# AvishaiBarnoy/membrane_solver

Measured on AMD Instinct MI355X. Metric: minimizer steps/sec (energy+grad+CG) on 2M-facet icosphere, higher is better.
Workload: dtype f64

## Files before the change

### include/membrane_hip.h

```cpp
#ifndef MEMBRANE_HIP_H
#define MEMBRANE_HIP_H

#include <stddef.h>
#include <stdint.h>

#ifdef __cplusplus
extern "C" {
#endif

#define MS_OK 0
#define MS_ERR_INVALID (-1)
#define MS_ERR_HIP (-2)
#define MS_ERR_TILE_CAPACITY (-3)
#define MS_ERR_STATE (-4)
#define MS_ERR_NOMEM (-5)

#define MS_MOD_SURFACE 1u
#define MS_MOD_BENDING 2u
#define MS_MOD_VOLUME_PENALTY 4u
#define MS_CON_VOLUME 8u
#define MS_TRACK_VOLUME 16u
#define MS_MOD_TILT 32u
#define MS_MOD_BENDING_TILT 64u
#define MS_MOD_TILT_SMOOTH 128u
// ... 162 lines not shown
  double lambda;
  double center[3];
  double normal[3];
  double radius;
} ms_disk_target_params;
int ms_set_leaflet_disk_target(ms_ctx *ctx, int leaflet, const uint8_t *disk_rows ,
                               const ms_disk_target_params *params);
int ms_set_leaflet_bending(ms_ctx *ctx, int leaflet, const double *kappa , const double *c0 );
int ms_leaflet_tilt_energy_and_gradient(ms_ctx *ctx, double *energy, double *grad_in ,
                                        double *grad_out );
int ms_leaflet_tilt_energy_and_gradient_ex(ms_ctx *ctx, int module_form, double *energy,
                                           double *grad_in , double *grad_out );
int ms_relax_leaflet_tilts(ms_ctx *ctx, const ms_tilt_relax_params *params,
                           int *iters_out, int *evals_out);

int ms_project_tilts_to_tangent(ms_ctx *ctx);

int ms_angle_defects(ms_ctx *ctx, double *defects );
int ms_curvature_fields(ms_ctx *ctx, double *mean_curvature_normal, double *h_area_anglesum,
                        double *defect_kg, double *principal);

int ms_set_positions(ms_ctx *ctx, const double *positions );
int ms_get_positions(ms_ctx *ctx, double *positions );
int ms_get_gradient(ms_ctx *ctx, double *grad );
int ms_get_vertex_buffer(ms_ctx *ctx, int buffer, double *out );

int ms_energy_and_gradient(ms_ctx *ctx, double energies[4], double *grad);
int ms_energy_and_raw_gradient(ms_ctx *ctx, double energies[4], double *grad);
int ms_energy(ms_ctx *ctx, double energies[4]);

int ms_step(ms_ctx *ctx, const ms_stepper_params *sp, double step_size,
            double tol, ms_step_result *out);
int ms_reset_stepper(ms_ctx *ctx);

typedef struct ms_minimize_params {
  ms_stepper_params stepper;
  double step_size;
  double tol;
  int fixed_step_mode;
  double fixed_step;
  int max_zero_steps;
  double step_size_floor;
  int drift_check;
  double target_volume;
  double volume_tolerance;
  int project_on_drift;
  int relax_tilts;
  ms_tilt_relax_params relax;
} ms_minimize_params;

typedef struct ms_minimize_result {
  int iterations;
  int converged;
  int zero_step_exit;
  int step_success;
  int accepted, trials, guard_rejects, moved;
  double step_size;
  double energy_eval;
  double grad_norm;
  int volume_cache_current;
  int energy_current_valid;
  double energy_current;
} ms_minimize_result;

int ms_minimize(ms_ctx *ctx, const ms_minimize_params *params, int n_steps,
                ms_minimize_result *out, double *step_log);
int ms_project_volume(ms_ctx *ctx, double target, double tol, int max_iter,
                      int *iters_out, double *volume_out);
int ms_project_volume_cached(ms_ctx *ctx, double target, double tol, int max_iter,
                             int first_step_cached, int *iters_out, double *volume_out);

int ms_phase_energy(ms_ctx *ctx, int use_direction, double alpha, int write_trial,
                    int guard, int write_bending_factors);
int ms_phase_gradient(ms_ctx *ctx);
int ms_phase_direction(ms_ctx *ctx, int stepper, int use_history);
int ms_phase_accept(ms_ctx *ctx, int keep_history);
int ms_fetch_scalars(ms_ctx *ctx, double *out );
int ms_store_scalars(ms_ctx *ctx, const double *in );

int ms_phase_commit_trial(ms_ctx *ctx, double alpha, int keep_history);

int ms_phase_gradient_direction(ms_ctx *ctx, int stepper, int use_history);
int ms_phase_set_factors_valid(ms_ctx *ctx, int valid);

int ms_boundary_info(ms_ctx *ctx, int64_t info[4]);
size_t ms_exchange_bytes(ms_ctx *ctx, int n_buffers, const int *buffer_ids);
int ms_pack_boundary(ms_ctx *ctx, int n_buffers, const int *buffer_ids,
                     void *send_dev, size_t send_bytes);
int ms_unpack_boundary(ms_ctx *ctx, int n_buffers, const int *buffer_ids,
                       const void *recv_dev, size_t stride_bytes,
                       double *scal_all_host);

typedef int (*ms_allgather_fn)(void *user, const void *send_dev, void *recv_dev,
                               size_t bytes_per_rank);
int ms_shard_unique_id(void *id128);
int ms_shard_comm_init(ms_ctx *ctx, const void *id128);
int ms_shard_set_allgather(ms_ctx *ctx, ms_allgather_fn fn, void *user);
int ms_shard_peer_export(ms_ctx *ctx, void *handles128);
int ms_shard_peer_open(ms_ctx *ctx, const void *handles_all);
int ms_shard_peer_local(ms_ctx *ctx, void **recv_slab, void **flag_words);
int ms_shard_peer_set_pointers(ms_ctx *ctx, void *const *recv_slabs, void *const *flag_words);
typedef int (*ms_barrier_fn)(void *user);
int ms_shard_peer_set_barrier(ms_ctx *ctx, ms_barrier_fn fn, void *user);
int ms_shard_step(ms_ctx *ctx, const ms_stepper_params *params, double step_size,
                  double tol, ms_step_result *out);
int64_t ms_shard_exchange_count(const ms_ctx *ctx);
int ms_shard_chain_stats(const ms_ctx *ctx, int64_t stats[8]);
int ms_shard_comm_ranks(ms_ctx *ctx);
int ms_shard_peer_memory_kind(const ms_ctx *ctx);

size_t ms_state_bytes(const ms_ctx *ctx);
int ms_rebind_state(ms_ctx *ctx, void *device_base, size_t bytes);

int ms_device_buffer(ms_ctx *ctx, int buffer, void **dev_ptr, size_t *bytes);
int ms_shard_info(ms_ctx *ctx, int64_t *nvp, int64_t *row0, int64_t *row1,
                  int64_t *rows_per_shard);
int ms_tile_stats(ms_ctx *ctx, int64_t *n_tiles, int64_t *facet_instances,
                  int64_t *max_halo, int64_t *lds_bytes_energy,
                  int64_t *lds_bytes_gradient);

#define MS_PROF_KINDS 13
int ms_profile_enable(ms_ctx *ctx, int on);
int ms_profile_read(ms_ctx *ctx, double total_ms[MS_PROF_KINDS],
                    int64_t launches[MS_PROF_KINDS]);

int ms_queue_stats(ms_ctx *ctx, int64_t stats[8]);
int ms_direction_stats(ms_ctx *ctx, int64_t *skipped, int64_t *materialized);
int ms_exec_stats(ms_ctx *ctx, int64_t stats[4]);
int ms_resident_stats(ms_ctx *ctx, int64_t stats[4]);

#define MS_PIN_STAGE_FIXED 0
#define MS_PIN_STAGE_PLANE_GROUP 1
#define MS_PIN_STAGE_CIRCLE_GROUP 2
#define MS_PIN_OP_PLANE 0
#define MS_PIN_OP_CIRCLE 1
#define MS_PIN_GRAD_PLANE 0
#define MS_PIN_GRAD_CIRCLE 1
#define MS_PIN_GRAD_RADIAL 2
#define MS_PIN_LANE_SKIP 0
#define MS_PIN_LANE_PROJECT 1
int ms_set_pins(ms_ctx *ctx, int n_params, const double *params, int n_stages, const int32_t *stage_kind,
                const int32_t *stage_param, const int32_t *stage_off, const int32_t *item_row,
                const int32_t *item_arg, int lane, int n_grad, const int32_t *grad_row, const int32_t *grad_kind,
                const int32_t *grad_param, int n_avg, const int32_t *avg_param, const int32_t *avg_off,
                const int32_t *avg_row);
int ms_enforce_pins(ms_ctx *ctx);
int ms_pin_stats(ms_ctx *ctx, int64_t stats[4]);
int ms_tsearch_stats(ms_ctx *ctx, int64_t stats[2]);
int ms_exec_trace(ms_ctx *ctx, int on, double *rows, int max_rows, int *n_rows);

int ms_plan_tiling(int nv, int nf, const double *positions, const int32_t *tri,
                   int tile_vertices, int shard_count, int64_t stats[8],
                   int32_t *perm_out);
int ms_plan_tiling_conflicts(int nv, int nf, const double *positions,
                             const int32_t *tri, int tile_vertices, double model[4]);

int ms_surface_energy_and_gradient_host(int nv, int nf, const double *pos,
                                        const int32_t *tri, const double *gamma,
                                        double *grad, double *energy);
int ms_grad_cotan_batch_host(int n, const double *u, const double *v,
                             double *grad_u, double *grad_v);
int ms_apply_beltrami_laplacian_host(int dim, int nv, int nf,
                                     const double *weights, const int32_t *tri,
                                     const double *field, double *out);
int ms_p1_triangle_divergence_host(int nv, int nf, const double *pos,
                                   const double *tilts, const int32_t *tri,
                                   double *div_tri, double *area, double *g0,
                                   double *g1, double *g2);
int ms_compute_curvature_data_host(int nv, int nf, const double *pos,
                                   const int32_t *tri, double *k_vecs,
                                   double *vertex_areas, double *weights,
                                   double *va0, double *va1, double *va2);

#ifdef __cplusplus
}
#endif
#endif
```

### membrane_solver_amd/_lib.py

```python

from __future__ import annotations

import ctypes
import os
import subprocess

_PKG = os.path.dirname(os.path.abspath(__file__))
LIB_PATH = os.environ.get("MEMBRANE_HIP_LIB") or os.path.join(_PKG, "libmembrane_hip.so")
_CSRC = os.path.join(_PKG, "csrc")

MS_OK = 0
MS_ERR = {-1: "MS_ERR_INVALID", -2: "MS_ERR_HIP", -3: "MS_ERR_TILE_CAPACITY",
          -4: "MS_ERR_STATE", -5: "MS_ERR_NOMEM"}

MS_MOD_SURFACE = 1
MS_MOD_BENDING = 2
MS_MOD_VOLUME_PENALTY = 4
MS_CON_VOLUME = 8
MS_TRACK_VOLUME = 16
MS_MOD_TILT = 32
MS_MOD_BENDING_TILT = 64
MS_MOD_TILT_SMOOTH = 128
MS_MOD_TILT_IN, MS_MOD_TILT_OUT, MS_MOD_TILT_SMOOTH_IN, MS_MOD_TILT_SMOOTH_OUT = 256, 512, 1024, 2048
MS_MOD_BENDING_TILT_IN, MS_MOD_BENDING_TILT_OUT = 4096, 8192
# ... 42 lines not shown
                ("tol", ctypes.c_double), ("jacobi", ctypes.c_int)]


class ms_leaflet_params(ctypes.Structure):
    _fields_ = [("tilt_modulus", ctypes.c_double), ("tilt_mass_consistent", ctypes.c_int),
                ("smoothness", ctypes.c_double), ("precond_smoothness", ctypes.c_double)]


class ms_disk_target_params(ctypes.Structure):
    _fields_ = [("strength", ctypes.c_double), ("theta_b", ctypes.c_double), ("lam", ctypes.c_double),
                ("center", ctypes.c_double * 3), ("normal", ctypes.c_double * 3), ("radius", ctypes.c_double)]


class ms_minimize_params(ctypes.Structure):
    _fields_ = [("stepper", ms_stepper_params), ("step_size", ctypes.c_double), ("tol", ctypes.c_double),
                ("fixed_step_mode", ctypes.c_int), ("fixed_step", ctypes.c_double),
                ("max_zero_steps", ctypes.c_int), ("step_size_floor", ctypes.c_double),
                ("drift_check", ctypes.c_int), ("target_volume", ctypes.c_double),
                ("volume_tolerance", ctypes.c_double), ("project_on_drift", ctypes.c_int),
                ("relax_tilts", ctypes.c_int), ("relax", ms_tilt_relax_params)]


class ms_minimize_result(ctypes.Structure):
    _fields_ = [("iterations", ctypes.c_int), ("converged", ctypes.c_int), ("zero_step_exit", ctypes.c_int),
                ("step_success", ctypes.c_int), ("accepted", ctypes.c_int), ("trials", ctypes.c_int),
                ("guard_rejects", ctypes.c_int), ("moved", ctypes.c_int), ("step_size", ctypes.c_double),
                ("energy_eval", ctypes.c_double), ("grad_norm", ctypes.c_double),
                ("volume_cache_current", ctypes.c_int), ("energy_current_valid", ctypes.c_int),
                ("energy_current", ctypes.c_double)]


class ms_step_result(ctypes.Structure):
    _fields_ = [("success", ctypes.c_int), ("converged", ctypes.c_int), ("trials", ctypes.c_int),
                ("guard_rejects", ctypes.c_int), ("next_step", ctypes.c_double),
                ("energy", ctypes.c_double), ("alpha", ctypes.c_double),
                ("energy_eval", ctypes.c_double), ("grad_norm", ctypes.c_double),
                ("g_dot_d", ctypes.c_double), ("volume", ctypes.c_double)]


_P = ctypes.c_void_p
_D = ctypes.POINTER(ctypes.c_double)
_I32 = ctypes.POINTER(ctypes.c_int32)
_U8 = ctypes.POINTER(ctypes.c_uint8)
_I64 = ctypes.POINTER(ctypes.c_int64)

ALLGATHER_FN = ctypes.CFUNCTYPE(ctypes.c_int, ctypes.c_void_p, ctypes.c_void_p, ctypes.c_void_p, ctypes.c_size_t)

SIGNATURES = {
    "ms_version": (ctypes.c_char_p, []),
    "ms_device_count": (ctypes.c_int, []),
    "ms_last_error": (ctypes.c_char_p, [_P]),
    "ms_create": (ctypes.c_int, [ctypes.POINTER(_P), ctypes.c_int, ctypes.c_int, ctypes.c_int, _D,
                                 _I32, _U8, _U8, _U8, ctypes.c_int, ctypes.c_int, ctypes.c_int]),
    "ms_destroy": (None, [_P]),
    "ms_set_stream": (ctypes.c_int, [_P, _P]),
    "ms_set_surface_tension": (ctypes.c_int, [_P, _D]),
    "ms_set_bending_params": (ctypes.c_int, [_P, _D, _D]),
    "ms_set_params": (ctypes.c_int, [_P, ctypes.POINTER(ms_params)]),
    "ms_set_area_penalty": (ctypes.c_int, [_P, ctypes.c_double, ctypes.c_double]),
    "ms_get_body_area": (ctypes.c_int, [_P, _D]),
    "ms_set_line_tension": (ctypes.c_int, [_P, ctypes.c_int, _I32, _I32, _D]),
    "ms_get_line_energy": (ctypes.c_int, [_P, _D]),
    "ms_line_stats": (ctypes.c_int, [_P, _D]),
    "ms_line_tables_host": (ctypes.c_int, [ctypes.c_int, _I32, ctypes.c_int, _I32, _I32, _D, _I32, _I32, _I32, _D, _I32,
                                          _I32, _I32, _D]),
    "ms_set_tilts": (ctypes.c_int, [_P, _D, ctypes.c_double]),
    "ms_get_tilts": (ctypes.c_int, [_P, _D]),
    "ms_get_tilt_gradient": (ctypes.c_int, [_P, _D]),
    "ms_project_tilts_to_tangent": (ctypes.c_int, [_P]),
    "ms_angle_defects": (ctypes.c_int, [_P, _D]),
    "ms_curvature_fields": (ctypes.c_int, [_P, _D, _D, _D, _D]),
    "ms_set_tilt_fixed": (ctypes.c_int, [_P, ctypes.POINTER(ctypes.c_uint8)]),
    "ms_set_tilt_smoothness": (ctypes.c_int, [_P, ctypes.c_double]),
    "ms_set_deterministic": (ctypes.c_int, [_P, ctypes.c_int]),
    "ms_tilt_energy_and_gradient": (ctypes.c_int, [_P, _D, _D]),
    "ms_relax_tilts": (ctypes.c_int, [_P, ctypes.POINTER(ms_tilt_relax_params),
                                      ctypes.POINTER(ctypes.c_int), ctypes.POINTER(ctypes.c_int)]),
    "ms_set_leaflet_tilts": (ctypes.c_int, [_P, ctypes.c_int, _D, ctypes.POINTER(ctypes.c_uint8),
                                            ctypes.POINTER(ms_leaflet_params)]),
    "ms_get_leaflet_tilts": (ctypes.c_int, [_P, ctypes.c_int, _D]),
    "ms_set_leaflet_bending": (ctypes.c_int, [_P, ctypes.c_int, _D, _D]),
    "ms_set_leaflet_disk_target": (ctypes.c_int, [_P, ctypes.c_int, ctypes.POINTER(ctypes.c_uint8),
                                                  ctypes.POINTER(ms_disk_target_params)]),
    "ms_leaflet_tilt_energy_and_gradient": (ctypes.c_int, [_P, _D, _D, _D]),
    "ms_leaflet_tilt_energy_and_gradient_ex": (ctypes.c_int, [_P, ctypes.c_int, _D, _D, _D]),
    "ms_relax_leaflet_tilts": (ctypes.c_int, [_P, ctypes.POINTER(ms_tilt_relax_params),
                                              ctypes.POINTER(ctypes.c_int), ctypes.POINTER(ctypes.c_int)]),
    "ms_set_positions": (ctypes.c_int, [_P, _D]),
    "ms_get_positions": (ctypes.c_int, [_P, _D]),
    "ms_get_gradient": (ctypes.c_int, [_P, _D]),
    "ms_get_vertex_buffer": (ctypes.c_int, [_P, ctypes.c_int, _D]),
    "ms_energy_and_gradient": (ctypes.c_int, [_P, _D, _D]),
    "ms_energy_and_raw_gradient": (ctypes.c_int, [_P, _D, _D]),
    "ms_energy": (ctypes.c_int, [_P, _D]),
    "ms_step": (ctypes.c_int, [_P, ctypes.POINTER(ms_stepper_params), ctypes.c_double,
                               ctypes.c_double, ctypes.POINTER(ms_step_result)]),
    "ms_reset_stepper": (ctypes.c_int, [_P]),
    "ms_minimize": (ctypes.c_int, [_P, ctypes.POINTER(ms_minimize_params), ctypes.c_int,
                                   ctypes.POINTER(ms_minimize_result), _D]),
    "ms_project_volume": (ctypes.c_int, [_P, ctypes.c_double, ctypes.c_double, ctypes.c_int,
                                         ctypes.POINTER(ctypes.c_int), _D]),
    "ms_project_volume_cached": (ctypes.c_int, [_P, ctypes.c_double, ctypes.c_double, ctypes.c_int, ctypes.c_int,
                                                ctypes.POINTER(ctypes.c_int), _D]),
    "ms_phase_energy": (ctypes.c_int, [_P, ctypes.c_int, ctypes.c_double, ctypes.c_int,
                                       ctypes.c_int, ctypes.c_int]),
    "ms_phase_gradient": (ctypes.c_int, [_P]),
    "ms_phase_direction": (ctypes.c_int, [_P, ctypes.c_int, ctypes.c_int]),
    "ms_phase_accept": (ctypes.c_int, [_P, ctypes.c_int]),
    "ms_phase_commit_trial": (ctypes.c_int, [_P, ctypes.c_double, ctypes.c_int]),
    "ms_phase_gradient_direction": (ctypes.c_int, [_P, ctypes.c_int, ctypes.c_int]),
    "ms_phase_set_factors_valid": (ctypes.c_int, [_P, ctypes.c_int]),
    "ms_boundary_info": (ctypes.c_int, [_P, _I64]),
    "ms_exchange_bytes": (ctypes.c_size_t, [_P, ctypes.c_int, ctypes.POINTER(ctypes.c_int)]),
    "ms_pack_boundary": (ctypes.c_int, [_P, ctypes.c_int, ctypes.POINTER(ctypes.c_int), _P,
                                        ctypes.c_size_t]),
    "ms_unpack_boundary": (ctypes.c_int, [_P, ctypes.c_int, ctypes.POINTER(ctypes.c_int), _P,
                                          ctypes.c_size_t, _D]),
    "ms_shard_unique_id": (ctypes.c_int, [_P]),
    "ms_shard_comm_init": (ctypes.c_int, [_P, _P]),
    "ms_shard_set_allgather": (ctypes.c_int, [_P, ALLGATHER_FN, _P]),
    "ms_shard_step": (ctypes.c_int, [_P, ctypes.POINTER(ms_stepper_params), ctypes.c_double, ctypes.c_double,
                                     ctypes.POINTER(ms_step_result)]),
    "ms_shard_exchange_count": (ctypes.c_int64, [_P]),
    "ms_shard_chain_stats": (ctypes.c_int, [_P, _I64]),
    "ms_shard_comm_ranks": (ctypes.c_int, [_P]),
    "ms_shard_peer_memory_kind": (ctypes.c_int, [_P]),
    "ms_state_bytes": (ctypes.c_size_t, [_P]),
    "ms_rebind_state": (ctypes.c_int, [_P, _P, ctypes.c_size_t]),
    "ms_fetch_scalars": (ctypes.c_int, [_P, _D]),
    "ms_store_scalars": (ctypes.c_int, [_P, _D]),
    "ms_device_buffer": (ctypes.c_int, [_P, ctypes.c_int, ctypes.POINTER(_P),
                                        ctypes.POINTER(ctypes.c_size_t)]),
    "ms_shard_info": (ctypes.c_int, [_P, _I64, _I64, _I64, _I64]),
    "ms_tile_stats": (ctypes.c_int, [_P, _I64, _I64, _I64, _I64, _I64]),
    "ms_profile_enable": (ctypes.c_int, [_P, ctypes.c_int]),
    "ms_profile_read": (ctypes.c_int, [_P, _D, _I64]),
    "ms_queue_stats": (ctypes.c_int, [_P, _I64]),
    "ms_direction_stats": (ctypes.c_int, [_P, _I64, _I64]),
    "ms_exec_stats": (ctypes.c_int, [_P, _I64]),
    "ms_resident_stats": (ctypes.c_int, [_P, _I64]),
    "ms_set_pins": (ctypes.c_int, [_P, ctypes.c_int, _D, ctypes.c_int, _I32, _I32, _I32, _I32, _I32, ctypes.c_int,
                                   ctypes.c_int, _I32, _I32, _I32, ctypes.c_int, _I32, _I32, _I32]),
    "ms_enforce_pins": (ctypes.c_int, [_P]),
    "ms_pin_stats": (ctypes.c_int, [_P, _I64]),
    "ms_tsearch_stats": (ctypes.c_int, [_P, _I64]),
    "ms_exec_trace": (ctypes.c_int, [_P, ctypes.c_int, _D, ctypes.c_int, ctypes.POINTER(ctypes.c_int)]),
    "ms_shard_peer_export": (ctypes.c_int, [_P, _P]),
    "ms_shard_peer_open": (ctypes.c_int, [_P, _P]),
    "ms_shard_peer_local": (ctypes.c_int, [_P, ctypes.POINTER(_P), ctypes.POINTER(_P)]),
    "ms_shard_peer_set_pointers": (ctypes.c_int, [_P, ctypes.POINTER(_P), ctypes.POINTER(_P)]),
    "ms_shard_peer_set_barrier": (ctypes.c_int, [_P, _P, _P]),
    "ms_plan_tiling": (ctypes.c_int, [ctypes.c_int, ctypes.c_int, _D, _I32, ctypes.c_int, ctypes.c_int,
                                      _I64, _I32]),
    "ms_plan_tiling_conflicts": (ctypes.c_int, [ctypes.c_int, ctypes.c_int, _D, _I32, ctypes.c_int, _D]),
    "ms_surface_energy_and_gradient_host": (ctypes.c_int, [ctypes.c_int, ctypes.c_int, _D, _I32, _D,
                                                           _D, _D]),
    "ms_grad_cotan_batch_host": (ctypes.c_int, [ctypes.c_int, _D, _D, _D, _D]),
    "ms_apply_beltrami_laplacian_host": (ctypes.c_int, [ctypes.c_int, ctypes.c_int, ctypes.c_int, _D,
                                                        _I32, _D, _D]),
    "ms_p1_triangle_divergence_host": (ctypes.c_int, [ctypes.c_int, ctypes.c_int, _D, _D, _I32, _D,
                                                      _D, _D, _D, _D]),
    "ms_compute_curvature_data_host": (ctypes.c_int, [ctypes.c_int, ctypes.c_int, _D, _I32, _D, _D,
                                                      _D, _D, _D, _D]),
}

_lib = None


def build(force: bool = False, fp_contract: str | None = None) -> str:
    srcs = [os.path.join(_CSRC, f) for f in ("ms_kernels.hip", "ms_pins.hip", "ms_line.hip", "ms_api.cpp",
                                             "ms_tiles.cpp", "ms_internal.h", "Makefile")]
    srcs.append(os.path.join(_PKG, "..", "include", "membrane_hip.h"))
    stale = (not os.path.exists(LIB_PATH)) or any(
        os.path.exists(s) and os.path.getmtime(s) > os.path.getmtime(LIB_PATH) for s in srcs)
    if force or stale:
        cmd = ["make", "-s", "-C", _CSRC]
        if force:
            cmd.append("-B")
        if fp_contract:
            cmd.append(f"MS_FP_CONTRACT={fp_contract}")
        subprocess.check_call(cmd)
    return LIB_PATH


HIP_RUNTIME_PATH = None


def _preload_hip_runtime() -> str:
    global HIP_RUNTIME_PATH
    if HIP_RUNTIME_PATH is not None:
        return HIP_RUNTIME_PATH
    candidates = []
    if os.environ.get("MEMBRANE_HIP_RUNTIME"):
        candidates.append(os.environ["MEMBRANE_HIP_RUNTIME"])
    try:
        import importlib.util

        spec = importlib.util.find_spec("torch")
        if spec is not None and spec.submodule_search_locations:
            candidates.append(os.path.join(list(spec.submodule_search_locations)[0], "lib", "libamdhip64.so"))
    except Exception:
        pass
    rocm = os.environ.get("ROCM_PATH", "/opt/rocm")
    candidates += [os.path.join(rocm, "lib", "libamdhip64.so"), "libamdhip64.so.7", "libamdhip64.so"]
    errors = []
    for c in candidates:
        if os.path.isabs(c) and not os.path.exists(c):
            continue
        try:
            ctypes.CDLL(c, mode=ctypes.RTLD_GLOBAL)
            HIP_RUNTIME_PATH = c
            return c
        except OSError as e:
            errors.append(f"{c}: {e}")
    raise MembraneHipError("no HIP runtime (libamdhip64) could be loaded: " + "; ".join(errors))


def lib() -> ctypes.CDLL:
    global _lib
    if _lib is None:
        if not os.path.exists(LIB_PATH):
            raise MembraneHipError(
                f"{LIB_PATH} is missing: run `python -c 'import __graft_entry__ as g; g.build()'` "
                "(hipcc --offload-arch=gfx950).  There is no CPU fallback for this path.")
        _preload_hip_runtime()
        cd = ctypes.CDLL(LIB_PATH)
        for name, (res, args) in SIGNATURES.items():
            fn = getattr(cd, name)
            fn.restype = res
            fn.argtypes = args
        _lib = cd
    return _lib


def check(rc: int, ctx=None, what: str = "") -> None:
    if rc == MS_OK:
        return
    msg = lib().ms_last_error(ctx)
    text = msg.decode("utf-8", "replace") if msg else ""
    raise MembraneHipError(f"{what or 'libmembrane_hip'} failed: {MS_ERR.get(rc, rc)}: {text}")
```

### membrane_solver_amd/csrc/ms_api_context.inc

```
extern "C" {

const char* ms_version(void) { return "membrane_hip 0.1 (gfx950)"; }

int ms_device_count(void) {
  int n = 0;
  hipError_t e = hipGetDeviceCount(&n);
  if (e != hipSuccess) {
    g_last_error = std::string("hipGetDeviceCount: ") + hipGetErrorString(e);
    return MS_ERR_HIP;
  }
  return n;
}

const char* ms_last_error(const ms_ctx* ctx) {
  return ctx ? ctx->err.c_str() : g_last_error.c_str();
}

int ms_create(ms_ctx** out, int device, int nv, int nf, const double* positions,
              const int32_t* tri, const uint8_t* fixed, const uint8_t* boundary,
              const uint8_t* body_facets, int tile_vertices, int shard_rank, int shard_count) {
  if (!out) return fail(nullptr, MS_ERR_INVALID, "ms_create: out is NULL");
  *out = nullptr;
  if (shard_count < 1 || shard_rank < 0 || shard_rank >= shard_count)
    return fail(nullptr, MS_ERR_INVALID, "ms_create: bad shard_rank/shard_count");
  ms_ctx* c = new (std::nothrow) ms_ctx();
  if (!c) return fail(nullptr, MS_ERR_NOMEM, "ms_create: out of host memory");
  std::string err;
  int rc = build_tiling(nv, nf, positions, tri, body_facets, tile_vertices, shard_count, c->til, err);
  if (rc != MS_OK) {
    delete c;
    return fail(nullptr, rc, err);
  }
  c->device = device;
  c->shard_rank = shard_rank;
  c->shard_count = shard_count;
  const Tiling& t = c->til;
  c->tile0 = std::min(t.n_tiles, shard_rank * t.tiles_per_shard);
  c->tile1 = std::min(t.n_tiles, (shard_rank + 1) * t.tiles_per_shard);
  c->cap = t.own + t.max_halo;
  {
    const size_t le = energy_lds_bytes(t.T, c->cap, t.max_ent, true, true, true);
    const size_t lg = gradient_lds_bytes(t.T, c->cap, t.max_ent, true, true);
    if (le > 160 * 1024 || lg > 160 * 1024) {
      delete c;
      return fail(nullptr, MS_ERR_TILE_CAPACITY,
                  "ms_create: a vertex patch (tile + halo) exceeds the 160 KiB LDS of a CU; "
                  "use a smaller tile_vertices");
    }
  }
#define CREATE_CHK(call)                                       \
  do {                                                         \
    int rc_ = (call);                                          \
    if (rc_ != MS_OK) {                                        \
      std::string m_ = c->err;                                 \
      ms_destroy(c);                                           \
      return fail(nullptr, rc_, m_);                           \
    }                                                          \
  } while (0)
#define CREATE_HIP(call)                                                         \
  do {                                                                           \
    hipError_t e_ = (call);                                                      \
    if (e_ != hipSuccess) {                                                      \
      std::string m_ = std::string(#call) + ": " + hipGetErrorString(e_);        \
      ms_destroy(c);                                                             \
      return fail(nullptr, MS_ERR_HIP, m_);                                      \
    }                                                                            \
  } while (0)
  CREATE_HIP(hipSetDevice(device));
  CREATE_HIP(hipStreamCreateWithFlags(&c->stream, hipStreamNonBlocking));
  c->own_stream = true;
  CREATE_CHK(upload(c, &c->d_perm, t.perm));
  CREATE_CHK(upload(c, &c->d_tile_facet_off, t.tile_facet_off));
  CREATE_CHK(upload(c, &c->d_tile_facets, t.tile_facets));
  if (t.own + t.max_halo <= 1024) {
    std::vector<uint32_t> packed(t.tile_facets.size());
    for (size_t i = 0; i < packed.size(); ++i) {
      const TileFacet& f = t.tile_facets[i];
      packed[i] = (uint32_t)f.l0 | ((uint32_t)f.l1 << 10) | ((uint32_t)f.l2 << 20) | ((uint32_t)(f.flags & 3u) << 30);
    }
    CREATE_CHK(upload(c, &c->d_tile_facets32, packed));
  }
  CREATE_CHK(upload(c, &c->d_tile_halo_off, t.tile_halo_off));
  CREATE_CHK(upload(c, &c->d_halo_ids, t.halo_ids));
  CREATE_CHK(upload(c, &c->d_tile_ent_off, t.tile_ent_off));
  CREATE_CHK(upload(c, &c->d_tile_voff, t.tile_voff));
  CREATE_CHK(upload(c, &c->d_vent, t.vent));
  {
    std::vector<double> ones(t.tile_facets.size(), 1.0);
    CREATE_CHK(upload(c, &c->d_tf_gamma, ones));
  }
  {
    std::vector<uint8_t> fl((size_t)t.nvp, VF_FIXED);
    for (int i = 0; i < nv; ++i) {
      const int e = t.perm[i];
      uint8_t f = 0;
      if (fixed && fixed[e]) f |= VF_FIXED;
      if (boundary && boundary[e]) {
        f |= VF_BOUNDARY;
        c->has_boundary = true;
      }
      fl[i] = f;
    }
    CREATE_CHK(upload(c, &c->d_vflags, fl));
    c->h_vflags = fl;
    std::vector<double> zeros((size_t)t.nvp, 0.0);
    CREATE_CHK(upload(c, &c->d_kappa, zeros));
    CREATE_CHK(upload(c, &c->d_c0, zeros));
  }
  {
    const size_t n3 = 3 * (size_t)t.nvp;
    const size_t total = 8 * n3 + 2 * (size_t)t.nvp;
    CREATE_HIP(hipMalloc(reinterpret_cast<void**>(&c->state), total * sizeof(double)));
    CREATE_HIP(hipMemset(c->state, 0, total * sizeof(double)));
    for (int b = 0; b <= MS_BUF_FK; ++b) c->buf[b] = c->state + (size_t)b * n3;
    c->buf[MS_BUF_FA] = c->state + 8 * n3;
  }
  CREATE_HIP(hipMalloc(reinterpret_cast<void**>(&c->d_partials),
                       sizeof(double) * MS_NPART * (size_t)std::max(1, t.n_tiles)));
  CREATE_HIP(hipMemset(c->d_partials, 0, sizeof(double) * MS_NPART * (size_t)std::max(1, t.n_tiles)));
  CREATE_HIP(hipMalloc(reinterpret_cast<void**>(&c->d_scal), sizeof(double) * MS_NSCAL));
  CREATE_HIP(hipMemset(c->d_scal, 0, sizeof(double) * MS_NSCAL));
  c->buf[MS_BUF_SCAL] = c->d_scal;
  c->h_scal = static_cast<double*>(calloc(MS_NSCAL, sizeof(double)));
  CREATE_HIP(hipHostMalloc(reinterpret_cast<void**>(&c->h_seq), sizeof(unsigned long long) * 2 * MS_MB_WORDS,
                           hipHostMallocMapped));
  memset(c->h_seq, 0, sizeof(unsigned long long) * 2 * MS_MB_WORDS);
  CREATE_HIP(hipHostGetDevicePointer(reinterpret_cast<void**>(&c->d_h_seq), c->h_seq, 0));
  CREATE_HIP(hipHostMalloc(reinterpret_cast<void**>(&c->h_err), sizeof(unsigned long long) * 8, hipHostMallocMapped));
  memset(c->h_err, 0, sizeof(unsigned long long) * 8);
  CREATE_HIP(hipHostGetDevicePointer(reinterpret_cast<void**>(&c->d_h_err), c->h_err, 0));
  CREATE_HIP(hipMalloc(reinterpret_cast<void**>(&c->d_stage), sizeof(double) * 3 * (size_t)nv));
  {
    const int W = shard_count;
    const int rows_per = t.tiles_per_shard * t.own;
    std::vector<std::vector<int32_t>> lists((size_t)W);
    std::vector<int32_t> my_halo;
    for (int tile = 0; tile < t.n_tiles; ++tile) {
      const int tr = tile / t.tiles_per_shard;
      for (int h = t.tile_halo_off[tile]; h < t.tile_halo_off[tile + 1]; ++h) {
        const int32_t v = t.halo_ids[h];
        const int owner = v / rows_per;
        if (owner == tr) continue;
        lists[(size_t)owner].push_back(v);
        if (tr == shard_rank) my_halo.push_back(v);
      }
    }
    std::vector<int32_t> flat;
    c->bnd_off.assign((size_t)W + 1, 0);
    for (int r = 0; r < W; ++r) {
      auto& l = lists[(size_t)r];
      std::sort(l.begin(), l.end());
      l.erase(std::unique(l.begin(), l.end()), l.end());
      c->bnd_off[(size_t)r + 1] = c->bnd_off[(size_t)r] + (int32_t)l.size();
      c->bnd_max = std::max(c->bnd_max, (int)l.size());
      flat.insert(flat.end(), l.begin(), l.end());
    }
    std::sort(my_halo.begin(), my_halo.end());
    my_halo.erase(std::unique(my_halo.begin(), my_halo.end()), my_halo.end());
    c->n_halo_rows = (int)my_halo.size();
    CREATE_CHK(upload(c, &c->d_bnd_rows, flat));
    CREATE_CHK(upload(c, &c->d_bnd_off, c->bnd_off));
    CREATE_CHK(upload(c, &c->d_halo_rows, my_halo));
    CREATE_HIP(hipMalloc(reinterpret_cast<void**>(&c->d_scal_all), sizeof(double) * MS_NSCAL * (size_t)W));
    CREATE_HIP(hipMemset(c->d_scal_all, 0, sizeof(double) * MS_NSCAL * (size_t)W));
  }
  {
    TiltField& f0 = c->tf[0];
    f0.fixed_bit = VF_TILT_FIXED; f0.mod_tilt = MS_MOD_TILT; f0.mod_smooth = MS_MOD_TILT_SMOOTH;
    f0.s_etilt = MS_S_ETILT; f0.s_ets = MS_S_ETS; f0.s_gn2 = MS_S_TGNORM2; f0.s_rz = MS_S_TRZ;
    TiltField& f1 = c->tf[1];
    f1.fixed_bit = VF_TILT_FIXED_IN; f1.mod_tilt = MS_MOD_TILT_IN; f1.mod_smooth = MS_MOD_TILT_SMOOTH_IN;
    f1.s_etilt = MS_S_ETILT_IN; f1.s_ets = MS_S_ETS_IN; f1.s_gn2 = MS_S_TGNORM2_IN; f1.s_rz = MS_S_TRZ_IN;
    f1.mod_bt = MS_MOD_BENDING_TILT_IN; f1.s_ebt = MS_S_EBT_IN; f1.div_sign = -1.0;
    f0.mod_bt = MS_MOD_BENDING_TILT; f0.s_ebt = MS_S_EBT;
    f1.mod_dt = MS_MOD_TILT_DISK_TARGET_IN; f1.s_edt = MS_S_EDT_IN; f1.s_dtr = MS_S_DTR_IN;
    TiltField& f2 = c->tf[2];
    f2.fixed_bit = VF_TILT_FIXED_OUT; f2.mod_tilt = MS_MOD_TILT_OUT; f2.mod_smooth = MS_MOD_TILT_SMOOTH_OUT;
    f2.s_etilt = MS_S_ETILT_OUT; f2.s_ets = MS_S_ETS_OUT; f2.s_gn2 = MS_S_TGNORM2_OUT; f2.s_rz = MS_S_TRZ_OUT;
    f2.mod_bt = MS_MOD_BENDING_TILT_OUT; f2.s_ebt = MS_S_EBT_OUT; f2.div_sign = 1.0;
    f2.mod_dt = MS_MOD_TILT_DISK_TARGET_OUT; f2.s_edt = MS_S_EDT_OUT; f2.s_dtr = MS_S_DTR_OUT;
  }
  if (const char* pe = getenv("MS_PAIR")) {
    c->pair_enable = atoi(pe) != 0;
    c->pair_force = atoi(pe) >= 2 ? std::min(atoi(pe), 4) : 0;
  }
  c->speculate = !(getenv("MS_SPECULATE") != nullptr && atoi(getenv("MS_SPECULATE")) == 0);
  c->ahead_enable = !(getenv("MS_AHEAD") != nullptr && atoi(getenv("MS_AHEAD")) == 0);
  c->escalate = !(getenv("MS_ESCALATE") != nullptr && atoi(getenv("MS_ESCALATE")) == 0);
  if (getenv("MS_ESCALATE") != nullptr && atoi(getenv("MS_ESCALATE")) > 0) c->escalate_after = atoi(getenv("MS_ESCALATE"));
  c->ls_reset = !(getenv("MS_LS_RESET") != nullptr && atoi(getenv("MS_LS_RESET")) == 0);
  c->no_fast = variant_env("MS_NO_FAST") != nullptr && atoi(variant_env("MS_NO_FAST")) != 0;
  c->pair_lean_enable = !(getenv("MS_PAIR_LEAN") != nullptr && atoi(getenv("MS_PAIR_LEAN")) == 0);
  c->deterministic = getenv("MS_DETERMINISTIC") != nullptr && atoi(getenv("MS_DETERMINISTIC")) != 0;
  c->resident_enable = !(getenv("MS_RESIDENT") != nullptr && atoi(getenv("MS_RESIDENT")) == 0);
  c->params.modules = MS_MOD_SURFACE;
  c->params.bending_model = MS_BEND_HELFRICH;
  c->params.bending_grad_mode = MS_GRAD_ANALYTIC;
  c->params.volume_stiffness = 1000.0;
  c->params.target_volume = 0.0;
  c->carry.last_g = c->buf[MS_BUF_G];
  c->exec_wanted = t.n_tiles == 1 && t.T == 256 && t.own == 256 && shard_count == 1 &&
                   !(getenv("MS_EXEC") != nullptr && atoi(getenv("MS_EXEC")) == 0);
  if (c->exec_wanted) {
    c->exec.stream = c->stream;
    c->exec.T = t.T;
    exec_attach(&c->exec);
    c->exec_on = true;
    c->pair_enable = false;
    c->exec_relax = !(getenv("MS_EXEC_RELAX") != nullptr && atoi(getenv("MS_EXEC_RELAX")) == 0);
    c->exec_fused = !(getenv("MS_EXEC_FUSED") != nullptr && atoi(getenv("MS_EXEC_FUSED")) == 0);
  }
  c->shard_chain_enable = !(getenv("MS_SHARD_CHAIN") != nullptr && atoi(getenv("MS_SHARD_CHAIN")) == 0);
  c->tenergy_enable = shard_count == 1 && !(getenv("MS_TSEARCH") != nullptr && atoi(getenv("MS_TSEARCH")) == 0);
  c->tsearch_enable = !c->exec_on && c->tenergy_enable;
  CREATE_CHK(ext_to_patch(c, positions, c->buf[MS_BUF_X], 3));
#undef CREATE_CHK
#undef CREATE_HIP
  *out = c;
  return MS_OK;
}

void ms_destroy(ms_ctx* c) {
  if (g_host_timing.on && g_host_timing.n > 0) {
    fprintf(stderr, "[ms host timing] %ld waits followed by an energy launch: mailbox seen -> launch call returned %.2f us "
                    "on average (max %.1f), of which the launch call itself %.2f us\n",
            g_host_timing.n, g_host_timing.sum_gap / g_host_timing.n, g_host_timing.max_gap,
            g_host_timing.sum_launch / g_host_timing.n);
    g_host_timing.n = 0;
    g_host_timing.sum_gap = g_host_timing.sum_launch = g_host_timing.max_gap = 0.0;
  }
  if (!c) return;
  (void)hipSetDevice(c->device);
  if (c->exec_on) {
    (void)c->exec.flush();
    exec_detach(&c->exec);
    c->exec_on = false;
  }
  if (c->stream) (void)hipStreamSynchronize(c->stream);
  if (!c->own_state) c->state = nullptr;
  void* ptrs[] = {c->d_perm, c->d_tile_facet_off, c->d_tile_facets, c->d_tile_facets32, c->d_tf_gamma, c->d_volgrad_cache,
                  c->d_tile_halo_off, c->d_halo_ids, c->d_tile_ent_off, c->d_tile_voff, c->d_vent,
                  c->d_vflags, c->d_kappa, c->d_c0, c->tf[0].tilts, c->tf[0].grad, c->tf[0].trial, c->d_bt_vert, c->d_tn, c->tf[0].dir, c->tf[0].minv,
                  c->tf[1].tilts, c->tf[1].grad, c->tf[1].trial, c->tf[1].dir, c->tf[1].minv,
                  c->tf[2].tilts, c->tf[2].grad, c->tf[2].trial, c->tf[2].dir, c->tf[2].minv,
                  c->tf[1].kappa, c->tf[1].c0, c->tf[1].bt_vert, c->tf[2].kappa, c->tf[2].c0, c->tf[2].bt_vert,
                  c->tf[1].disk, c->tf[1].diff, c->tf[2].disk, c->tf[2].diff, c->tf[0].va, c->tf[1].va, c->tf[2].va,
                  c->state, c->d_partials, c->d_scal, c->d_stage, c->d_bnd_rows, c->d_bnd_off,
                  c->d_halo_rows, c->d_scal_all, c->d_pins, c->d_line};
  for (void* p : ptrs)
    if (p) (void)hipFree(p);
  for (auto& evs : c->line_prof)
    for (auto& ev : evs) {
      (void)hipEventDestroy(ev.first);
      (void)hipEventDestroy(ev.second);
    }
  for (void* q : c->peer_opened) (void)hipIpcCloseMemHandle(q);
  if (c->d_peer_slab) (void)hipFree(c->d_peer_slab);
  if (c->d_peer_flag) (void)hipFree(c->d_peer_flag);
  if (c->d_peer_flagtab) (void)hipFree(c->d_peer_flagtab);
  if (c->d_peer_arrived) (void)hipFree(c->d_peer_arrived);
  if (c->comm) shard_comm_destroy(c->comm);
  if (c->d_xsend) (void)hipFree(c->d_xsend);
  if (c->d_xrecv) (void)hipFree(c->d_xrecv);
  if (c->h_scal_all) (void)hipHostFree(c->h_scal_all);
  if (c->h_xseq) (void)hipHostFree(c->h_xseq);
  for (int p = 0; p < 2; ++p) {
    for (auto& m : c->spec[p]) {
      free(m.h_scal);
      if (m.h_seq) (void)hipHostFree(m.h_seq);
    }
    for (ms_ctx::Mailbox* m : {&c->grad_mb[p], &c->first_mb[p]}) {
      free(m->h_scal);
      if (m->h_seq) (void)hipHostFree(m->h_seq);
    }
  }
  if (c->d_sh_dec) (void)hipFree(c->d_sh_dec);
  if (c->h_sh_post) (void)hipHostFree(c->h_sh_post);
  free(c->tsearch_mb.h_scal);
  if (c->tsearch_mb.h_seq) (void)hipHostFree(c->tsearch_mb.h_seq);
  if (c->d_dec) (void)hipFree(c->d_dec);
  if (c->h_err) (void)hipHostFree(c->h_err);
  if (c->d_prof_ran) (void)hipFree(c->d_prof_ran);
  if (c->exec.d_stamps) (void)hipFree(c->exec.d_stamps);
  if (c->d_res_partials) (void)hipFree(c->d_res_partials);
  if (c->d_res_bar) (void)hipFree(c->d_res_bar);
  if (c->d_res_log) (void)hipFree(c->d_res_log);
  if (c->d_res_result) (void)hipFree(c->d_res_result);
  for (int l = 0; l < 3; ++l)
    if (c->tf[l].dt_target) (void)hipFree(c->tf[l].dt_target);
  if (c->d_relax_cells) (void)hipFree(c->d_relax_cells);
  if (c->h_relax_box) (void)hipHostFree(c->h_relax_box);
  for (auto& sd : c->side) {
    if (sd.partials) (void)hipFree(sd.partials);
    if (sd.scal) (void)hipFree(sd.scal);
    for (auto& m : sd.mb) {
      free(m.h_scal);
      if (m.h_seq) (void)hipHostFree(m.h_seq);
    }
  }
  for (double* q : {c->xt2, c->fK2, c->fA2, c->xt3, c->fK3, c->fA3})
    if (q) (void)hipFree(q);
  free(c->h_scal);
  if (c->h_seq) (void)hipHostFree(c->h_seq);
  for (auto& r : c->prof_pending) {
    (void)hipEventDestroy(r.a);
    (void)hipEventDestroy(r.b);
  }
  for (auto e : c->prof_pool) (void)hipEventDestroy(e);
  if (c->own_stream && c->stream) (void)hipStreamDestroy(c->stream);
  delete c;
}

int ms_set_stream(ms_ctx* c, void* hip_stream) {
  if (!c) return MS_ERR_INVALID;
  HIPCHK(c, hipStreamSynchronize(S(c)));
  if (c->own_stream && c->stream) {
    HIPCHK(c, hipStreamDestroy(c->stream));
    c->own_stream = false;
  }
  if (hip_stream) {
    c->stream = static_cast<hipStream_t>(hip_stream);
  } else {
    HIPCHK(c, hipStreamCreateWithFlags(&c->stream, hipStreamNonBlocking));
    c->own_stream = true;
  }
  if (c->exec_on) {
    exec_detach(&c->exec);
    c->exec.stream = c->stream;
    if (exec_find(c->stream) != nullptr) {
      c->exec_on = false;
      c->exec_wanted = false;
    } else {
      exec_attach(&c->exec);
    }
  } else {
    c->exec.stream = c->stream;
  }
  return MS_OK;
}

int ms_set_surface_tension(ms_ctx* c, const double* gamma) {
  if (!c || !gamma) return fail(c, MS_ERR_INVALID, "ms_set_surface_tension: NULL argument");
  const Tiling& t = c->til;
  HIPCHK(c, hipStreamSynchronize(S(c)));
  std::vector<double> g(t.tile_facets.size());
  for (size_t p = 0; p < g.size(); ++p) g[p] = gamma[t.tile_facet_ext[p]];
  c->gamma_uniform = true;
  c->gamma_const = t.nf > 0 ? gamma[0] : 1.0;
  for (int f = 1; f < t.nf && c->gamma_uniform; ++f) c->gamma_uniform = gamma[f] == c->gamma_const;
  if (!g.empty())
    HIPCHK(c, hipMemcpy(c->d_tf_gamma, g.data(), g.size() * sizeof(double), hipMemcpyHostToDevice));
  c->carry.carry_valid = c->carry.grad_valid = c->carry.bt_valid = c->carry.maxg2_valid = false;
  c->sh_carry_valid = c->sh_grad_valid = false;
  return MS_OK;
}

int ms_set_bending_params(ms_ctx* c, const double* kappa, const double* c0) {
  if (!c || !kappa || !c0) return fail(c, MS_ERR_INVALID, "ms_set_bending_params: NULL argument");
  const Tiling& t = c->til;
  HIPCHK(c, hipStreamSynchronize(S(c)));
  std::vector<double> k((size_t)t.nvp, 0.0), z((size_t)t.nvp, 0.0);
  c->kc_uniform = true;
  c->kappa_const = kappa[0];
  c->c0_const = c0[0];
  for (int i = 0; i < t.nv; ++i) {
    k[i] = kappa[t.perm[i]];
    z[i] = c0[t.perm[i]];
    c->kc_uniform = c->kc_uniform && kappa[i] == c->kappa_const && c0[i] == c->c0_const;
  }
  HIPCHK(c, hipMemcpy(c->d_kappa, k.data(), k.size() * sizeof(double), hipMemcpyHostToDevice));
  HIPCHK(c, hipMemcpy(c->d_c0, z.data(), z.size() * sizeof(double), hipMemcpyHostToDevice));
  c->carry.factors_valid = false;
  c->carry.carry_valid = c->carry.grad_valid = c->carry.bt_valid = c->carry.maxg2_valid = false;
  c->sh_carry_valid = c->sh_grad_valid = false;
  return MS_OK;
}

int ms_set_params(ms_ctx* c, const ms_params* p) {
  if (!c || !p) return fail(c, MS_ERR_INVALID, "ms_set_params: NULL argument");
  if (p->bending_model != MS_BEND_HELFRICH && p->bending_model != MS_BEND_WILLMORE)
    return fail(c, MS_ERR_INVALID, "ms_set_params: bad bending_model");
  if (p->bending_grad_mode != MS_GRAD_ANALYTIC && p->bending_grad_mode != MS_GRAD_APPROX)
    return fail(c, MS_ERR_INVALID, "ms_set_params: bad bending_grad_mode");
  if ((p->modules & MS_MOD_BENDING) && (p->modules & MS_MOD_BENDING_TILT))
    return fail(c, MS_ERR_INVALID, "ms_set_params: bending and bending_tilt are mutually exclusive");
  if ((p->modules & MS_LEAFLET_BT) && (p->modules & (MS_MOD_BENDING | MS_MOD_BENDING_TILT)))
    return fail(c, MS_ERR_INVALID, "ms_set_params: bending / bending_tilt together with bending_tilt_in/out is outside the device path");
  if ((p->modules & MS_MOD_BENDING_TILT) && c->shard_count != 1)
    return fail(c, MS_ERR_STATE, "the bending_tilt module is not sharded yet (single GPU only)");
  if ((p->modules & MS_MOD_AREA_PENALTY) && c->shard_count != 1)
    return fail(c, MS_ERR_STATE, "the body_area_penalty module is not sharded (single GPU only)");
  if ((p->modules & MS_MOD_AREA_PENALTY) && (p->modules & MS_ANY_TILT_MODS))
    return fail(c, MS_ERR_STATE, "body_area_penalty together with a tilt-family module is outside the device path");
  if ((p->modules & MS_MOD_LINE_TENSION) && c->shard_count != 1)
    return fail(c, MS_ERR_STATE, "the line_tension module is not sharded (single GPU only)");
  if ((p->modules & MS_MOD_LINE_TENSION) && (p->modules & MS_ANY_TILT_MODS))
    return fail(c, MS_ERR_STATE, "line_tension together with a tilt-family module is outside the device path");
  if ((p->modules & MS_MOD_BENDING_TILT) && !c->d_bt_vert) {
    const size_t bytes = sizeof(double) * 4 * (size_t)c->til.nvp;
    HIPCHK(c, hipMalloc(reinterpret_cast<void**>(&c->d_bt_vert), bytes));
    HIPCHK(c, hipMemset(c->d_bt_vert, 0, bytes));
  }
  c->params = *p;
  c->carry.factors_valid = false;
  c->carry.carry_valid = c->carry.grad_valid = c->carry.bt_valid = c->carry.maxg2_valid = false;
  c->sh_carry_valid = c->sh_grad_valid = false;
  return MS_OK;
}

int ms_set_area_penalty(ms_ctx* c, double stiffness, double target_area) {
  if (!c) return MS_ERR_INVALID;
  if (!std::isfinite(stiffness) || !std::isfinite(target_area))
    return fail(c, MS_ERR_INVALID, "ms_set_area_penalty: stiffness and target area must be finite");
  c->area_stiffness = stiffness;
  c->target_area = target_area;
  c->carry.carry_valid = c->carry.grad_valid = c->carry.maxg2_valid = false;
  c->sh_carry_valid = c->sh_grad_valid = false;
  return MS_OK;
}

int ms_get_body_area(ms_ctx* c, double* area) {
  if (!c || !area) return fail(c, MS_ERR_INVALID, "ms_get_body_area: NULL argument");
  if (!(c->params.modules & MS_MOD_AREA_PENALTY))
    return fail(c, MS_ERR_STATE, "ms_get_body_area: MS_MOD_AREA_PENALTY is not in the module mask");
  int rc = fetch(c);
  if (rc) return rc;
  *area = c->h_scal[MS_S_AREA];
  return MS_OK;
}

int ms_set_tilts(ms_ctx* c, const double* tilts, double tilt_rigidity) {
  if (!c || !tilts) return fail(c, MS_ERR_INVALID, "ms_set_tilts: NULL argument");
  const size_t bytes = sizeof(double) * 3 * (size_t)c->til.nvp;
  if (!c->tf[0].tilts) {
    HIPCHK(c, hipMalloc(reinterpret_cast<void**>(&c->tf[0].tilts), bytes));
    HIPCHK(c, hipMalloc(reinterpret_cast<void**>(&c->tf[0].grad), bytes));
    HIPCHK(c, hipMalloc(reinterpret_cast<void**>(&c->tf[0].trial), bytes));
    HIPCHK(c, hipMemset(c->tf[0].trial, 0, bytes));
    HIPCHK(c, hipMemset(c->tf[0].tilts, 0, bytes));
    HIPCHK(c, hipMemset(c->tf[0].grad, 0, bytes));
  }
  c->tf[0].k_tilt = tilt_rigidity;
  c->carry.carry_valid = c->carry.grad_valid = c->carry.bt_valid = c->carry.maxg2_valid = false;
  c->sh_carry_valid = c->sh_grad_valid = false;
  return ext_to_patch(c, tilts, c->tf[0].tilts, 3);
}

int ms_get_tilts(ms_ctx* c, double* tilts) {
  if (!c || !tilts || !c->tf[0].tilts) return fail(c, MS_ERR_INVALID, "ms_get_tilts: no tilts set");
  return patch_to_ext(c, c->tf[0].tilts, tilts, 3);
}

int ms_get_tilt_gradient(ms_ctx* c, double* tilt_grad) {
  if (!c || !tilt_grad || !c->tf[0].grad) return fail(c, MS_ERR_INVALID, "ms_get_tilt_gradient: no tilts set");
  return patch_to_ext(c, c->tf[0].grad, tilt_grad, 3);
}

int ms_angle_defects(ms_ctx* c, double* defects) {
  if (!c || !defects) return fail(c, MS_ERR_INVALID, "ms_angle_defects: NULL argument");
  if (c->shard_count != 1) return fail(c, MS_ERR_STATE, "ms_angle_defects: single shard only");
  const Tiling& t = c->til;
  double* d_out = nullptr;
  HIPCHK(c, hipMalloc(reinterpret_cast<void**>(&d_out), sizeof(double) * (size_t)std::max<int64_t>(1, t.nvp)));
  HIPCHK(c, hipMemsetAsync(d_out, 0, sizeof(double) * (size_t)std::max<int64_t>(1, t.nvp), S(c)));
  TiltArgs a;
  a.fields = nullptr;
  a.fields_rows = 0;
  a.m = device_mesh(c);
  a.tile0 = c->tile0;
  a.tile1 = c->tile1;
  a.x = c->buf[MS_BUF_X];
  a.d = nullptr;
  a.alpha = 0.0;
  a.tilts = c->buf[MS_BUF_X];
  a.tilts_out = nullptr;
  a.k_tilt = 0.0;
  a.g = nullptr;
  a.tilt_grad = nullptr;
  a.minv = d_out;
  a.partials = c->d_partials;
  a.e_slot = MS_S_ETILT;
  a.consistent = 0;
  a.tg_accumulate = 0;
  a.cons_tilt_grad = 0;
  a.va_out = nullptr;
  hipError_t e = launch_tilt(a, 4, c->cap, t.max_ent, c->stream);
  int rc = MS_OK;
  if (e != hipSuccess) rc = fail(c, MS_ERR_HIP, std::string("ms_angle_defects: ") + hipGetErrorString(e));
  if (rc == MS_OK) rc = patch_to_ext(c, d_out, defects, 1);
  (void)hipStreamSynchronize(S(c));
  (void)hipFree(d_out);
  return rc;
}

int ms_curvature_fields(ms_ctx* c, double* mean_curvature_normal, double* h_area_anglesum, double* defect_kg,
                        double* principal) {
  if (!c) return MS_ERR_INVALID;
  if (c->shard_count != 1) return fail(c, MS_ERR_STATE, "ms_curvature_fields: single shard only");
  const Tiling& t = c->til;
  const size_t plane = 3 * (size_t)std::max<int64_t>(1, t.nvp);
  double* d_out = nullptr;
  HIPCHK(c, hipMalloc(reinterpret_cast<void**>(&d_out), sizeof(double) * 4 * plane));
  HIPCHK(c, hipMemsetAsync(d_out, 0, sizeof(double) * 4 * plane, S(c)));
  TiltArgs a;
// ... 78 lines not shown
```

### membrane_solver_amd/csrc/ms_api_ctx.inc

```
struct StageCtl {
  const uint32_t* cur_gate = nullptr;
  uint32_t cur_gate_want = 0;
  bool cur_gate_fold_only = false;
  bool cur_check_ran = false;
  uint32_t* cur_dec = nullptr;
  double cur_rhs[MS_MAX_TRIALS] = {0};
  const double* cur_rhs_dev = nullptr;
  uint32_t cur_extra_mask = 0;
  int cur_go_kind = 0;
  uint32_t* cur_go = nullptr;
  double cur_go_val[6] = {0};
  int cur_parity = 0;
  int pair_on = 0;
  bool pair_lean = false;
  double pair_alpha[MS_MAX_TRIALS] = {0};
  double* pair_scal2 = nullptr;
  bool multi_any_slot = false;
  bool defer_dir = false;
  bool energy_tilt_only = false;
  bool proj_at_x_in_normals = false;
};
struct CarryState {
  bool dir_implicit = false;
  bool dir_unwritten = false;
  bool pd_neg_pg = false;
  bool kc_pending = false;
  int kc_parity = 0;
  bool bt_valid = false;
  double* last_g = nullptr;
  bool cg_have_history = false;
  int cg_iter_count = 0;
  bool factors_valid = false;
  bool carry_valid = false;
  bool grad_valid = false;
  bool maxg2_valid = false;
};
struct ms_ctx {
  int device = 0;
  hipStream_t stream = nullptr;
  bool own_stream = false;
  Tiling til;
  int shard_rank = 0, shard_count = 1;
  int tile0 = 0, tile1 = 0;
  int cap = 0;
  int32_t* d_perm = nullptr;
  int32_t* d_tile_facet_off = nullptr;
  TileFacet* d_tile_facets = nullptr;
  uint32_t* d_tile_facets32 = nullptr;
  double* d_tf_gamma = nullptr;
  double* d_volgrad_cache = nullptr;
  double volgrad_cache_norm2 = 0.0;
  bool volgrad_cache_valid = false;
  bool gamma_uniform = true, kc_uniform = true;
  double gamma_const = 1.0, kappa_const = 0.0, c0_const = 0.0;
  int32_t* d_tile_halo_off = nullptr;
  int32_t* d_halo_ids = nullptr;
  int32_t* d_tile_ent_off = nullptr;
  uint16_t* d_tile_voff = nullptr;
  uint16_t* d_vent = nullptr;
  uint8_t* d_vflags = nullptr;
  double* d_kappa = nullptr;
  double* d_c0 = nullptr;
  struct TiltField {
    double* tilts = nullptr;
    double* trial = nullptr;
    double* grad = nullptr;
    double* dir = nullptr;
    double* minv = nullptr;
    double k_tilt = 0.0;
    int consistent = 0;
    double k_smooth = 0.0;
    double k_smooth_precond = 0.0;
    uint8_t fixed_bit = 0;
    uint32_t mod_tilt = 0, mod_smooth = 0, mod_bt = 0;
    int s_etilt = 0, s_ets = 0, s_gn2 = 0, s_rz = 0, s_ebt = 0;
    double* kappa = nullptr;
    double* c0 = nullptr;
    double* bt_vert = nullptr;
    double div_sign = 1.0;
    uint8_t* disk = nullptr;
    double* diff = nullptr;
    double* dt_target = nullptr;
    bool dt_target_valid = false;
    ms_disk_target_params dt = {};
    uint32_t mod_dt = 0;
    int s_edt = 0, s_dtr = 0;
    bool any_free = true;
    double* va = nullptr;
  } tf[3];
  CarryState carry;
  bool precond = false;
  static constexpr int SPEC_STAGES = 3;
  struct Mailbox {
    double* h_scal = nullptr;
    unsigned long long* h_seq = nullptr;
    unsigned long long* d_h_seq = nullptr;
    unsigned long long expected[MS_MB_WORDS] = {0};
  } spec[2][SPEC_STAGES];
  Mailbox first_mb[2];
  Mailbox grad_mb[2];
  int next_parity = 0;
  struct RoundPlanT {
    int n0 = 1, n_st = 0;
    double alphas[MS_MAX_TRIALS + SPEC_STAGES] = {0};
  };
  struct Ahead {
    bool valid = false;
    bool go_known = false, go = false;
    int kind = 0, go_kind = 0, parity = 0, src = 0, stepper = 0, max_iter = 0;
    bool implicit = false;
    double alpha0 = 0, energy0 = 0, beta = 0, c1 = 0, tol2p = 0, lim = 0;
    RoundPlanT plan;
  } ahead;
  bool ahead_enable = true;
  int steps_left = 0;
  bool ahead_allowed = false;
  uint32_t dir_deferred_mask = 0;
  bool dir_pending[2] = {false, false};
  uint32_t dir_mask[2] = {0, 0};
  uint32_t* kc_gate[2] = {nullptr, nullptr};
  bool last_hist_descent = false;
  long q_ahead = 0, q_adopted = 0, q_dropped = 0;
  int kc_stepper = 0;
  bool kc_use_history = false;
  bool kc_dir_unwritten[2] = {false, false};
  long dir_skipped = 0, dir_materialized = 0;
  uint32_t* d_dec = nullptr;
  static constexpr int N_DEC = 16;
  unsigned long long* h_err = nullptr;
  unsigned long long* d_h_err = nullptr;
  long queue_mismatches = 0;
  long q_rounds = 0, q_multi = 0, q_wasted = 0, q_side_accepts = 0;
  int escalate_after = 3;
  bool pair_enable = true;
  bool escalate = true;
  int pair_force = 0;
  bool lbt_normals_current = false;
  bool tenergy_enable = true;
  bool tsearch_enable = true;
  bool tsearch_first_single = true;
  int64_t tsearch_launches = 0, tsearch_trials = 0;
  bool tsearch_all_failed = false;
  Mailbox tsearch_mb;
  bool no_fast = false;
  bool pair_lean_enable = true;
  static constexpr int N_SIDE = MS_MAX_TRIALS - 1;
  struct SideSet {
    double* partials = nullptr;
    double* scal = nullptr;
    Mailbox mb[2];
  } side[N_SIDE];
  double* xt3 = nullptr;
  double* fK3 = nullptr;
  double* fA3 = nullptr;
  double* xt2 = nullptr;
  double* fK2 = nullptr;
  double* fA2 = nullptr;
  static constexpr int LS_HIST = 8;
  struct LsHist {
    int pred_trials = 1;
    double acc[LS_HIST] = {0};
    double rej[LS_HIST] = {0};
    int n = 0;
  } ls[2];
  bool ls_reset = true;
  bool speculate = true;
  bool relax_va_valid = false;
  bool tilt_module_form = false;
  int factors_leaflet = 0;
  double* d_bt_vert = nullptr;
  double* d_tn = nullptr;
  std::vector<uint8_t> h_vflags;
  double* state = nullptr;
  bool own_state = true;
  double* buf[MS_BUF_COUNT] = {nullptr};
  double* d_partials = nullptr;
  double* d_scal = nullptr;
  double* h_scal = nullptr;
  unsigned long long* h_seq = nullptr;
  unsigned long long* d_h_seq = nullptr;
  unsigned long long ticket = 0;
  unsigned long long expected[MS_MB_WORDS] = {0};
  bool has_boundary = false;
  double* d_stage = nullptr;
  ms_params params{};
  double area_stiffness = 0.0, target_area = 0.0;
  std::vector<int32_t> bnd_off;
  int32_t* d_bnd_rows = nullptr;
  int32_t* d_bnd_off = nullptr;
  int bnd_max = 0;
  int32_t* d_halo_rows = nullptr;
  int n_halo_rows = 0;
  double* d_scal_all = nullptr;
  void* comm = nullptr;
  ms_allgather_fn allgather_cb = nullptr;
  void* allgather_user = nullptr;
  double* d_xsend = nullptr;
  double* d_xrecv = nullptr;
  bool shard_chain_enable = true;
  uint32_t* d_sh_dec = nullptr;
  unsigned long long* h_sh_post = nullptr;
// ... 93 lines not shown
```

### membrane_solver_amd/csrc/ms_api_misc.inc

```
size_t ms_state_bytes(const ms_ctx* c) {
  if (!c) return 0;
  return sizeof(double) * (8 * 3 * (size_t)c->til.nvp + 2 * (size_t)c->til.nvp);
}

int ms_rebind_state(ms_ctx* c, void* device_base, size_t bytes) {
  if (!c || !device_base) return fail(c, MS_ERR_INVALID, "ms_rebind_state: NULL argument");
  const size_t need = ms_state_bytes(c);
  if (bytes < need) return fail(c, MS_ERR_INVALID, "ms_rebind_state: buffer smaller than ms_state_bytes");
  HIPCHK(c, hipStreamSynchronize(S(c)));
  HIPCHK(c, hipMemcpy(device_base, c->state, need, hipMemcpyDeviceToDevice));
  double* nb = static_cast<double*>(device_base);
  for (int b = 0; b <= MS_BUF_FA; ++b) c->buf[b] = nb + (c->buf[b] - c->state);
  c->carry.last_g = nb + (c->carry.last_g - c->state);
  if (c->own_state) HIPCHK(c, hipFree(c->state));
  c->state = nb;
  c->own_state = false;
  return MS_OK;
}

int ms_fetch_scalars(ms_ctx* c, double* out) {
  if (!c || !out) return MS_ERR_INVALID;
  int rc = fetch(c);
  if (rc) return rc;
  memcpy(out, c->h_scal, sizeof(double) * MS_NSCAL);
// ... 54 lines not shown
  for (int k = 0; k < 8; ++k) stats[k] = 0;
  stats[0] = c->q_rounds;
  stats[1] = c->q_multi;
  stats[2] = c->q_wasted;
  stats[3] = c->q_side_accepts;
  stats[4] = c->queue_mismatches;
  stats[5] = c->q_ahead;
  stats[6] = c->q_adopted;
  stats[7] = c->q_dropped;
  return MS_OK;
}

int ms_direction_stats(ms_ctx* c, int64_t* skipped, int64_t* materialized) {
  if (!c || !skipped || !materialized) return MS_ERR_INVALID;
  *skipped = c->dir_skipped;
  *materialized = c->dir_materialized;
  return MS_OK;
}

int ms_resident_stats(ms_ctx* c, int64_t stats[4]) {
  if (!c || !stats) return MS_ERR_INVALID;
  stats[0] = c->resident_ok;
  stats[1] = c->resident_launches;
  stats[2] = c->resident_steps;
  stats[3] = c->resident_bails;
  return MS_OK;
}

int ms_tsearch_stats(ms_ctx* c, int64_t stats[2]) {
  if (!c || !stats) return MS_ERR_INVALID;
  stats[0] = c->tsearch_launches;
  stats[1] = c->tsearch_trials;
  return MS_OK;
}

int ms_exec_stats(ms_ctx* c, int64_t stats[4]) {
  if (!c || !stats) return MS_ERR_INVALID;
  stats[0] = c->exec_on ? 1 : 0;
  stats[1] = c->exec.launches;
  stats[2] = c->exec.cmds;
  stats[3] = (c->exec_wanted ? 1 : 0) | ((int64_t)(c->relax_programs & 0xffffff) << 8) | ((int64_t)c->relax_fused_runs << 32);
  return MS_OK;
}

int ms_exec_trace(ms_ctx* c, int on, double* rows, int max_rows, int* n_rows) {
  if (!c) return MS_ERR_INVALID;
  if (n_rows) *n_rows = 0;
  int rc = exec_flush(c);
  if (rc) return rc;
  HIPCHK(c, hipStreamSynchronize(c->stream));
  if (c->exec.d_stamps && rows && max_rows > 0 && n_rows) {
    std::vector<unsigned long long> h((size_t)2 * EXEC_STAMP_CAP);
    HIPCHK(c, hipMemcpy(h.data(), c->exec.d_stamps, sizeof(unsigned long long) * h.size(), hipMemcpyDeviceToHost));
    const size_t n = (size_t)std::min<unsigned long long>(h[0], (unsigned long long)EXEC_STAMP_CAP - 1);
    std::map<unsigned long long, std::pair<long, double>> acc;
    for (size_t i = 0; i < n; ++i) {
      auto& e = acc[h[1 + 2 * i]];
      e.first += 1;
      e.second += 0.01 * (double)h[2 + 2 * i];
    }
    int k = 0;
    for (auto& kv : acc) {
      if (k >= max_rows) break;
      rows[4 * k] = (double)(kv.first >> 32);
      rows[4 * k + 1] = (double)(kv.first & 0xffffffffull);
      rows[4 * k + 2] = (double)kv.second.first;
      rows[4 * k + 3] = kv.second.second;
      ++k;
    }
    *n_rows = k;
  }
  if (on && !c->exec.d_stamps)
    HIPCHK(c, hipMalloc(reinterpret_cast<void**>(&c->exec.d_stamps), sizeof(unsigned long long) * 2 * EXEC_STAMP_CAP));
  if (c->exec.d_stamps) HIPCHK(c, hipMemset(c->exec.d_stamps, 0, sizeof(unsigned long long) * 2 * EXEC_STAMP_CAP));
  if (!on && c->exec.d_stamps) {
    (void)hipFree(c->exec.d_stamps);
    c->exec.d_stamps = nullptr;
  }
  return MS_OK;
}

int ms_profile_enable(ms_ctx* c, int on) {
  if (!c) return MS_ERR_INVALID;
  if (on && !c->d_prof_ran) {
    HIPCHK(c, hipMalloc(reinterpret_cast<void**>(&c->d_prof_ran), sizeof(uint32_t) * ms_ctx::PROF_RAN_CAP));
    HIPCHK(c, hipMemset(c->d_prof_ran, 0, sizeof(uint32_t) * ms_ctx::PROF_RAN_CAP));
  }
  if (on && c->exec_on) {
    int rc = exec_flush(c);
    if (rc) return rc;
    exec_detach(&c->exec);
    c->exec_on = false;
  } else if (!on && c->exec_wanted && !c->exec_on) {
    c->exec.stream = c->stream;
    exec_attach(&c->exec);
    c->exec_on = true;
  }
  c->profiling = on != 0;
  return MS_OK;
}

int ms_profile_read(ms_ctx* c, double total_ms[MS_PROF_KINDS], int64_t launches[MS_PROF_KINDS]) {
  if (!c || !total_ms || !launches) return MS_ERR_INVALID;
  HIPCHK(c, hipStreamSynchronize(S(c)));
  std::vector<uint32_t> ran((size_t)c->prof_ran_next);
  if (c->prof_ran_next > 0)
    HIPCHK(c, hipMemcpy(ran.data(), c->d_prof_ran, sizeof(uint32_t) * ran.size(), hipMemcpyDeviceToHost));
  c->prof_ran_next = 0;
  for (auto& r : c->prof_pending) {
    float ms = 0.f;
    const bool empty = r.ran_idx >= 0 && ran[(size_t)r.ran_idx] == 0u;
    if (hipEventElapsedTime(&ms, r.a, r.b) == hipSuccess && !empty) {
      c->prof_ms[r.kind] += ms;
      c->prof_n[r.kind] += 1;
    }
    c->prof_pool.push_back(r.a);
    c->prof_pool.push_back(r.b);
  }
  c->prof_pending.clear();
  for (int k = 0; k < MS_PROF_KINDS; ++k) {
    total_ms[k] = c->prof_ms[k];
    launches[k] = c->prof_n[k];
    c->prof_ms[k] = 0.0;
    c->prof_n[k] = 0;
  }
  return MS_OK;
}

int ms_plan_tiling(int nv, int nf, const double* positions, const int32_t* tri, int tile_vertices,
                   int shard_count, int64_t stats[8], int32_t* perm_out) {
  if (!stats) return fail(nullptr, MS_ERR_INVALID, "ms_plan_tiling: stats is NULL");
  Tiling t;
  std::string err;
  int rc = build_tiling(nv, nf, positions, tri, nullptr, tile_vertices, shard_count, t, err);
  if (rc != MS_OK) return fail(nullptr, rc, err);
  int64_t owners = 0, owned_corners = 0;
  for (int tile = 0; tile < t.n_tiles; ++tile) {
    const int n_owned = std::min(t.own, t.nv - tile * t.own);
    for (int p = t.tile_facet_off[tile]; p < t.tile_facet_off[tile + 1]; ++p) {
      const TileFacet& f = t.tile_facets[p];
      if (f.flags & TF_OWNER) ++owners;
      owned_corners += (f.l0 < n_owned) + (f.l1 < n_owned) + (f.l2 < n_owned);
    }
  }
  stats[0] = t.n_tiles;
  stats[1] = (int64_t)t.tile_facets.size();
  stats[2] = t.max_halo;
  stats[3] = t.max_tile_facets;
  stats[4] = t.dropped_facets;
  stats[5] = owners;
  stats[6] = owned_corners;
  stats[7] = (int64_t)gradient_lds_bytes(t.T, t.own + t.max_halo, t.max_ent, true, true);
  if (perm_out) memcpy(perm_out, t.perm.data(), sizeof(int32_t) * (size_t)nv);
  return MS_OK;
}

int ms_plan_tiling_conflicts(int nv, int nf, const double* positions, const int32_t* tri, int tile_vertices,
                             double model[4]) {
  if (!model) return fail(nullptr, MS_ERR_INVALID, "ms_plan_tiling_conflicts: model is NULL");
  Tiling t;
  std::string err;
  int rc = build_tiling(nv, nf, positions, tri, nullptr, tile_vertices, 1, t, err);
  if (rc != MS_OK) return fail(nullptr, rc, err);
  double rd_cyc = 0, at_cyc = 0, rd_free = 0, at_free = 0;
  int64_t rd_groups = 0, at_groups = 0;
  for (int tile = 0; tile < t.n_tiles; ++tile) {
    const int n_owned = std::min(t.own, t.nv - tile * t.own);
    const int f0 = t.tile_facet_off[tile], f1 = t.tile_facet_off[tile + 1];
    for (int k = 0; k < 3; ++k) {
      for (int g0 = f0; g0 < f1; g0 += 32) {
        int slots[32], ns = 0, cnt[32] = {0};
        for (int p = g0; p < std::min(f1, g0 + 32); ++p) {
          const TileFacet& f = t.tile_facets[p];
          const int s = k == 0 ? f.l0 : (k == 1 ? f.l1 : f.l2);
          bool dup = false;
          for (int q = 0; q < ns; ++q) dup |= slots[q] == s;
          if (!dup) {
            slots[ns++] = s;
            ++cnt[s & 31];
          }
        }
        int mx = 1;
        for (int q = 0; q < 32; ++q) mx = std::max(mx, cnt[q]);
        rd_cyc += mx;
        rd_free += mx == 1;
        ++rd_groups;
      }
      for (int g0 = f0; g0 < f1; g0 += 16) {
        int cnt[16] = {0}, any = 0;
        for (int p = g0; p < std::min(f1, g0 + 16); ++p) {
          const TileFacet& f = t.tile_facets[p];
          const int s = k == 0 ? f.l0 : (k == 1 ? f.l1 : f.l2);
          if (s < n_owned) {
            ++cnt[s & 15];
            any = 1;
          }
        }
        if (!any) continue;
        int mx = 1;
        for (int q = 0; q < 16; ++q) mx = std::max(mx, cnt[q]);
        at_cyc += mx;
        at_free += mx == 1;
        ++at_groups;
      }
    }
  }
  model[0] = rd_groups ? rd_cyc / rd_groups : 0.0;
  model[1] = at_groups ? at_cyc / at_groups : 0.0;
  model[2] = rd_groups ? rd_free / rd_groups : 0.0;
  model[3] = at_groups ? at_free / at_groups : 0.0;
  return MS_OK;
}


int ms_surface_energy_and_gradient_host(int nv, int nf, const double* pos, const int32_t* tri,
                                        const double* gamma, double* grad, double* energy) {
  if (!pos || !gamma || !energy || (nf > 0 && !tri))
    return fail(nullptr, MS_ERR_INVALID, "ms_surface_energy_and_gradient_host: NULL argument");
  ms_ctx* c = nullptr;
  int rc = ms_create(&c, 0, nv, nf, pos, tri, nullptr, nullptr, nullptr, 0, 0, 1);
  if (rc) return rc;
  rc = ms_set_surface_tension(c, gamma);
  ms_params p = c->params;
  p.modules = MS_MOD_SURFACE;
  if (!rc) rc = ms_set_params(c, &p);
  double e[3] = {0, 0, 0};
  std::vector<double> g;
  if (!rc) {
    g.resize(3 * (size_t)nv);
    rc = ms_energy_and_gradient(c, e, grad ? g.data() : nullptr);
  }
  if (rc) g_last_error = c->err;
  ms_destroy(c);
  if (rc) return rc;
  *energy = e[0];
  if (grad)
    for (size_t i = 0; i < g.size(); ++i) grad[i] += g[i];
  return MS_OK;
}

int ms_grad_cotan_batch_host(int n, const double* u, const double* v, double* grad_u, double* grad_v) {
  if (n < 0 || !u || !v || !grad_u || !grad_v)
    return fail(nullptr, MS_ERR_INVALID, "ms_grad_cotan_batch_host: bad argument");
  const size_t b = sizeof(double) * 3 * (size_t)n;
  DevBuf du, dv, dgu, dgv;
  SEAM_HIP(du.alloc(b));
  SEAM_HIP(dv.alloc(b));
  SEAM_HIP(dgu.alloc(b));
  SEAM_HIP(dgv.alloc(b));
  SEAM_HIP(hipMemcpy(du.p, u, b, hipMemcpyHostToDevice));
  SEAM_HIP(hipMemcpy(dv.p, v, b, hipMemcpyHostToDevice));
  SEAM_HIP(launch_grad_cotan(n, du.as<double>(), dv.as<double>(), dgu.as<double>(), dgv.as<double>(), nullptr));
  SEAM_HIP(hipMemcpy(grad_u, dgu.p, b, hipMemcpyDeviceToHost));
  SEAM_HIP(hipMemcpy(grad_v, dgv.p, b, hipMemcpyDeviceToHost));
  return MS_OK;
}

int ms_apply_beltrami_laplacian_host(int dim, int nv, int nf, const double* weights,
                                     const int32_t* tri, const double* field, double* out) {
  if (dim <= 0 || nv <= 0 || nf < 0 || !weights || !tri || !field || !out)
    return fail(nullptr, MS_ERR_INVALID, "ms_apply_beltrami_laplacian_host: bad argument");
  const size_t bw = sizeof(double) * 3 * (size_t)nf, bt = sizeof(int32_t) * 3 * (size_t)nf,
               bf = sizeof(double) * (size_t)nv * dim;
  DevBuf dw, dt, df, dout;
  SEAM_HIP(dw.alloc(bw));
  SEAM_HIP(dt.alloc(bt));
  SEAM_HIP(df.alloc(bf));
  SEAM_HIP(dout.alloc(bf));
  SEAM_HIP(hipMemcpy(dw.p, weights, bw, hipMemcpyHostToDevice));
  SEAM_HIP(hipMemcpy(dt.p, tri, bt, hipMemcpyHostToDevice));
  SEAM_HIP(hipMemcpy(df.p, field, bf, hipMemcpyHostToDevice));
  SEAM_HIP(hipMemset(dout.p, 0, bf));
  SEAM_HIP(launch_laplacian_scatter(dim, nv, nf, dw.as<double>(), dt.as<int32_t>(), df.as<double>(),
                                    dout.as<double>(), nullptr));
  SEAM_HIP(hipMemcpy(out, dout.p, bf, hipMemcpyDeviceToHost));
  return MS_OK;
}

int ms_p1_triangle_divergence_host(int nv, int nf, const double* pos, const double* tilts,
                                   const int32_t* tri, double* div_tri, double* area, double* g0,
                                   double* g1, double* g2) {
  if (nv <= 0 || nf < 0 || !pos || !tilts || !tri || !div_tri || !area || !g0 || !g1 || !g2)
    return fail(nullptr, MS_ERR_INVALID, "ms_p1_triangle_divergence_host: bad argument");
  const size_t bp = sizeof(double) * 3 * (size_t)nv, bt = sizeof(int32_t) * 3 * (size_t)nf,
               b1 = sizeof(double) * (size_t)nf, b3 = 3 * b1;
  DevBuf dp, dtl, dt, dd, da, d0, d1, d2;
  SEAM_HIP(dp.alloc(bp));
  SEAM_HIP(dtl.alloc(bp));
  SEAM_HIP(dt.alloc(bt));
  SEAM_HIP(dd.alloc(b1));
  SEAM_HIP(da.alloc(b1));
  SEAM_HIP(d0.alloc(b3));
  SEAM_HIP(d1.alloc(b3));
  SEAM_HIP(d2.alloc(b3));
  SEAM_HIP(hipMemcpy(dp.p, pos, bp, hipMemcpyHostToDevice));
  SEAM_HIP(hipMemcpy(dtl.p, tilts, bp, hipMemcpyHostToDevice));
  SEAM_HIP(hipMemcpy(dt.p, tri, bt, hipMemcpyHostToDevice));
  SEAM_HIP(hipMemset(dd.p, 0, b1));
  SEAM_HIP(hipMemset(da.p, 0, b1));
  SEAM_HIP(hipMemset(d0.p, 0, b3));
  SEAM_HIP(hipMemset(d1.p, 0, b3));
  SEAM_HIP(hipMemset(d2.p, 0, b3));
  SEAM_HIP(launch_p1_divergence(nv, nf, dp.as<double>(), dtl.as<double>(), dt.as<int32_t>(),
                                dd.as<double>(), da.as<double>(), d0.as<double>(), d1.as<double>(),
                                d2.as<double>(), nullptr));
  SEAM_HIP(hipMemcpy(div_tri, dd.p, b1, hipMemcpyDeviceToHost));
// ... 45 lines not shown
```

### membrane_solver_amd/csrc/ms_api_phases.inc

```
namespace {

inline hipStream_t S(ms_ctx* c) {
  if (c->exec_on) (void)c->exec.flush();
  return c->stream;
}
int pin_grad_run(ms_ctx* c, bool volrow);
int line_energy_run(ms_ctx* c, bool use_dir, double alpha);
int line_grad_run(ms_ctx* c, double* g, bool volrow);
inline int exec_flush(ms_ctx* c) {
  if (!c->exec_on) return MS_OK;
  const hipError_t e = c->exec.flush();
  if (e == hipSuccess) return MS_OK;
  c->err = std::string("k_exec launch: ") + hipGetErrorString(e);
  return MS_ERR_HIP;
}

inline int zero_doubles(ms_ctx* c, double* p, size_t bytes) {
  if (c->exec_on) {
    ExecMemsetArgs a;
    a.p = p;
    a.n = (int64_t)(bytes / sizeof(double));
    const hipError_t e = c->exec.push(CK_MEMSET, 0, 0, 0, 1, 0, 0, &a, sizeof(a));
    if (e == hipSuccess) return MS_OK;
    c->err = std::string("k_exec record: ") + hipGetErrorString(e);
    return MS_ERR_HIP;
  }
  const hipError_t e = hipMemsetAsync(p, 0, bytes, c->stream);
  if (e == hipSuccess) return MS_OK;
  c->err = std::string("hipMemsetAsync: ") + hipGetErrorString(e);
  return MS_ERR_HIP;
}

inline const double* trial_dir(const ms_ctx* c) { return c->carry.dir_implicit ? c->buf[MS_BUF_G] : c->buf[MS_BUF_D]; }
inline double trial_alpha(const ms_ctx* c, double alpha) { return c->carry.dir_implicit ? -alpha : alpha; }

int fail(ms_ctx* c, int code, const std::string& msg) {
  if (c) c->err = msg;
  g_last_error = msg;
  return code;
}

int fail_hip(ms_ctx* c, hipError_t e, const char* what) {
  return fail(c, MS_ERR_HIP, std::string(what) + ": " + hipGetErrorString(e));
}

#define HIPCHK(c, call)                                   \
  do {                                                    \
    hipError_t e_ = (call);                               \
    if (e_ != hipSuccess) return fail_hip((c), e_, #call); \
  } while (0)

DeviceMesh device_mesh(const ms_ctx* c) {
  DeviceMesh m;
  m.nv = c->til.nv;
  m.T = c->til.T;
  m.own = c->til.own;
  m.n_tiles = c->til.n_tiles;
  m.has_boundary = c->has_boundary ? 1 : 0;
  m.tile_facet_off = c->d_tile_facet_off;
  m.tile_facets = c->d_tile_facets;
  m.tile_facets32 = c->d_tile_facets32;
  m.no_fast = c->no_fast ? 1 : 0;
  m.tf_gamma = c->d_tf_gamma;
  m.gamma_uniform = c->gamma_uniform ? 1 : 0;
  m.gamma_const = c->gamma_const;
  m.kc_uniform = c->kc_uniform ? 1 : 0;
  m.kappa_const = c->kappa_const;
  m.c0_const = c->c0_const;
  m.tile_halo_off = c->d_tile_halo_off;
  m.halo_ids = c->d_halo_ids;
  m.tile_ent_off = c->d_tile_ent_off;
  m.tile_voff = c->d_tile_voff;
  m.vent = c->d_vent;
  m.vflags = c->d_vflags;
  m.kappa = c->d_kappa;
  m.c0 = c->d_c0;
  return m;
}

struct HostTiming {
  bool on = getenv("MS_HOST_TIMING") != nullptr && atoi(getenv("MS_HOST_TIMING")) != 0;
  double t_fetch = 0.0;
  bool armed = false;
  double sum_gap = 0.0, sum_launch = 0.0, max_gap = 0.0;
  long n = 0;
  static double now() {
    timespec ts;
    clock_gettime(CLOCK_MONOTONIC, &ts);
    return ts.tv_sec * 1e6 + ts.tv_nsec * 1e-3;
  }
};
static HostTiming g_host_timing;

struct ProfScope {
  ms_ctx* c;
  hipEvent_t a = nullptr, b = nullptr;
  int kind;
  const uint32_t* gate = nullptr;
  uint32_t want = 0;
  ProfScope(ms_ctx* ctx, int k, const uint32_t* gate_word = nullptr, uint32_t gate_want = 0)
      : c(ctx), kind(k), gate(gate_word), want(gate_want) {
    if (!c->profiling || k < 0) return;
    auto get = [&]() {
      hipEvent_t e = nullptr;
      if (!c->prof_pool.empty()) {
        e = c->prof_pool.back();
        c->prof_pool.pop_back();
      } else if (hipEventCreate(&e) != hipSuccess) {
        e = nullptr;
      }
      return e;
    };
    a = get();
    b = get();
    if (a && b) (void)hipEventRecord(a, c->stream);
  }
  ~ProfScope() {
    if (!c->profiling || kind < 0 || !a || !b) return;
    (void)hipEventRecord(b, c->stream);
    int ran_idx = -1;
    if (gate != nullptr && c->d_prof_ran != nullptr && c->prof_ran_next < ms_ctx::PROF_RAN_CAP) {
      ran_idx = c->prof_ran_next++;
      (void)launch_gate_probe(gate, want, c->d_prof_ran + ran_idx, c->stream);
    }
    c->prof_pending.push_back({a, b, kind, ran_idx});
  }
};

constexpr uint32_t MASK_ENERGY = (1u << MS_S_ESURF) | (1u << MS_S_VOL) | (1u << MS_S_EBEND) |
                                 (1u << MS_S_MINEDGE2) | (1u << MS_S_GUARD) | (1u << MS_S_ETILT) |
                                 (1u << MS_S_EBT) | (1u << MS_S_ETS) | (1u << MS_S_ETILT_IN) |
                                 (1u << MS_S_ETILT_OUT) | (1u << MS_S_ETS_IN) | (1u << MS_S_ETS_OUT) |
                                 (1u << MS_S_EBT_IN) | (1u << MS_S_EBT_OUT) | (1u << MS_S_EDT_IN) | (1u << MS_S_EDT_OUT);
constexpr uint32_t MS_TILT_MODS = MS_MOD_TILT | MS_MOD_BENDING_TILT | MS_MOD_TILT_SMOOTH;
constexpr uint32_t MS_LEAFLET_BT = MS_MOD_BENDING_TILT_IN | MS_MOD_BENDING_TILT_OUT;
constexpr uint32_t MS_LEAFLET_DT = MS_MOD_TILT_DISK_TARGET_IN | MS_MOD_TILT_DISK_TARGET_OUT;
constexpr uint32_t MS_LEAFLET_MODS = MS_MOD_TILT_IN | MS_MOD_TILT_OUT | MS_MOD_TILT_SMOOTH_IN | MS_MOD_TILT_SMOOTH_OUT | MS_LEAFLET_BT | MS_LEAFLET_DT;
constexpr uint32_t MS_ANY_TILT_MODS = MS_TILT_MODS | MS_LEAFLET_MODS;
constexpr uint32_t MS_TILT_SHAPE_MODS = MS_MOD_TILT | MS_MOD_TILT_IN | MS_MOD_TILT_OUT | MS_LEAFLET_BT | MS_LEAFLET_DT;
using TiltField = ms_ctx::TiltField;
using RoundPlan = ms_ctx::RoundPlanT;

int active_fields(ms_ctx* c, uint32_t mods, TiltField* out[3]) {
  int n = 0;
  for (int k = 0; k < 3; ++k) {
    TiltField& f = c->tf[k];
    const uint32_t reads = k == 0 ? MS_TILT_MODS : (f.mod_tilt | f.mod_smooth | f.mod_bt | f.mod_dt);
    if (mods & reads) out[n++] = &f;
  }
  return n;
}

int tilt_pass_f(ms_ctx* c, TiltField& f, int mode, bool use_dir, double alpha, const double* src = nullptr,
                double* dst = nullptr, bool shape_gradient = true, bool lumped = false, double k_override = -1.0,
                int slot_override = -1, bool tg_accumulate = false) {
  if (!f.tilts) return fail(c, MS_ERR_STATE, "tilt module active but its tilt field was never set (ms_set_tilts / ms_set_leaflet_tilts)");
  TiltArgs a;
  a.fields = nullptr;
  a.fields_rows = 0;
  a.m = device_mesh(c);
  a.tile0 = c->tile0;
  a.tile1 = c->tile1;
  a.x = c->buf[MS_BUF_X];
  a.d = use_dir ? trial_dir(c) : nullptr;
  a.alpha = trial_alpha(c, alpha);
  a.tilts = src ? src : f.tilts;
  a.tilts_out = dst ? dst : f.tilts;
  a.k_tilt = k_override >= 0.0 ? k_override : f.k_tilt;
  a.g = shape_gradient ? c->buf[MS_BUF_G] : nullptr;
  a.tilt_grad = f.grad;
  a.minv = nullptr;
  a.partials = c->d_partials;
  a.e_slot = slot_override >= 0 ? slot_override : f.s_etilt;
  a.consistent = (f.consistent && !lumped) ? 1 : 0;
  a.tg_accumulate = tg_accumulate ? 1 : 0;
  a.cons_tilt_grad = (a.consistent && c->tilt_module_form) ? 1 : 0;
  a.va_out = nullptr;
  {
    ProfScope ps(c, 4);
    HIPCHK(c, launch_tilt(a, mode, c->cap, c->til.max_ent, c->stream));
  }
  return MS_OK;
}
int tilt_pass(ms_ctx* c, int mode, bool use_dir, double alpha, const double* src = nullptr,
              double* dst = nullptr, bool shape_gradient = true) {
  return tilt_pass_f(c, c->tf[0], mode, use_dir, alpha, src, dst, shape_gradient);
}
int bt_pass_f(ms_ctx* c, TiltField& f, int mode, bool use_dir, double alpha, const double* tilts,
              bool with_tilt_energy = false);
int bt_pass(ms_ctx* c, int mode, bool use_dir, double alpha, const double* tilts, bool with_tilt_energy = false) {
  return bt_pass_f(c, c->tf[0], mode, use_dir, alpha, tilts, with_tilt_energy);
}
int bt_pass_f(ms_ctx* c, TiltField& f, int mode, bool use_dir, double alpha, const double* tilts, bool with_tilt_energy) {
  if (!f.tilts) return fail(c, MS_ERR_STATE, "bending_tilt module active but its tilt field was never set");
  const bool leaflet = &f != &c->tf[0];
  if (leaflet && (!f.kappa || !f.bt_vert))
    return fail(c, MS_ERR_STATE, "bending_tilt_in/out active but ms_set_leaflet_bending was never called");
  BtArgs a;
  a.m = device_mesh(c);
  if (leaflet) {
    a.m.kappa = f.kappa;
    a.m.kc_uniform = 0;
    a.m.c0 = f.c0;
  }
  a.tile0 = c->tile0;
  a.tile1 = c->tile1;
  a.x = c->buf[MS_BUF_X];
  a.d = use_dir ? trial_dir(c) : nullptr;
  a.alpha = trial_alpha(c, alpha);
  a.tilts = tilts;
  a.bt_vert = leaflet ? f.bt_vert : c->d_bt_vert;
  a.fK = c->buf[MS_BUF_FK];
  a.fA = c->buf[MS_BUF_FA];
  a.tilt_grad = f.grad;
// ... 844 lines not shown
```

### membrane_solver_amd/csrc/ms_exec.inc

```

typedef const __attribute__((address_space(4))) unsigned char* exec_kptr;
#define MS_EXEC_FN

__device__ __forceinline__ exec_kptr exec_uniform_ptr(exec_kptr p) {
  const unsigned long long v = (unsigned long long)p;
  const unsigned int lo = (unsigned int)__builtin_amdgcn_readfirstlane((int)(unsigned int)v);
  const unsigned int hi = (unsigned int)__builtin_amdgcn_readfirstlane((int)(unsigned int)(v >> 32));
  return (exec_kptr)(((unsigned long long)hi << 32) | lo);
}
template <int SKIP, typename A>
__device__ __forceinline__ void exec_load(A& dst, exec_kptr src) {
  static_assert(SKIP % 8 == 0 && sizeof(A) % 8 == 0, "8-byte granules");
  typedef const __attribute__((address_space(4))) unsigned long long* q8;
  unsigned long long w[(sizeof(A) - SKIP) / 8];
#pragma unroll
  for (int i = 0; i < (int)((sizeof(A) - SKIP) / 8); ++i) w[i] = ((q8)src)[i];
  __builtin_memcpy(reinterpret_cast<char*>(&dst) + SKIP, w, sizeof(A) - SKIP);
}
__device__ __forceinline__ int exec_uniform(int v) { return __builtin_amdgcn_readfirstlane(v); }

static_assert(offsetof(EnergyArgs, m) == 0 && offsetof(GradientArgs, m) == 0 && offsetof(TiltArgs, m) == 0 &&
                  offsetof(BtArgs, m) == 0 && offsetof(TsArgs, m) == 0,
              "the tile kernels' argument structs start with their DeviceMesh");
static_assert(sizeof(DeviceMesh) % 8 == 0, "DeviceMesh is a whole number of 8-byte granules");
// ... 123 lines not shown

__device__ __forceinline__ void exec_run_one(exec_kptr base, int off, double* lds) {
  unsigned long long* const stamps = reinterpret_cast<unsigned long long*>(
      *(const __attribute__((address_space(4))) unsigned long long*)(base + offsetof(ExecPackHead, stamps)));
  if (stamps == nullptr) {
    exec_dispatch(base, off, lds);
    return;
  }
  const unsigned long long t0 = __builtin_amdgcn_s_memrealtime();
  exec_dispatch(base, off, lds);
  __syncthreads();
  const unsigned long long t1 = __builtin_amdgcn_s_memrealtime();
  if (threadIdx.x == 0) {
    ExecCmdHead h;
    exec_load<0>(h, base + off);
    const unsigned long long idx = atomicAdd(stamps, 1ull);
    if (idx + 1 < (unsigned long long)EXEC_STAMP_CAP) {
      stamps[1 + 2 * idx] = ((unsigned long long)h.kind << 32) | (unsigned int)(h.mode & 0xffff) | ((unsigned long long)(h.inst & 0xffu) << 16);
      stamps[2 + 2 * idx] = t1 - t0;
    }
  }
}
__device__ __forceinline__ void exec_run_list(exec_kptr base, int off, int n, double* lds) {
  for (int i = 0; i < n; ++i) {
    exec_run_one(base, off, lds);
    off += (int)((const __attribute__((address_space(4))) unsigned short*)(base + off))[1];
  }
}

__device__ __noinline__ void exec_relax(exec_kptr base_v, int off_v, double* lds) {
  const exec_kptr base = exec_uniform_ptr(base_v);
  const int off = exec_uniform(off_v);
  ExecRelaxHead r;
  ExecCmdHead h;
  exec_plain_args(r, h, base, off);
  int par = 0, iters = 0, evals = 0;
  auto energy = [&]() {
    double e = 0.0;
#pragma unroll
    for (int k = 0; k < 16; ++k)
      if (k < r.n_e) e += ld_agent(r.scal + r.e_slot[k]);
    return e;
  };
  double gnorm = 0.0, rz = 0.0, E0 = 0.0;
  auto grad_at = [&](double& rz_out) {
    exec_run_list(base, par ? r.off_grad[1] : r.off_grad[0], par ? r.n_grad[1] : r.n_grad[0], lds);
    ++evals;
    E0 = energy();
    double g2 = 0.0, z = 0.0;
    g2 += ld_agent(r.scal + r.s_gn2[0]);
    z += ld_agent(r.scal + r.s_rz[0]);
    if (r.nf > 1) {
      g2 += ld_agent(r.scal + r.s_gn2[1]);
      z += ld_agent(r.scal + r.s_rz[1]);
    }
    gnorm = sqrt(g2);
    rz_out = z;
  };
  auto search = [&](double sign) {
    double step = r.step_size;
    for (int bt = 0; bt < 12; ++bt) {
      if (threadIdx.x == 0) st_agent(r.cells, sign * step);
      __syncthreads();
      exec_run_list(base, par ? r.off_trial[1] : r.off_trial[0], par ? r.n_trial[1] : r.n_trial[0], lds);
      ++evals;
      const double E1 = energy();
      if (E1 <= E0) {
        par ^= 1;
        return true;
      }
      step *= 0.5;
      if (step < 1e-16) break;
    }
    return false;
  };
  const double tol = r.tol > 0.0 ? r.tol : 0.0;
  auto small = [&]() { return gnorm == 0.0 || (tol > 0.0 && gnorm < tol); };
  if (r.solver == 0) {
    for (int it = 0; it < r.max_iters; ++it) {
      grad_at(rz);
      if (small()) break;
      const bool acc = search(-1.0);
      ++iters;
      if (!acc) break;
    }
  } else {
    double rz_old = 0.0;
    grad_at(rz_old);
    if (!small()) {
      exec_run_list(base, r.off_dir0, r.n_dir0, lds);
      for (int it = 0; it < r.max_iters; ++it) {
        if (small()) break;
        const bool acc = search(1.0);
        ++iters;
        if (!acc) break;
        double rz_new = 0.0;
        grad_at(rz_new);
        if (small()) break;
        if (rz_old == 0.0) break;
        const double beta = rz_new / rz_old;
        if (threadIdx.x == 0) st_agent(r.cells + 1, beta);
        __syncthreads();
        exec_run_list(base, r.off_dir1, r.n_dir1, lds);
        rz_old = rz_new;
      }
    }
  }
  if (threadIdx.x == 0 && r.host_box != nullptr) {
    post_entry(r.host_box, 0, (unsigned long long)iters, r.ticket);
    post_entry(r.host_box, 1, (unsigned long long)evals, r.ticket);
    post_entry(r.host_box, 2, (unsigned long long)par, r.ticket);
    post_entry(r.host_box, 3, 1ull, r.ticket);
  }
  __syncthreads();
}

#include "ms_relax_fused.inc"

template <int NB>
struct ExecPackArg {
  unsigned char b[NB];
};
template <int NB>
__global__ __launch_bounds__(256) void k_exec(ExecPackArg<NB> pack) {
  extern __shared__ double lds[];
  (void)pack;
  const exec_kptr base = (exec_kptr)__builtin_amdgcn_kernarg_segment_ptr();
  typedef const __attribute__((address_space(4))) int* qi;
  const int n = ((qi)base)[0];
  int off = (int)sizeof(ExecPackHead);
  for (int i = 0; i < n; ++i) {
    ExecCmdHead h;
    exec_load<0>(h, base + off);
    if (h.kind == CK_RELAX) {
      exec_relax(base, off, lds);
      off += h.pad;
    } else if (h.kind == CK_RELAX_FUSED) {
      exec_relax_fused(base, off, lds);
      off += (int)h.bytes;
    } else {
      exec_run_one(base, off, lds);
      off += (int)h.bytes;
    }
  }
}

namespace {
constexpr int EXEC_SLOTS = 32;
std::atomic<ExecRecorder*> g_exec_slots[EXEC_SLOTS];
std::atomic<int> g_exec_count{0};
bool same_mesh(const DeviceMesh& a, const DeviceMesh& b) {
  return a.nv == b.nv && a.T == b.T && a.n_tiles == b.n_tiles && a.own == b.own && a.has_boundary == b.has_boundary &&
         a.tile_facet_off == b.tile_facet_off && a.tile_facets == b.tile_facets && a.tile_facets32 == b.tile_facets32 &&
         a.no_fast == b.no_fast && a.tf_gamma == b.tf_gamma && a.gamma_uniform == b.gamma_uniform &&
         a.kc_uniform == b.kc_uniform && a.gamma_const == b.gamma_const && a.kappa_const == b.kappa_const &&
         a.c0_const == b.c0_const && a.tile_halo_off == b.tile_halo_off && a.halo_ids == b.halo_ids &&
         a.tile_ent_off == b.tile_ent_off && a.tile_voff == b.tile_voff && a.vent == b.vent && a.vflags == b.vflags &&
         a.kappa == b.kappa && a.c0 == b.c0;
}
}

ExecRecorder* exec_find(hipStream_t s) {
  if (g_exec_count.load(std::memory_order_acquire) == 0) return nullptr;
  for (int i = 0; i < EXEC_SLOTS; ++i) {
    ExecRecorder* r = g_exec_slots[i].load(std::memory_order_acquire);
    if (r != nullptr && r->stream == s) return r;
  }
  return nullptr;
}
void exec_attach(ExecRecorder* r) {
  for (int i = 0; i < EXEC_SLOTS; ++i) {
    ExecRecorder* expected = nullptr;
    if (g_exec_slots[i].compare_exchange_strong(expected, r)) {
      g_exec_count.fetch_add(1, std::memory_order_release);
      return;
    }
  }
}
void exec_detach(ExecRecorder* r) {
  for (int i = 0; i < EXEC_SLOTS; ++i) {
    ExecRecorder* expected = r;
    if (g_exec_slots[i].compare_exchange_strong(expected, nullptr)) g_exec_count.fetch_sub(1, std::memory_order_release);
  }
}

hipError_t ExecRecorder::push(uint16_t kind, int mode, int cap, int max_ent, int grid, uint32_t inst, size_t lds_bytes,
                              const void* args, size_t bytes, const DeviceMesh* mesh) {
  const size_t skip = mesh ? sizeof(DeviceMesh) : 0;
  const size_t rec = sizeof(ExecCmdHead) + ((bytes - skip + 7) & ~(size_t)7);
  if (sizeof(ExecPackHead) + rec > (size_t)EXEC_PACK_BYTES) return hipErrorInvalidValue;
  if (kind == CK_ENERGY && !EnergyInst::from_code(inst).in_exec()) return hipErrorInvalidValue;
  if (kind == CK_GRADIENT && !GradientInst::from_code(inst).in_exec()) return hipErrorInvalidValue;
  const size_t limit = capture ? (size_t)EXEC_PACK_BIG : (size_t)EXEC_PACK_BYTES;
  for (int attempt = 0; attempt < 2; ++attempt) {
    if (buf.empty()) {
      buf.assign(sizeof(ExecPackHead), 0);
      n_mesh = 0;
      lds = 0;
    }
    int mi = -1;
    ExecPackHead* ph = reinterpret_cast<ExecPackHead*>(buf.data());
    if (mesh) {
      for (int k = 0; k < n_mesh && mi < 0; ++k)
        if (same_mesh(ph->m[k], *mesh)) mi = k;
      if (mi < 0 && n_mesh < EXEC_MESHES) {
        mi = n_mesh++;
        ph->m[mi] = *mesh;
      }
    } else {
      mi = 0;
    }
    if (mi >= 0 && buf.size() + rec <= limit) {
      ExecCmdHead h;
      memset(&h, 0, sizeof(h));
      h.kind = kind;
      h.bytes = (uint16_t)rec;
      h.mode = mode;
      h.cap = cap;
      h.max_ent = max_ent;
      h.grid = grid;
      h.inst = inst;
      h.mesh = mi;
      const size_t at = buf.size();
      buf.resize(at + rec, 0);
      memcpy(buf.data() + at, &h, sizeof(h));
      memcpy(buf.data() + at + sizeof(h), static_cast<const unsigned char*>(args) + skip, bytes - skip);
      ph = reinterpret_cast<ExecPackHead*>(buf.data());
      ph->n_cmds += 1;
      lds = std::max(lds, lds_bytes);
      ++cmds;
      return hipSuccess;
    }
    if (capture) return hipErrorInvalidValue;
    const hipError_t e = flush();
    if (e != hipSuccess) return e;
  }
  return hipErrorInvalidValue;
}

hipError_t ExecRecorder::flush() {
  if (capture || buf.empty()) return hipSuccess;
  ExecPackHead* ph = reinterpret_cast<ExecPackHead*>(buf.data());
  if (ph->n_cmds == 0) {
    buf.clear();
    return hipSuccess;
  }
  std::vector<unsigned char> pack;
  pack.swap(buf);
  return launch_pack(pack, lds);
}

namespace {
template <int NB>
hipError_t exec_launch_n(const std::vector<unsigned char>& pack, size_t need, int T, hipStream_t stream) {
  static ExecPackArg<NB> arg;
  static std::mutex mu;
  std::lock_guard<std::mutex> lock(mu);
  memcpy(arg.b, pack.data(), pack.size());
  static size_t lds_allowed = 48 * 1024;
  if (need > lds_allowed) {
    const size_t want = std::max(need, (size_t)152 * 1024);
    hipError_t e = ensure_lds(k_exec<NB>, want);
    if (e != hipSuccess) {
      (void)hipGetLastError();
      e = ensure_lds(k_exec<NB>, need);
      if (e != hipSuccess) return e;
      lds_allowed = need;
    } else {
      lds_allowed = want;
    }
  }
  hipLaunchKernelGGL((k_exec<NB>), dim3(1), dim3(T), need, stream, arg);
  return hipGetLastError();
}
}

namespace {
struct ExecHostTiming {
  bool on = getenv("MS_EXEC_TIMING") != nullptr && atoi(getenv("MS_EXEC_TIMING")) != 0;
  double sum_us = 0.0, max_us = 0.0;
  long n = 0;
  ~ExecHostTiming() {
    if (on && n > 0)
      fprintf(stderr, "[ms exec timing] %ld k_exec launches: %.2f us of host time per launch on average (max %.1f)\n", n,
              sum_us / n, max_us);
  }
} g_exec_timing;
}

hipError_t ExecRecorder::launch_pack(const std::vector<unsigned char>& pack_in, size_t lds_bytes) {
  struct timespec ts0;
  if (g_exec_timing.on) clock_gettime(CLOCK_MONOTONIC, &ts0);
  struct Lap {
    const struct timespec* t0;
    ~Lap() {
      if (!g_exec_timing.on) return;
      struct timespec t1;
      clock_gettime(CLOCK_MONOTONIC, &t1);
      const double us = 1e6 * (double)(t1.tv_sec - t0->tv_sec) + 1e-3 * (double)(t1.tv_nsec - t0->tv_nsec);
      g_exec_timing.sum_us += us;
      g_exec_timing.max_us = std::max(g_exec_timing.max_us, us);
      ++g_exec_timing.n;
    }
  } lap{&ts0};
  std::vector<unsigned char> pack = pack_in;
  ExecPackHead* ph = reinterpret_cast<ExecPackHead*>(pack.data());
// ... 20 lines not shown
```

### membrane_solver_amd/csrc/ms_internal.h

```cpp
#pragma once

#include <hip/hip_runtime.h>

#include <cstdint>
#include <cstdlib>
#include <string>
#include <vector>

#include "membrane_hip.h"

namespace ms {

inline const char* variant_env(const char* name) {
#ifdef MS_VARIANT_ENV
  return getenv(name);
#else
  (void)name;
  return nullptr;
#endif
}

struct TileFacet {
  uint16_t l0, l1, l2;
  uint16_t flags;
};
static_assert(sizeof(TileFacet) == 8, "TileFacet must be 8 bytes");

constexpr uint16_t TF_OWNER = 1;
constexpr uint16_t TF_BODY = 2;

constexpr int MS_MAX_TRIALS = 8;
constexpr int MS_P_RAN = MS_NSCAL;
constexpr int MS_NPART = MS_NSCAL + 1;
constexpr int MS_MB_DEC = MS_NSCAL;
constexpr int MS_MB_WORDS = MS_NSCAL + 1;
constexpr int MS_DEC_STRIDE = 64;
enum : uint32_t {
  DEC_NONE = 0,
  DEC_CONTINUE = 1,
  DEC_ACCEPT_MAIN = 2,
  DEC_ACCEPT_SIDE = 3,
  DEC_GO = 4,
  DEC_STOP = 5,
  DEC_ERR_RAN = 0x100
};

constexpr uint8_t VF_FIXED = 1;
constexpr uint8_t VF_BOUNDARY = 2;
constexpr uint8_t VF_TILT_FIXED = 4;
constexpr uint8_t VF_TILT_FIXED_IN = 8;
constexpr uint8_t VF_TILT_FIXED_OUT = 16;

struct Tiling {
  int nv = 0, nf = 0, T = 256;
  int own = 256;
  int n_tiles = 0;
  int n_tiles_padded = 0;
  int tiles_per_shard = 0;
  int64_t nvp = 0;
  std::vector<int32_t> perm;
  std::vector<int32_t> iperm;
  std::vector<int32_t> tile_facet_off;
  std::vector<TileFacet> tile_facets;
  std::vector<int32_t> tile_facet_ext;
  std::vector<int32_t> tile_halo_off;
  std::vector<int32_t> halo_ids;
  std::vector<int32_t> tile_ent_off;
  std::vector<uint16_t> tile_voff;
  std::vector<uint16_t> vent;
  int max_ent = 0;
  int max_halo = 0;
  int max_tile_facets = 0;
  int64_t dropped_facets = 0;
};

int build_tiling(int nv, int nf, const double* positions, const int32_t* tri,
                 const uint8_t* body_facets, int T, int shard_count, Tiling& out,
                 std::string& err);

struct DeviceMesh {
  int nv, T, n_tiles;
  int own;
  int has_boundary;
  const int32_t* tile_facet_off;
  const TileFacet* tile_facets;
  const uint32_t* tile_facets32;
  int no_fast;
  const double* tf_gamma;
  int gamma_uniform, kc_uniform;
  double gamma_const, kappa_const, c0_const;
  const int32_t* tile_halo_off;
  const int32_t* halo_ids;
  const int32_t* tile_ent_off;
  const uint16_t* tile_voff;
  const uint16_t* vent;
  const uint8_t* vflags;
  const double* kappa;
  const double* c0;
};

struct EnergyArgs {
  DeviceMesh m;
  int tile0, tile1;
  const double* x;
  const double* d;
  double alpha;
  double* xt;
  double* fK;
  double* fA;
  double* partials;
  int bending_model;
  uint32_t modules;
  double* bt_vert;
  const uint32_t* gate;
  uint32_t gate_want;
  const double* bt_normals;
  double* bt_vert2 = nullptr;
  const double* kappa2 = nullptr;
  const double* c02 = nullptr;
  int atomic;
  int pair;
  double alpha_side[MS_MAX_TRIALS - 1];
  double* partials_side[MS_MAX_TRIALS - 1];
  double* xt_side[2];
  double* fK_side[2];
  double* fA_side[2];
};

struct GradientArgs {
  DeviceMesh m;
  int tile0, tile1;
  const double* x;
  const double* fK;
  const double* fA;
  double* g;
  double* gC;
  double* partials;
  const double* scal;
  uint32_t modules;
  int bending_grad_mode;
  double volume_stiffness, target_volume;
  double area_stiffness, target_area;
  int accumulate;
  int dir_mode;
  double* d;
  const double* pg;
  const double* pd;
  const uint32_t* gate;
  uint32_t gate_want;
  int pd_neg_pg;
  int atomic;
  const double* bt_vert;
  const double* tilts;
  double div_sign;
};

struct TiltArgs {
  DeviceMesh m;
  int tile0, tile1;
  const double* x;
  const double* d;
  double alpha;
  const double* tilts;
  double* tilts_out;
  double k_tilt;
  double* g;
  double* tilt_grad;
  double* minv;
  double* partials;
  int e_slot;
  int consistent;
  int tg_accumulate;
  int cons_tilt_grad;
  double* va_out;
  double* fields;
  int64_t fields_rows;
  double* proj_out = nullptr;
  int finish_minv = 0;
  int fixed_bit = 0;
  const double* fld_in[2] = {nullptr, nullptr};
  double* fld_out[2] = {nullptr, nullptr};
  const double* tilts_b = nullptr;
  double* proj_out_b = nullptr;
  double* minv_b = nullptr;
  double* va_out_b = nullptr;
  double k_tilt_b = 0.0;
  int finish_minv_b = 0;
  int fixed_bit_b = 0;
};

struct DiskTargetArgs {
  int tile0, tile1, nv, T, n_tiles;
  const uint8_t* vflags;
  const uint8_t* disk;
  const double* x;
  const double* d;
  double alpha;
  const double* tilts;
  double* diff;
  double* target;
  double theta_b, lambda, radius;
  double center[3], normal[3];
  const double* scal;
  double* partials;
  int r_slot;
};
hipError_t launch_disk_target(const DiskTargetArgs& a, int mode, hipStream_t s);

struct BtArgs {
  DeviceMesh m;
  int tile0, tile1;
  const double* x;
  const double* d;
  double alpha;
  const double* tilts;
  const double* bt_vert;
  double* fK;
  double* fA;
  double* tilt_grad;
  double* partials;
  double* g;
  double div_sign;
  int e_slot;
  double k_tilt_fused;
  int e_tilt_slot;
};

struct TsArgs {
  DeviceMesh m;
  int tile0, tile1;
  const double* x;
  const double* d;
  double alpha;
  const double* tilts;
  double k_smooth;
  double* tilt_grad;
  double* diag;
  double* partials;
  int e_slot;
// ... 449 lines not shown
```

### membrane_solver_amd/csrc/ms_kernels.hip

```cpp
#include <hip/hip_runtime.h>
#include <atomic>
#include <cstddef>
#include <cstdio>
#include <cstdlib>
#include <cstring>
#include <ctime>
#include <mutex>
#include <type_traits>

#include "ms_internal.h"

#ifndef MS_RSQRT_NORM
#define MS_RSQRT_NORM 1
#endif

namespace ms {

struct V3 {
  double x, y, z;
};
__device__ __forceinline__ V3 mk(double x, double y, double z) { return V3{x, y, z}; }
__device__ __forceinline__ V3 operator-(V3 a, V3 b) { return mk(a.x - b.x, a.y - b.y, a.z - b.z); }
__device__ __forceinline__ V3 operator+(V3 a, V3 b) { return mk(a.x + b.x, a.y + b.y, a.z + b.z); }
__device__ __forceinline__ V3 operator-(V3 a) { return mk(-a.x, -a.y, -a.z); }
// ... 202 lines not shown
#if MS_GATE_PROBE
__device__ unsigned long long g_probe[32];
__device__ double g_shadow[MS_NSCAL];
#endif

__device__ __forceinline__ bool gate_open(const uint32_t* word, uint32_t want, double* ran_cell) {
  const bool run = ld_agent(word) == want;
  if (threadIdx.x == 0 && ran_cell) *ran_cell = run ? 1.0 : 0.0;
  return run;
}

__device__ __forceinline__ void norm_and_inverse(double n2, double& nrm, double& inv) {
  double rs = 0.0;
  if (n2 > 1.0e-30) {
    rs = __builtin_amdgcn_rsq(n2);
    const double hn = 0.5 * n2;
    rs = rs * fma(-hn, rs * rs, 1.5);
    rs = rs * fma(-hn, rs * rs, 1.5);
  }
  nrm = n2 * rs;
  inv = rs;
}

__device__ __forceinline__ V3 lds_v3(const double* base, int cap, int slot) {
  return mk(base[slot], base[cap + slot], base[2 * cap + slot]);
}
__device__ __forceinline__ V3 lds_row3(const double* rows, int slot) {
  const double* r = rows + 3 * slot;
  return mk(r[0], r[1], r[2]);
}
__device__ __forceinline__ void lds_put3(double* rows, int slot, double x, double y, double z) {
  double* r = rows + 3 * slot;
  r[0] = x;
  r[1] = y;
  r[2] = z;
}

template <bool PACKED>
struct FacetRec {
  TileFacet v;
};
template <>
struct FacetRec<true> {
  uint32_t v;
};
template <bool PACKED>
__device__ __forceinline__ FacetRec<PACKED> facet_load(const DeviceMesh& m, size_t i) {
  FacetRec<PACKED> r;
  if constexpr (PACKED) r.v = m.tile_facets32[i];
  else r.v = m.tile_facets[i];
  return r;
}
template <bool PACKED>
__device__ __forceinline__ FacetRec<PACKED> facet_null() {
  FacetRec<PACKED> r;
  if constexpr (PACKED) r.v = 0u;
  else r.v = TileFacet{0, 0, 0, 0};
  return r;
}
template <bool PACKED>
__device__ __forceinline__ TileFacet facet_unpack(const FacetRec<PACKED>& r) {
  if constexpr (PACKED) {
    TileFacet f;
    f.l0 = (uint16_t)(r.v & 1023u);
    f.l1 = (uint16_t)((r.v >> 10) & 1023u);
    f.l2 = (uint16_t)((r.v >> 20) & 1023u);
    f.flags = (uint16_t)(r.v >> 30);
    return f;
  } else {
    return r.v;
  }
}

struct TileCtx {
  int tile, v_lo, n_owned, h0, nh, f0, f1, e0, n_ent;
};
__device__ __forceinline__ TileCtx tile_ctx(const DeviceMesh& m, int tile) {
  TileCtx t;
  t.tile = tile;
  t.v_lo = tile * m.own;
  t.n_owned = min(m.own, m.nv - t.v_lo);
  t.h0 = m.tile_halo_off[tile];
  t.nh = m.tile_halo_off[tile + 1] - t.h0;
  t.f0 = m.tile_facet_off[tile];
  t.f1 = m.tile_facet_off[tile + 1];
#ifdef MS_ABL_CLAMP
  t.f1 = min(t.f1, t.f0 + MS_ABL_CLAMP);
#endif
  t.e0 = m.tile_ent_off[tile];
  t.n_ent = m.tile_ent_off[tile + 1] - t.e0;
  return t;
}

#ifndef MS_WPE_ENERGY
#define MS_WPE_ENERGY
#endif
#ifndef MS_WPE_GRADIENT
#define MS_WPE_GRADIENT
#endif
#ifndef MS_KA_SLOTS
#define MS_KA_SLOTS 5
#endif
#ifndef MS_LEAN_SLOTS
#define MS_LEAN_SLOTS 5
#endif
constexpr int CSR_REGS = 12;
struct CsrStage {
  uint16_t vo0, vo1;
  uint16_t e[CSR_REGS];
};
__device__ __forceinline__ void csr_issue(CsrStage& r, const DeviceMesh& m, const TileCtx& t, int T,
                                          int tid) {
  const uint16_t* gv = m.tile_voff + (size_t)t.tile * (T + 1);
  r.vo0 = gv[tid];
  r.vo1 = gv[tid + 1];
  const uint16_t* ge = m.vent + t.e0;
#pragma unroll
  for (int k = 0; k < CSR_REGS; ++k) {
    const int j = tid + k * T;
    r.e[k] = j < t.n_ent ? ge[j] : (uint16_t)0;
  }
}
__device__ __forceinline__ void csr_commit(const CsrStage& r, const DeviceMesh& m, const TileCtx& t,
                                           int T, int tid, uint16_t* vent) {
#pragma unroll
  for (int k = 0; k < CSR_REGS; ++k) {
    const int j = tid + k * T;
    if (j < t.n_ent) vent[j] = r.e[k];
  }
  const uint16_t* ge = m.vent + t.e0;
  for (int j = tid + CSR_REGS * T; j < t.n_ent; j += T) vent[j] = ge[j];
}

#ifndef MS_STAMPS
#define MS_STAMPS 0
#endif
#if MS_STAMPS
__device__ unsigned long long g_stamps[8 * 16384];
#define MS_STAMP(k)                                                                   \
  do {                                                                                \
    if (threadIdx.x == 0) g_stamps[8 * (size_t)blk + (k)] = __builtin_amdgcn_s_memrealtime(); \
  } while (0)
#define MS_STAMP_ID()                                                                                  \
  do {                                                                                                 \
    if (threadIdx.x == 0) {                                                                            \
      g_stamps[8 * (size_t)blk + 4] = __builtin_amdgcn_s_getreg((20 << 0) | (0 << 6) | (31 << 11));  \
      g_stamps[8 * (size_t)blk + 5] = __builtin_amdgcn_s_getreg((4 << 0) | (0 << 6) | (31 << 11));    \
    }                                                                                                  \
  } while (0)
#else
#define MS_STAMP(k) do {} while (0)
#define MS_STAMP_ID() do {} while (0)
#endif
template <bool BEND, bool GUARD, int TT, int CAPC, bool ATOMIC, int MULTI = 0, bool AREA = false>
__device__ __forceinline__ void energy_body(EnergyArgs& a, int cap_rt, int max_ent, double* lds, int block_id) {
  int bid = block_id;
  double* const ran_row = a.partials + (size_t)MS_P_RAN * a.m.n_tiles;
  bool last_trial = true;
  if (MULTI) {
    const int nm = MULTI == 8 ? a.pair : MULTI;
    const int k = bid % NXCD, j2 = bid / NXCD;
    const int st = j2 % nm;
    bid = (j2 / nm) * NXCD + k;
    if (bid >= a.tile1 - a.tile0) return;
    if (st != 0) {
      last_trial = false;
      a.xt = a.fK = a.fA = nullptr;
#pragma unroll
      for (int j = 0; j < MS_MAX_TRIALS - 1; ++j)
        if (j < (MULTI == 8 ? MS_MAX_TRIALS - 1 : MULTI - 1) && st - 1 == j) {
          a.alpha = a.alpha_side[j];
          a.partials = a.partials_side[j];
          if (j < 2) {
            a.xt = a.xt_side[j];
            a.fK = a.fK_side[j];
            a.fA = a.fA_side[j];
          }
        }
    }
  }
  const int T = TT ? TT : a.m.T;
  const int cap = CAPC ? CAPC : cap_rt;
  double* px = lds;
  double* ox = px + 3 * cap;
  double* stg = ox + (GUARD ? 3 * cap : 0);
  double* red = stg;
  uint16_t* vent = reinterpret_cast<uint16_t*>(stg + (BEND ? (ATOMIC ? 5 : 9) * T : 6 * 16));
  uint8_t* lfl = reinterpret_cast<uint8_t*>(vent + ((BEND && !ATOMIC) ? ((max_ent + 3) & ~3) : 0));
  const bool stage_flags = a.m.has_boundary || GUARD;
  const int my_tile = a.tile0 + xcd_tile(bid, a.tile1 - a.tile0);
  if (a.gate != nullptr && !gate_open(a.gate, a.gate_want, last_trial ? ran_row + my_tile : nullptr)) return;

  const int blk = bid;
  (void)blk;
  MS_STAMP(0);
  MS_STAMP_ID();
  const TileCtx t = tile_ctx(a.m, my_tile);
  const int tid = threadIdx.x;
  const bool have_d = a.d != nullptr;

  constexpr bool PACKED = TT == 256;
  FacetRec<PACKED> tf_nx = facet_null<PACKED>();
  double gam_nx = 0.0;
  if (t.f0 + tid < t.f1) {
    tf_nx = facet_load<PACKED>(a.m, (size_t)(t.f0 + tid));
    gam_nx = a.m.gamma_uniform ? a.m.gamma_const : a.m.tf_gamma[t.f0 + tid];
  }

  double kappa_v = 0.0, c0_v = 0.0;
  if (BEND && tid < t.n_owned) {
    kappa_v = a.m.kc_uniform ? a.m.kappa_const : a.m.kappa[t.v_lo + tid];
    c0_v = a.m.kc_uniform ? a.m.c0_const : a.m.c0[t.v_lo + tid];
  }

  uint8_t own_fl = 0;
  int cur = 0, end = 0;
  {
    const bool own = tid < t.n_owned;
    const int v_own = t.v_lo + tid;
    const bool has_h = tid < t.nh;
    int hv = 0;
    if (has_h) hv = a.m.halo_ids[t.h0 + tid];
    double xo0 = 0, xo1 = 0, xo2 = 0, dd0 = 0, dd1 = 0, dd2 = 0;
    uint8_t fl = 0;
    if (own) {
      const size_t g = 3 * (size_t)v_own;
      fl = a.m.vflags[v_own];
      xo0 = a.x[g];
      xo1 = a.x[g + 1];
      xo2 = a.x[g + 2];
      if (have_d) {
        dd0 = a.d[g];
        dd1 = a.d[g + 1];
        dd2 = a.d[g + 2];
      }
    }
    CsrStage cs;
    if (BEND && !ATOMIC) csr_issue(cs, a.m, t, T, tid);
    if (BEND && ATOMIC) {
      for (int j = tid; j < 5 * T; j += T) stg[j] = 0.0;
    }
    own_fl = fl;
    double h0 = 0, h1 = 0, h2 = 0, e0 = 0, e1 = 0, e2 = 0;
    uint8_t hfl = 0;
    if (has_h) {
      const size_t g = 3 * (size_t)hv;
      hfl = a.m.vflags[hv];
      h0 = a.x[g];
      h1 = a.x[g + 1];
      h2 = a.x[g + 2];
      if (have_d) {
        e0 = a.d[g];
        e1 = a.d[g + 1];
        e2 = a.d[g + 2];
      }
    }
    if (own) {
      const size_t g = 3 * (size_t)v_own;
      const bool mv = have_d && !(fl & VF_FIXED);
      const double x0 = mv ? axpy1(xo0, a.alpha, dd0) : xo0;
      const double x1 = mv ? axpy1(xo1, a.alpha, dd1) : xo1;
      const double x2 = mv ? axpy1(xo2, a.alpha, dd2) : xo2;
      if (stage_flags) lfl[tid] = fl;
      lds_put3(px, tid, x0, x1, x2);
      if (GUARD) lds_put3(ox, tid, xo0, xo1, xo2);
      if (a.xt) {
        a.xt[g] = x0;
        a.xt[g + 1] = x1;
        a.xt[g + 2] = x2;
      }
    }
    if (BEND && !ATOMIC) {
      csr_commit(cs, a.m, t, T, tid, vent);
      cur = cs.vo0;
      end = cs.vo1;
    }
    if (has_h) {
      const int s = t.n_owned + tid;
      const bool mv = have_d && !(hfl & VF_FIXED);
      if (stage_flags) lfl[s] = hfl;
      lds_put3(px, s, mv ? axpy1(h0, a.alpha, e0) : h0, mv ? axpy1(h1, a.alpha, e1) : h1, mv ? axpy1(h2, a.alpha, e2) : h2);
      if (GUARD) lds_put3(ox, s, h0, h1, h2);
    }
    for (int h = tid + T; h < t.nh; h += T) {
      const int v = a.m.halo_ids[t.h0 + h];
      const size_t g = 3 * (size_t)v;
      const uint8_t f2 = a.m.vflags[v];
      const double q0 = a.x[g], q1 = a.x[g + 1], q2 = a.x[g + 2];
      double r0 = 0, r1 = 0, r2 = 0;
      if (have_d) {
        r0 = a.d[g];
        r1 = a.d[g + 1];
        r2 = a.d[g + 2];
      }
      const int s = t.n_owned + h;
      const bool mv = have_d && !(f2 & VF_FIXED);
      if (stage_flags) lfl[s] = f2;
      lds_put3(px, s, mv ? axpy1(q0, a.alpha, r0) : q0, mv ? axpy1(q1, a.alpha, r1) : q1, mv ? axpy1(q2, a.alpha, r2) : q2);
      if (GUARD) lds_put3(ox, s, q0, q1, q2);
    }
  }
  __syncthreads();
  MS_STAMP(1);

  double e_surf = 0.0, vol = 0.0, min_e2 = 1.0e300, guard = 0.0;
  const bool want_surf = a.modules & MS_MOD_SURFACE;
  const bool want_vol = a.modules & (MS_MOD_VOLUME_PENALTY | MS_CON_VOLUME | MS_TRACK_VOLUME);
  constexpr bool want_area = AREA;
  double area = 0.0;
  double aKx = 0, aKy = 0, aKz = 0, aAv = 0, aAe = 0;
  if (!(BEND && tid < t.n_owned)) cur = end = 0;
  const int ent_begin = cur;

  for (int c0 = t.f0; c0 < t.f1; c0 += T) {
    const int p = c0 + tid;
    const TileFacet tf = facet_unpack<PACKED>(tf_nx);
    const double gam = gam_nx;
    if (p + T < t.f1) {
      tf_nx = facet_load<PACKED>(a.m, (size_t)(p + T));
      gam_nx = a.m.gamma_uniform ? a.m.gamma_const : a.m.tf_gamma[p + T];
    }
    double va0 = 0, va1 = 0, va2 = 0, ve0 = 0, ve1 = 0, ve2 = 0;
    if (p < t.f1) {
      const bool owner = tf.flags & TF_OWNER;
      if (BEND || owner) {
        const V3 v0 = lds_row3(px, tf.l0), v1 = lds_row3(px, tf.l1), v2 = lds_row3(px, tf.l2);
        const V3 e0 = v2 - v1, e1 = v0 - v2, e2 = v1 - v0;
        const double l0 = dot(e0, e0), l1 = dot(e1, e1), l2 = dot(e2, e2);
        const V3 n = cross(e2, -e1);
#if MS_RSQRT_NORM
        double A2, inv_A2;
        norm_and_inverse(dot(n, n), A2, inv_A2);
#else
        const double A2 = norm(n);
#endif
        if (owner) {
          if (want_surf && A2 >= 1.0e-12) e_surf += gam * (0.5 * A2);
          if (want_vol && (tf.flags & TF_BODY)) vol += dot(cross(v1, v2), v0);
          if (want_area && (tf.flags & TF_BODY) && A2 >= 1.0e-12) area += 0.5 * A2;
          min_e2 = min_plain(min_e2, min_plain(l0, min_plain(l1, l2)));
          if (GUARD) {
            const V3 o0 = lds_row3(ox, tf.l0), o1 = lds_row3(ox, tf.l1), o2 = lds_row3(ox, tf.l2);
            const V3 no = cross(o1 - o0, o2 - o0);
            const double nno = norm(no);
            if (nno > 1.0e-12) {
              if (A2 < 1.0e-12) {
                guard = 1.0;
              } else {
                double dd = dot(no, n) / (nno * A2);
                dd = fmin(1.0, fmax(-1.0, dd));
                if (!(acos(dd) <= 0.5)) guard = 1.0;
              }
            }
          }
        }
        if (BEND) {
          const double ad = A2 < 1.0e-12 ? 1.0e-12 : A2;
#if MS_RSQRT_NORM
          const double inv_ad = A2 < 1.0e-12 ? 1.0e12 : inv_A2;
#else
          const double inv_ad = 1.0 / ad;
#endif
          const double tri_area = 0.5 * ad;
          const double c0 = dot(-e1, e2) * inv_ad, c1 = dot(-e2, e0) * inv_ad, c2 = dot(-e0, e1) * inv_ad;
          corner_areas(c0, c1, c2, l0, l1, l2, tri_area, va0, va1, va2);
          ve0 = va0;
          ve1 = va1;
          ve2 = va2;
          const double ta_eff = fmax(0.5 * A2, 1.0e-12);
          if (ta_eff != tri_area) corner_areas(c0, c1, c2, l0, l1, l2, ta_eff, ve0, ve1, ve2);
          if (a.m.has_boundary) {
            const int b0 = (lfl[tf.l0] & VF_BOUNDARY) ? 1 : 0;
            const int b1 = (lfl[tf.l1] & VF_BOUNDARY) ? 1 : 0;
            const int b2 = (lfl[tf.l2] & VF_BOUNDARY) ? 1 : 0;
            const int n_int = 3 - (b0 + b1 + b2);
            if (n_int > 0 && n_int < 3) {
              const double b_sum = ve0 * b0 + ve1 * b1 + ve2 * b2;
              const double extra = b_sum / (double)n_int;
              const double m0 = b0 ? 0.0 : 1.0, m1 = b1 ? 0.0 : 1.0, m2 = b2 ? 0.0 : 1.0;
              ve0 = ve0 * m0 + m0 * extra;
              ve1 = ve1 * m1 + m1 * extra;
              ve2 = ve2 * m2 + m2 * extra;
            }
          }
          const double hc0 = 0.5 * c0, hc1 = 0.5 * c1, hc2 = 0.5 * c2;
          const V3 K0 = hc2 * e2 - hc1 * e1;
          const V3 K1 = hc0 * e0 - hc2 * e2;
          const V3 K2 = mk(-K0.x - K1.x, -K0.y - K1.y, -K0.z - K1.z);
          if (ATOMIC) {
            const int no = t.n_owned;
            if (tf.l0 < no) {
              atomicAdd(&stg[tf.l0], K0.x); atomicAdd(&stg[T + tf.l0], K0.y); atomicAdd(&stg[2 * T + tf.l0], K0.z);
              atomicAdd(&stg[3 * T + tf.l0], va0);
              if (ve0 != va0) atomicAdd(&stg[4 * T + tf.l0], ve0 - va0);
            }
            if (tf.l1 < no) {
              atomicAdd(&stg[tf.l1], K1.x); atomicAdd(&stg[T + tf.l1], K1.y); atomicAdd(&stg[2 * T + tf.l1], K1.z);
              atomicAdd(&stg[3 * T + tf.l1], va1);
              if (ve1 != va1) atomicAdd(&stg[4 * T + tf.l1], ve1 - va1);
            }
            if (tf.l2 < no) {
              atomicAdd(&stg[tf.l2], K2.x); atomicAdd(&stg[T + tf.l2], K2.y); atomicAdd(&stg[2 * T + tf.l2], K2.z);
              atomicAdd(&stg[3 * T + tf.l2], va2);
              if (ve2 != va2) atomicAdd(&stg[4 * T + tf.l2], ve2 - va2);
            }
          } else {
            double* s = stg + tid;
            s[0 * T] = K0.x; s[1 * T] = K0.y; s[2 * T] = K0.z;
            s[3 * T] = K1.x; s[4 * T] = K1.y; s[5 * T] = K1.z;
            s[6 * T] = K2.x; s[7 * T] = K2.y; s[8 * T] = K2.z;
          }
        }
      }
    }
    if (BEND && !ATOMIC) {
      const int lo = c0 - t.f0, hi = min(c0 + T, t.f1) - t.f0;
      __syncthreads();
      const int cur0 = cur;
      while (cur < end) {
        const int ent = vent[cur];
        const int fl = ent >> 2;
        if (fl >= hi) break;
        const double* s = stg + (fl - lo) + 3 * (ent & 3) * T;
        aKx += s[0];
        aKy += s[T];
        aKz += s[2 * T];
        ++cur;
      }
      __syncthreads();
      if (p < t.f1) {
        double* s = stg + tid;
        s[0 * T] = va0; s[1 * T] = va1; s[2 * T] = va2;
        s[3 * T] = ve0; s[4 * T] = ve1; s[5 * T] = ve2;
      }
      __syncthreads();
      for (int q = cur0; q < cur; ++q) {
        const int ent = vent[q];
        const double* s = stg + ((ent >> 2) - lo) + (ent & 3) * T;
        aAv += s[0];
        aAe += s[3 * T];
      }
      __syncthreads();
    }
  }

  if (BEND && ATOMIC) {
    __syncthreads();
    MS_STAMP(2);
    if (tid < t.n_owned) {
      aKx = stg[tid];
      aKy = stg[T + tid];
      aKz = stg[2 * T + tid];
      aAv = stg[3 * T + tid];
      aAe = aAv + stg[4 * T + tid];
    }
    __syncthreads();
  }
  double e_bend = 0.0;
  if (BEND && tid < t.n_owned) {
    const int v = t.v_lo + tid;
    const V3 K = mk(aKx, aKy, aKz);
    const double kappa = kappa_v, c0 = c0_v;
    const bool interior = !(own_fl & VF_BOUNDARY);
    const double safe = fmax(aAv, 1.0e-12);
    double k_mag, inv_k_mag;
    norm_and_inverse(dot(K, K), k_mag, inv_k_mag);
    const double inv_safe = 1.0 / safe;
    double H = k_mag * (0.5 * inv_safe);
    const bool signed_h = a.bt_normals != nullptr;
    V3 nh = mk(0, 0, 0);
    if (signed_h) {
      nh = mk(a.bt_normals[3 * (size_t)v], a.bt_normals[3 * (size_t)v + 1], a.bt_normals[3 * (size_t)v + 2]);
      H = dot(K, nh) * (0.5 * inv_safe);
    }
    const double ratio = safe > 1.0e-15 ? aAe * inv_safe : 0.0;
    double scale_K, fe, fv;
    if (a.bt_vert) {
      double base = (2.0 * H) - c0;
      if (!interior) base = 0.0;
      scale_K = kappa * ratio;
      fe = fv = 0.0;
      double* rec = a.bt_vert + 4 * (size_t)v;
      rec[0] = base;
      rec[1] = aAe;
      rec[2] = kappa * ratio * H;
      rec[3] = 0.0;
      if (a.bt_vert2 != nullptr) {
        const double kappa_b = a.kappa2[v], c0_b = a.c02[v];
        double base_b = (2.0 * H) - c0_b;
        if (!interior) base_b = 0.0;
        double* rec_b = a.bt_vert2 + 4 * (size_t)v;
        rec_b[0] = base_b;
        rec_b[1] = aAe;
        rec_b[2] = kappa_b * ratio * H;
        rec_b[3] = 0.0;
      }
    } else if (a.bending_model == MS_BEND_HELFRICH) {
      double term = (2.0 * H) - c0;
      if (!interior) term = 0.0;
      e_bend = 0.5 * (kappa * (term * term) * aAe);
      scale_K = kappa * term * ratio;
      fe = 0.5 * kappa * (term * term);
      fv = -2.0 * kappa * term * ratio * H;
    } else {
      const double He = interior ? H : 0.0;
      e_bend = kappa * (He * He) * aAe;
      scale_K = kappa * He * ratio;
      fe = kappa * (He * He);
      fv = -2.0 * kappa * (He * He) * ratio;
    }
#ifndef MS_ABL_KA
#define MS_ABL_KA 0
#endif
    if (a.fK) {
      V3 Kd;
      if (signed_h) {
        Kd = nh;
      } else if ((MS_ABL_KA & 2) || k_mag > 1.0e-15) {
        const double inv_k = (MS_ABL_KA & 2) ? 1.0 / k_mag : inv_k_mag;
        Kd = mk(K.x * inv_k, K.y * inv_k, K.z * inv_k);
      } else {
#if MS_STAMPS
        atomicAdd(&g_stamps[8 * 16384 - 1], 1ull);
#endif
        V3 N = mk(0, 0, 0);
        int qb = ent_begin, qe = end;
        const uint16_t* ve = vent;
        if (ATOMIC) {
          const uint16_t* gv = a.m.tile_voff + (size_t)t.tile * (T + 1);
          qb = gv[tid];
          qe = gv[tid + 1];
          ve = a.m.vent + t.e0;
        }
        for (int q = qb; q < qe; ++q) {
          const TileFacet f = a.m.tile_facets[t.f0 + (ve[q] >> 2)];
          const V3 q0 = lds_row3(px, f.l0), q1 = lds_row3(px, f.l1), q2 = lds_row3(px, f.l2);
          N = N + cross(q1 - q0, q2 - q0);
        }
        const double nn = norm(N);
        Kd = nn > 1.0e-15 ? mk(N.x / nn, N.y / nn, N.z / nn) : N;
      }
#if (MS_ABL_KA & 1)
      e_bend += 1e-300 * (Kd.x * scale_K + Kd.y * scale_K + Kd.z * scale_K + fe + fv);
#else
      a.fK[3 * (size_t)v] = Kd.x * scale_K;
      a.fK[3 * (size_t)v + 1] = Kd.y * scale_K;
      a.fK[3 * (size_t)v + 2] = Kd.z * scale_K;
      a.fA[2 * (size_t)v] = fe;
      a.fA[2 * (size_t)v + 1] = fv;
#endif
    }
  }

  double* pout = a.partials + t.tile;
  const size_t pstride = (size_t)a.m.n_tiles;
  if (want_area) {
    const double vals[6] = {e_surf, vol, e_bend, min_e2, guard, area};
    const int ops[6] = {0, 0, 0, 1, 2, 0};
    const int slots[6] = {MS_S_ESURF, MS_S_VOL, MS_S_EBEND, MS_S_MINEDGE2, MS_S_GUARD, MS_S_AREA};
    block_reduce_store<6>(vals, ops, slots, red, pout, pstride);
  } else if (GUARD || want_vol) {
    const double vals[5] = {e_surf, vol, e_bend, min_e2, guard};
    const int ops[5] = {0, 0, 0, 1, 2};
    const int slots[5] = {MS_S_ESURF, MS_S_VOL, MS_S_EBEND, MS_S_MINEDGE2, MS_S_GUARD};
    block_reduce_store<5>(vals, ops, slots, red, pout, pstride);
  } else {
    const double vals[3] = {e_surf, e_bend, min_e2};
    const int ops[3] = {0, 0, 1};
    const int slots[3] = {MS_S_ESURF, MS_S_EBEND, MS_S_MINEDGE2};
    if constexpr (MS_REDUCE_STAGED && ATOMIC && BEND && !GUARD && !AREA && TT == 256)
      block_reduce_store_staged<3>(vals, ops, slots, stg, pout, pstride);
    else
      block_reduce_store<3>(vals, ops, slots, red, pout, pstride);
    if (tid == 0) {
      pout[MS_S_VOL * pstride] = 0.0;
      pout[MS_S_GUARD * pstride] = 0.0;
    }
  }
#if MS_STAMPS
  asm volatile("s_waitcnt vmcnt(0)" ::: "memory");
  MS_STAMP(3);
#endif
}

template <bool BEND, bool GUARD, int TT, int CAPC, bool ATOMIC, int MULTI = 0>
__global__ __launch_bounds__(TT ? TT : 512, (TT == 256 && BEND && !GUARD && ATOMIC) ? MS_KA_SLOTS : 1) MS_WPE_ENERGY void k_energy(EnergyArgs a, int cap_rt, int max_ent) {
  extern __shared__ double lds[];
  energy_body<BEND, GUARD, TT, CAPC, ATOMIC, MULTI>(a, cap_rt, max_ent, lds, (int)blockIdx.x);
}

static size_t u16_bytes(int T, int max_ent) { return 2 * ((size_t)((max_ent + 3) & ~3)); }

size_t energy_lds_bytes(int T, int cap, int max_ent, bool bend, bool guard, bool flags, bool atomic) {
  size_t d = 3 * (size_t)cap + (guard ? 3 * (size_t)cap : 0) + (bend ? (atomic ? 5 : 9) * (size_t)T : 6 * 16);
  return d * sizeof(double) + ((bend && !atomic) ? u16_bytes(T, max_ent) : 0) +
         ((flags || guard) ? (((size_t)cap + 15) / 16) * 16 : 0);
}

static bool no_lean() {
  static int v = -1;
  if (v < 0) {
    const char* e = getenv("MS_NO_LEAN");
    v = (e && atoi(e) != 0) ? 1 : 0;
  }
  return v != 0;
}

template <bool BEND, bool GUARD, int TT, int CAPC, bool ATOMIC>
__global__ __launch_bounds__(TT ? TT : 512, (TT == 256 && BEND && !GUARD && ATOMIC) ? MS_KA_SLOTS : 1) MS_WPE_ENERGY void k_energy_area(EnergyArgs a, int cap_rt, int max_ent) {
  extern __shared__ double lds[];
  energy_body<BEND, GUARD, TT, CAPC, ATOMIC, 0, true>(a, cap_rt, max_ent, lds, (int)blockIdx.x);
}

template <typename K>
static hipError_t ensure_lds(K kernel, size_t lds) {
  if (lds <= 48 * 1024) return hipSuccess;
  return hipFuncSetAttribute(reinterpret_cast<const void*>(kernel),
                             hipFuncAttributeMaxDynamicSharedMemorySize, (int)lds);
}

template <typename K, typename... Args>
static hipError_t launch(K kernel, int grid, int block, size_t lds, hipStream_t s, const Args&... args) {
  if (const hipError_t e = ensure_lds(kernel, lds); e != hipSuccess) return e;
  hipLaunchKernelGGL(kernel, dim3(grid), dim3(block), lds, s, args...);
  return hipGetLastError();
}

template <typename F>
__host__ __device__ __forceinline__ auto pick(bool v, F&& f) {
  if (v) return f(std::true_type{});
  return f(std::false_type{});
}
template <int V0, int... Vs, typename F>
__host__ __device__ __forceinline__ auto pick_int(int v, F&& f) {
  if constexpr (sizeof...(Vs) == 0) {
    return f(std::integral_constant<int, V0>{});
  } else {
    if (v == V0) return f(std::integral_constant<int, V0>{});
    return pick_int<Vs...>(v, f);
  }
}

constexpr int FAST_T = 256;
constexpr int FAST_CAP = 0;

static int abl_ntiles() {
#ifdef MS_ABL_NTILES_ENV
  static const int v = getenv("MS_ABL_NTILES") ? atoi(getenv("MS_ABL_NTILES")) : 0;
  return v;
#else
  return 0;
#endif
}

template <bool BEND, bool GUARD, bool ATOMIC, bool AREA, bool FAST, int MULTI>
struct EnergyTag {
  static constexpr EnergyInst d{BEND, GUARD, ATOMIC, AREA, FAST, MULTI};
};
template <int MODE, bool VOLROW, bool ATOMIC, bool LEAN, bool AREA, bool FAST>
struct GradientTag {
  static constexpr GradientInst d{MODE, VOLROW, ATOMIC, LEAN, AREA, FAST};
};
template <bool EXEC, typename I, typename F>
__host__ __device__ __forceinline__ bool visit_tag(F&& f) {
  if constexpr (EXEC ? I::d.in_exec() : I::d.valid()) {
    f(I{});
    return true;
  } else {
    return false;
  }
}
template <bool EXEC, typename F>
__host__ __device__ __forceinline__ bool visit_instance(const EnergyInst& d, F&& f) {
  if (!(EXEC ? d.in_exec() : d.valid())) return false;
  return pick(d.bend, [&](auto B) {
    return pick(d.guard, [&](auto G) {
      return pick(d.atomic, [&](auto AT) {
        return pick(d.area, [&](auto AR) {
          return pick(d.fast, [&](auto FA) {
            return pick_int<0, 2, 3, 8>(d.multi, [&](auto NM) {
              return visit_tag<EXEC, EnergyTag<decltype(B)::value, decltype(G)::value, decltype(AT)::value,
                                               decltype(AR)::value, decltype(FA)::value, decltype(NM)::value>>(f);
            });
          });
        });
      });
    });
  });
}
template <bool EXEC, typename F>
__host__ __device__ __forceinline__ bool visit_instance(const GradientInst& d, F&& f) {
  if (!(EXEC ? d.in_exec() : d.valid())) return false;
  return pick_int<0, 1, 2, 3>(d.mode, [&](auto M) {
    return pick(d.volrow, [&](auto V) {
      return pick(d.atomic, [&](auto AT) {
        return pick(d.lean, [&](auto LE) {
          return pick(d.area, [&](auto AR) {
            return pick(d.fast, [&](auto FA) {
              return visit_tag<EXEC, GradientTag<decltype(M)::value, decltype(V)::value, decltype(AT)::value,
                                                 decltype(LE)::value, decltype(AR)::value, decltype(FA)::value>>(f);
            });
          });
        });
      });
    });
  });
}

EnergyInst energy_instance(const EnergyArgs& a, bool guard) {
  const bool bend = (a.modules & (MS_MOD_BENDING | MS_MOD_BENDING_TILT)) != 0;
  const bool fast = a.m.T == FAST_T && a.m.tile_facets32 != nullptr && !a.m.no_fast;
  const bool atomic = a.atomic != 0 && bend;
  const bool area = (a.modules & MS_MOD_AREA_PENALTY) != 0;
  const int multi = !a.pair ? 0 : ((a.pair < 2 || a.pair > MS_MAX_TRIALS) ? -1 : (a.pair == 2 ? 2 : (a.pair == 3 ? 3 : 8)));
  return {bend, guard, atomic, area, fast, multi};
}

hipError_t launch_energy(const EnergyArgs& a_in, bool guard, int cap, int max_ent, hipStream_t s) {
  EnergyArgs a = a_in;
  if (abl_ntiles() > 0) a.tile1 = std::min(a.tile1, a.tile0 + abl_ntiles());
  const int nb = a.tile1 - a.tile0;
  if (nb <= 0) return hipSuccess;
  const EnergyInst d = energy_instance(a, guard);
  if (!d.valid()) return hipErrorInvalidValue;
  static const size_t lds_min = variant_env("MS_KA_LDS_MIN") ? (size_t)atol(variant_env("MS_KA_LDS_MIN")) : 0;
  const size_t lds = std::max(lds_min, energy_lds_bytes(a.m.T, cap, max_ent, d.bend, guard, a.m.has_boundary != 0, d.atomic));
  if (ExecRecorder* r = exec_find(s)) {
    if (d.in_exec()) return r->push(CK_ENERGY, 0, cap, max_ent, nb, d.code(), lds, &a, sizeof(a), &a.m);
    if (const hipError_t e = r->flush(); e != hipSuccess) return e;
  }
  const int grid = d.multi ? a.pair * NXCD * ((nb + NXCD - 1) / NXCD) : nb;
  hipError_t e = hipErrorInvalidValue;
  visit_instance<false>(d, [&](auto tag) {
    using I = decltype(tag);
    constexpr int TT = I::d.fast ? FAST_T : 0, CC = I::d.fast ? FAST_CAP : 0;
    if constexpr (I::d.area)
      e = launch(k_energy_area<I::d.bend, I::d.guard, TT, CC, I::d.atomic>, grid, a.m.T, lds, s, a, cap, max_ent);
    else
      e = launch(k_energy<I::d.bend, I::d.guard, TT, CC, I::d.atomic, I::d.multi>, grid, a.m.T, lds, s, a, cap, max_ent);
  });
  return e;
}

#ifndef MS_SCHED_FENCES
#define MS_SCHED_FENCES 1
#endif
#if MS_SCHED_FENCES
#define MS_SCHED_FENCE()                 \
  do {                                   \
    asm volatile("" ::: "memory");       \
    __builtin_amdgcn_sched_barrier(0);   \
  } while (0)
#else
#define MS_SCHED_FENCE() do {} while (0)
#endif
#ifndef MS_ABL_NOATOM
#define MS_ABL_NOATOM 0
#endif
#ifndef MS_ABL_NOMATH
#define MS_ABL_NOMATH 0
#endif
#ifndef MS_ABL_NOGATHER
#define MS_ABL_NOGATHER 0
#endif
#ifndef MS_ABL_NOLOOP
#define MS_ABL_NOLOOP 0
#endif
#ifndef MS_ABL_NOSTORE
#define MS_ABL_NOSTORE 0
#endif
#ifndef MS_ABL_NOHIST
#define MS_ABL_NOHIST 0
#endif
template <int BENDMODE, bool VOLROW, int TT, int CAPC, bool ATOMIC, bool LEAN = false, bool AREA = false>
__device__ __forceinline__ void gradient_body(const GradientArgs& a, int cap_rt, int max_ent, double* lds, int block_id) {
  constexpr bool BEND = BENDMODE != 0;
  constexpr bool LEAF = BENDMODE == 3;
  constexpr bool ANALYTIC = BENDMODE == 1 || BENDMODE == 3;
  const int T = TT ? TT : a.m.T;
  const int cap = CAPC ? CAPC : cap_rt;
  double* px = lds;
  double* fk = px + 3 * cap;
  double* fa = fk + (BEND ? 3 * cap : 0);
  double* kp = fa + (BEND ? 2 * cap : 0);
  double* tl = kp + (LEAF ? cap : 0);
  double* stg = tl + (LEAF ? 3 * cap : 0);
  constexpr int NACC = VOLROW ? 6 : 3;
  double* red = stg + (ATOMIC ? NACC : (VOLROW ? 18 : 9)) * T;
  uint16_t* vent = reinterpret_cast<uint16_t*>(red + 4 * 16);
  uint8_t* lfl = reinterpret_cast<uint8_t*>(vent + (ATOMIC ? 0 : ((max_ent + 3) & ~3)));
  const int my_tile = a.tile0 + xcd_tile(block_id, a.tile1 - a.tile0);
#if MS_GATE_PROBE
  if (a.gate != nullptr) {
    const double truth = ld_agent(a.scal + MS_S_EBEND);
    const double via_scalar = g_shadow[MS_S_EBEND];
    const double via_vector = *reinterpret_cast<const volatile double*>(g_shadow + MS_S_EBEND + (threadIdx.x >> 12));
    if (threadIdx.x == 0) {
      const unsigned xcc = __builtin_amdgcn_s_getreg((20 << 0) | (0 << 6) | (3 << 11)) & 7u;
      atomicAdd(&g_probe[0], 1ull);
      if (via_scalar != truth) {
        atomicAdd(&g_probe[1], 1ull);
        atomicAdd(&g_probe[8 + xcc], 1ull);
      }
      if (via_vector != truth) {
        atomicAdd(&g_probe[2], 1ull);
        atomicAdd(&g_probe[16 + xcc], 1ull);
      }
      if (block_id == 0) atomicAdd(&g_probe[3], 1ull);
    }
  }
#endif
  if (a.gate != nullptr && !gate_open(a.gate, a.gate_want, a.partials + (size_t)MS_P_RAN * a.m.n_tiles + my_tile)) return;

  const int blk = block_id;
  (void)blk;
  MS_STAMP(0);
  MS_STAMP_ID();
  const TileCtx t = tile_ctx(a.m, my_tile);
  const int tid = threadIdx.x;

  constexpr bool PACKED = TT == 256;
  FacetRec<PACKED> tf_nx = facet_null<PACKED>();
  double gam_nx = 0.0;
  if (t.f0 + tid < t.f1) {
    tf_nx = facet_load<PACKED>(a.m, (size_t)(t.f0 + tid));
    gam_nx = a.m.gamma_uniform ? a.m.gamma_const : a.m.tf_gamma[t.f0 + tid];
  }

  int cur = 0, end = 0;
  {
    const bool own = tid < t.n_owned;
    const int v_own = t.v_lo + tid;
    const bool has_h = tid < t.nh;
    int hv = 0;
    if (has_h) hv = a.m.halo_ids[t.h0 + tid];
    double x0 = 0, x1 = 0, x2 = 0, k0 = 0, k1 = 0, k2 = 0, ae = 0, av = 0;
    double okp = 0, ot0 = 0, ot1 = 0, ot2 = 0, hkp = 0, ht0 = 0, ht1 = 0, ht2 = 0;
    uint8_t fl = 0;
    if (own) {
      const size_t g = 3 * (size_t)v_own;
      fl = a.m.vflags[v_own];
      x0 = a.x[g];
      x1 = a.x[g + 1];
      x2 = a.x[g + 2];
      if (BEND) {
        k0 = a.fK[g];
        k1 = a.fK[g + 1];
        k2 = a.fK[g + 2];
        ae = LEAF ? a.bt_vert[4 * (size_t)v_own] : a.fA[2 * (size_t)v_own];
        av = a.fA[2 * (size_t)v_own + 1];
      }
      if (LEAF) {
        okp = a.m.kappa[v_own];
        ot0 = a.tilts[g];
        ot1 = a.tilts[g + 1];
        ot2 = a.tilts[g + 2];
      }
    }
    CsrStage cs;
    if (!ATOMIC) csr_issue(cs, a.m, t, T, tid);
    if (ATOMIC) {
      for (int j = tid; j < NACC * T; j += T) stg[j] = 0.0;
    }
    double hx0 = 0, hx1 = 0, hx2 = 0, hk0 = 0, hk1 = 0, hk2 = 0, hae = 0, hav = 0;
    uint8_t hfl = 0;
    if (has_h) {
      const size_t g = 3 * (size_t)hv;
      if (!LEAN) hfl = a.m.vflags[hv];
      hx0 = a.x[g];
      hx1 = a.x[g + 1];
      hx2 = a.x[g + 2];
      if (BEND) {
        hk0 = a.fK[g];
        hk1 = a.fK[g + 1];
        hk2 = a.fK[g + 2];
        hae = LEAF ? a.bt_vert[4 * (size_t)hv] : a.fA[2 * (size_t)hv];
        hav = a.fA[2 * (size_t)hv + 1];
      }
      if (LEAF) {
        hkp = a.m.kappa[hv];
        ht0 = a.tilts[g];
        ht1 = a.tilts[g + 1];
        ht2 = a.tilts[g + 2];
      }
    }
    if (own) {
      lfl[tid] = fl;
      lds_put3(px, tid, x0, x1, x2);
      if (BEND) {
        lds_put3(fk, tid, k0, k1, k2);
        if (LEAN) {
          fa[tid] = ae + av;
        } else {
          fa[2 * tid] = ae;
          fa[2 * tid + 1] = av;
        }
      }
      if (LEAF) {
        kp[tid] = okp;
        tl[tid] = ot0;
        tl[cap + tid] = ot1;
        tl[2 * cap + tid] = ot2;
      }
    }
    if (!ATOMIC) {
      csr_commit(cs, a.m, t, T, tid, vent);
      cur = cs.vo0;
      end = cs.vo1;
// ... 2223 lines not shown
```

### membrane_solver_amd/csrc/ms_tiles.cpp

```cpp
#include <algorithm>
#include <cstdlib>
#include <cmath>
#include <cstring>
#include <numeric>

#include "ms_internal.h"

namespace ms {

namespace {

inline uint64_t hilbert3(uint32_t x, uint32_t y, uint32_t z, int bits) {
  uint32_t X[3] = {x, y, z};
  const uint32_t M = 1u << (bits - 1);
  for (uint32_t Q = M; Q > 1; Q >>= 1) {
    uint32_t P = Q - 1;
    for (int i = 0; i < 3; ++i) {
      if (X[i] & Q) {
        X[0] ^= P;
      } else {
        uint32_t t = (X[0] ^ X[i]) & P;
        X[0] ^= t;
        X[i] ^= t;
      }
    }
  }
  for (int i = 1; i < 3; ++i) X[i] ^= X[i - 1];
  uint32_t t = 0;
  for (uint32_t Q = M; Q > 1; Q >>= 1)
    if (X[2] & Q) t ^= Q - 1;
  for (int i = 0; i < 3; ++i) X[i] ^= t;
  uint64_t h = 0;
  for (int b = bits - 1; b >= 0; --b)
    for (int i = 0; i < 3; ++i) h = (h << 1) | ((X[i] >> b) & 1u);
  return h;
}

}

int build_tiling(int nv, int nf, const double* positions, const int32_t* tri,
                 const uint8_t* body_facets, int T, int shard_count, Tiling& out,
                 std::string& err) {
  if (nv <= 0 || nf < 0 || !positions || (nf > 0 && !tri)) {
    err = "ms_create: nv must be > 0 and positions/tri non-null";
    return MS_ERR_INVALID;
  }
  if (T <= 0) T = 256;
  int R = T;
  if (T > 128 && T < 256) T = 256;
  if (!(T == 64 || T == 128 || T == 256 || T == 512)) {
    err = "ms_create: tile_vertices must be 64, 128, 129..256 or 512 (one thread per owned vertex)";
    return MS_ERR_INVALID;
  }
  if (shard_count < 1) shard_count = 1;
  out = Tiling();
  out.nv = nv;
  out.nf = nf;
  out.T = T;
  out.own = R;

  double lo[3] = {positions[0], positions[1], positions[2]};
  double hi[3] = {lo[0], lo[1], lo[2]};
  for (int i = 0; i < nv; ++i)
    for (int d = 0; d < 3; ++d) {
      double p = positions[3 * (size_t)i + d];
      if (!(p == p)) {
        err = "ms_create: NaN in positions";
        return MS_ERR_INVALID;
      }
      lo[d] = std::min(lo[d], p);
      hi[d] = std::max(hi[d], p);
    }
  double span = std::max({hi[0] - lo[0], hi[1] - lo[1], hi[2] - lo[2], 1e-300});
  const int bits = 21;
  const double scale = (double)((1u << bits) - 1) / span;
  std::vector<uint64_t> key(nv);
  for (int i = 0; i < nv; ++i) {
    uint32_t q[3];
    for (int d = 0; d < 3; ++d) {
      double v = (positions[3 * (size_t)i + d] - lo[d]) * scale;
      q[d] = (uint32_t)std::min(std::max(v, 0.0), (double)((1u << bits) - 1));
    }
    key[i] = hilbert3(q[0], q[1], q[2], bits);
  }
  out.perm.resize(nv);
  std::iota(out.perm.begin(), out.perm.end(), 0);
  const int tile_order = variant_env("MS_TILE_ORDER") ? atoi(variant_env("MS_TILE_ORDER")) : 1;
  if (tile_order == 0) {
    std::stable_sort(out.perm.begin(), out.perm.end(),
                     [&](int32_t a, int32_t b) { return key[a] < key[b]; });
  } else {
    struct Range { int lo, hi; };
    std::vector<Range> stack;
    stack.push_back({0, nv});
    while (!stack.empty()) {
      const Range r = stack.back();
      stack.pop_back();
      const int n = r.hi - r.lo;
      const int tiles = (n + R - 1) / R;
      if (tiles <= 1) {
        std::sort(out.perm.begin() + r.lo, out.perm.begin() + r.hi,
                  [&](int32_t a, int32_t b) { return key[a] < key[b] || (key[a] == key[b] && a < b); });
        continue;
      }
      double blo[3] = {1e300, 1e300, 1e300}, bhi[3] = {-1e300, -1e300, -1e300};
      for (int i = r.lo; i < r.hi; ++i)
        for (int d = 0; d < 3; ++d) {
          const double p = positions[3 * (size_t)out.perm[i] + d];
          blo[d] = std::min(blo[d], p);
          bhi[d] = std::max(bhi[d], p);
        }
      int ax = 0;
      for (int d = 1; d < 3; ++d)
        if (bhi[d] - blo[d] > bhi[ax] - blo[ax]) ax = d;
      const int mid = r.lo + (tiles / 2) * R;
      std::nth_element(out.perm.begin() + r.lo, out.perm.begin() + mid, out.perm.begin() + r.hi,
                       [&](int32_t a, int32_t b) {
                         const double pa = positions[3 * (size_t)a + ax], pb = positions[3 * (size_t)b + ax];
                         return pa < pb || (pa == pb && a < b);
                       });
      stack.push_back({mid, r.hi});
      stack.push_back({r.lo, mid});
    }
  }
  out.iperm.resize(nv);
  for (int i = 0; i < nv; ++i) out.iperm[out.perm[i]] = i;

  out.n_tiles = (nv + R - 1) / R;
  out.tiles_per_shard = (out.n_tiles + shard_count - 1) / shard_count;
  out.n_tiles_padded = out.tiles_per_shard * shard_count;
  out.nvp = (int64_t)out.n_tiles_padded * R;

  std::vector<int32_t> cnt(out.n_tiles + 1, 0);
  auto tiles_of = [&](int f, int tl[3], int iv[3]) -> int {
    for (int k = 0; k < 3; ++k) {
      int e = tri[3 * (size_t)f + k];
      if (e < 0 || e >= nv) return -1;
      iv[k] = out.iperm[e];
    }
    int n = 0;
    for (int k = 0; k < 3; ++k) {
      int t = iv[k] / R;
      bool dup = false;
      for (int j = 0; j < n; ++j) dup |= (tl[j] == t);
      if (!dup) tl[n++] = t;
    }
    return n;
  };
  for (int f = 0; f < nf; ++f) {
    int tl[3], iv[3];
    int n = tiles_of(f, tl, iv);
    if (n < 0) {
      ++out.dropped_facets;
      continue;
    }
    for (int j = 0; j < n; ++j) ++cnt[tl[j] + 1];
  }
  out.tile_facet_off.assign(out.n_tiles + 1, 0);
  for (int t = 0; t < out.n_tiles; ++t) out.tile_facet_off[t + 1] = out.tile_facet_off[t] + cnt[t + 1];
  const size_t n_inst = (size_t)out.tile_facet_off[out.n_tiles];
  out.tile_facets.resize(n_inst);
  out.tile_facet_ext.resize(n_inst);
  std::vector<int32_t> cursor(out.tile_facet_off.begin(), out.tile_facet_off.end() - 1);
  std::vector<int32_t> inst_v(3 * n_inst);
  std::vector<int32_t> forder(nf);
  std::iota(forder.begin(), forder.end(), 0);
  {
    std::vector<int32_t> fkey(nf);
    for (int f = 0; f < nf; ++f) {
      int e = tri[3 * (size_t)f];
      fkey[f] = (e >= 0 && e < nv) ? out.iperm[e] : 0;
    }
    std::stable_sort(forder.begin(), forder.end(),
                     [&](int32_t a, int32_t b) { return fkey[a] < fkey[b]; });
  }
  for (int fi = 0; fi < nf; ++fi) {
    int f = forder[fi];
    int tl[3], iv[3];
    int n = tiles_of(f, tl, iv);
    if (n < 0) continue;
    int owner_tile = iv[0] / R;
    for (int j = 0; j < n; ++j) {
      size_t p = (size_t)cursor[tl[j]]++;
      inst_v[3 * p] = iv[0];
      inst_v[3 * p + 1] = iv[1];
      inst_v[3 * p + 2] = iv[2];
      uint16_t fl = 0;
      if (tl[j] == owner_tile) fl |= TF_OWNER;
      if (!body_facets || body_facets[f]) fl |= TF_BODY;
      out.tile_facets[p].flags = fl;
      out.tile_facet_ext[p] = f;
    }
  }

  out.tile_halo_off.assign(out.n_tiles + 1, 0);
  out.tile_ent_off.assign(out.n_tiles + 1, 0);
  out.tile_voff.assign((size_t)out.n_tiles * (T + 1), 0);
  std::vector<int32_t> halo_tmp;
  std::vector<int32_t> vcnt(T + 1);
  const char* env_order = variant_env("MS_FACET_ORDER");
  const int order_mode = env_order ? atoi(env_order) : 2;
  const char* env_stride = getenv("MS_FACET_STRIDE");
  const int stride_mode = env_stride ? atoi(env_stride) : 1;
  std::vector<TileFacet> tf_tmp;
  std::vector<int32_t> ext_tmp;
  std::vector<int32_t> order;
  std::vector<uint8_t> taken;
  for (int t = 0; t < out.n_tiles; ++t) {
    const int v_lo = t * R;
    const int v_hi = std::min(nv, v_lo + R);
    const size_t b = (size_t)out.tile_facet_off[t], e = (size_t)out.tile_facet_off[t + 1];
    const size_t n = e - b;
    halo_tmp.clear();
    for (size_t p = b; p < e; ++p)
      for (int k = 0; k < 3; ++k) {
        int v = inst_v[3 * p + k];
        if (v < v_lo || v >= v_hi) halo_tmp.push_back(v);
      }
    std::sort(halo_tmp.begin(), halo_tmp.end());
    halo_tmp.erase(std::unique(halo_tmp.begin(), halo_tmp.end()), halo_tmp.end());
    const int n_owned = v_hi - v_lo;
    if ((size_t)n_owned + halo_tmp.size() > 65535u) {
      err = "ms_create: a vertex patch needs more than 65535 LDS slots (vertex valence too high)";
      return MS_ERR_TILE_CAPACITY;
    }
    for (size_t p = b; p < e; ++p) {
      uint16_t loc[3];
      for (int k = 0; k < 3; ++k) {
        int v = inst_v[3 * p + k];
        if (v >= v_lo && v < v_hi) {
          loc[k] = (uint16_t)(v - v_lo);
        } else {
          auto it = std::lower_bound(halo_tmp.begin(), halo_tmp.end(), v);
          loc[k] = (uint16_t)(n_owned + (int)(it - halo_tmp.begin()));
        }
      }
      out.tile_facets[p].l0 = loc[0];
      out.tile_facets[p].l1 = loc[1];
      out.tile_facets[p].l2 = loc[2];
    }

    if (n >= 128 && order_mode != 0) {
      tf_tmp.assign(out.tile_facets.begin() + b, out.tile_facets.begin() + e);
      ext_tmp.assign(out.tile_facet_ext.begin() + b, out.tile_facet_ext.begin() + e);
      order.clear();
      order.reserve(n);
      size_t S = std::max<size_t>(stride_mode > 1 ? (size_t)stride_mode : 7, (n + 63) / 64);
      while (std::gcd(S, n) != 1) ++S;
      std::vector<int32_t>& cand = order;
      for (size_t i = 0; i < n; ++i) cand.push_back((int32_t)((i * S) % n));
      if (order_mode >= 2) {
        std::vector<int32_t> seq(cand);
        taken.assign(n, 0);
        order.clear();
        size_t first_free = 0;
        while (order.size() < n) {
          uint32_t m32[3] = {0, 0, 0};
          const size_t group_end = std::min(n, order.size() + 32);
          for (int half = 0; half < 2 && order.size() < group_end; ++half) {
            uint32_t m16[3] = {0, 0, 0};
            const size_t half_end = std::min(group_end, order.size() + 16);
            while (order.size() < half_end) {
              size_t best = n;
              int best_cost = 99, seen = 0;
              for (size_t q = first_free; q < n && seen < 192; ++q) {
                if (taken[q]) continue;
                ++seen;
                const TileFacet& f = tf_tmp[seq[q]];
                const uint32_t r[3] = {f.l0, f.l1, f.l2};
                int cost = 0;
                for (int k = 0; k < 3; ++k)
                  cost += (int)((m32[k] >> (r[k] & 31)) & 1u) + (int)((m16[k] >> (r[k] & 15)) & 1u);
                if (cost < best_cost) {
                  best_cost = cost;
                  best = q;
                  if (cost == 0) break;
                }
              }
              if (best == n) break;
              const TileFacet& f = tf_tmp[seq[best]];
              const uint32_t r[3] = {f.l0, f.l1, f.l2};
              for (int k = 0; k < 3; ++k) {
                m32[k] |= 1u << (r[k] & 31);
                m16[k] |= 1u << (r[k] & 15);
              }
              taken[best] = 1;
              order.push_back(seq[best]);
              while (first_free < n && taken[first_free]) ++first_free;
            }
            while (first_free < n && taken[first_free]) ++first_free;
          }
        }
      }
      for (size_t i = 0; i < n; ++i) {
        out.tile_facets[b + i] = tf_tmp[order[i]];
        out.tile_facet_ext[b + i] = ext_tmp[order[i]];
      }
    }

    {
      if (e - b > 16383u) {
        err = "ms_create: a tile lists more than 16383 facets (vertex valence too high)";
        return MS_ERR_TILE_CAPACITY;
      }
      std::fill(vcnt.begin(), vcnt.end(), 0);
      for (size_t p = b; p < e; ++p) {
        const TileFacet& f = out.tile_facets[p];
        if (f.l0 < n_owned) ++vcnt[f.l0 + 1];
        if (f.l1 < n_owned) ++vcnt[f.l1 + 1];
        if (f.l2 < n_owned) ++vcnt[f.l2 + 1];
      }
      for (int i = 0; i < T; ++i) vcnt[i + 1] += vcnt[i];
      const int n_ent = vcnt[T];
      if (n_ent > 65535) {
        err = "ms_create: a tile has more than 65535 owned corners";
        return MS_ERR_TILE_CAPACITY;
      }
      uint16_t* voff = &out.tile_voff[(size_t)t * (T + 1)];
      for (int i = 0; i <= T; ++i) voff[i] = (uint16_t)vcnt[i];
      const size_t base = out.vent.size();
      out.vent.resize(base + n_ent);
      std::vector<int32_t> fill(vcnt.begin(), vcnt.end() - 1);
      for (size_t p = b; p < e; ++p) {
        const TileFacet& f = out.tile_facets[p];
        const uint16_t fl = (uint16_t)(p - b);
        if (f.l0 < n_owned) out.vent[base + fill[f.l0]++] = (uint16_t)(fl << 2 | 0);
        if (f.l1 < n_owned) out.vent[base + fill[f.l1]++] = (uint16_t)(fl << 2 | 1);
        if (f.l2 < n_owned) out.vent[base + fill[f.l2]++] = (uint16_t)(fl << 2 | 2);
      }
      out.tile_ent_off[t + 1] = (int32_t)out.vent.size();
      out.max_ent = std::max(out.max_ent, n_ent);
    }
    out.halo_ids.insert(out.halo_ids.end(), halo_tmp.begin(), halo_tmp.end());
    out.tile_halo_off[t + 1] = (int32_t)out.halo_ids.size();
    out.max_halo = std::max(out.max_halo, (int)halo_tmp.size());
    out.max_tile_facets = std::max(out.max_tile_facets, (int)(e - b));
  }
  return MS_OK;
}

}
```

Measured before the change: 19270.

## Pair adjacent facets into quads for the atomic bending energy kernel

At tiling time, each tile's facets are paired greedily along shared edges into quad records, packed into 64 bits with per-facet flags, and reordered to reduce LDS bank conflicts among atomic targets. The atomic bending energy path (TT=256, no guard or area) now iterates quads instead of single facets. Each thread processes two triangles that share an edge, reusing the shared-edge vertices' positions and merging their contributions before the LDS atomics. Kappa and c0 loads move after the loop, and gamma is remapped per quad instance. This cuts LDS gathers and atomics per facet at the cost of more per-thread work, possible imbalance where facets stay unpaired, and extra setup time.

```diff
diff --git a/include/membrane_hip.h b/include/membrane_hip.h
--- a/include/membrane_hip.h
+++ b/include/membrane_hip.h
@@ -338,6 +338,11 @@
 int ms_plan_tiling(int nv, int nf, const double *positions, const int32_t *tri,
                    int tile_vertices, int shard_count, int64_t stats[8],
                    int32_t *perm_out);
+int ms_plan_tiling_quads(int nv, int nf, const double *positions, const int32_t *tri,
+                         int tile_vertices, int64_t stats[4]);
+int ms_plan_tiling_quad_tile(int nv, int nf, const double *positions, const int32_t *tri,
+                             int tile_vertices, int tile, int max_records, uint64_t *records,
+                             int32_t *facets, int32_t *slot_vertex, int32_t counts[4]);
 int ms_plan_tiling_conflicts(int nv, int nf, const double *positions,
                              const int32_t *tri, int tile_vertices, double model[4]);
 
diff --git a/membrane_solver_amd/_lib.py b/membrane_solver_amd/_lib.py
--- a/membrane_solver_amd/_lib.py
+++ b/membrane_solver_amd/_lib.py
@@ -218,6 +218,9 @@
     "ms_shard_peer_set_barrier": (ctypes.c_int, [_P, _P, _P]),
     "ms_plan_tiling": (ctypes.c_int, [ctypes.c_int, ctypes.c_int, _D, _I32, ctypes.c_int, ctypes.c_int,
                                       _I64, _I32]),
+    "ms_plan_tiling_quads": (ctypes.c_int, [ctypes.c_int, ctypes.c_int, _D, _I32, ctypes.c_int, _I64]),
+    "ms_plan_tiling_quad_tile": (ctypes.c_int, [ctypes.c_int, ctypes.c_int, _D, _I32, ctypes.c_int, ctypes.c_int,
+                                                ctypes.c_int, ctypes.POINTER(ctypes.c_uint64), _I32, _I32, _I32]),
     "ms_plan_tiling_conflicts": (ctypes.c_int, [ctypes.c_int, ctypes.c_int, _D, _I32, ctypes.c_int, _D]),
     "ms_surface_energy_and_gradient_host": (ctypes.c_int, [ctypes.c_int, ctypes.c_int, _D, _I32, _D,
                                                            _D, _D]),
diff --git a/membrane_solver_amd/csrc/ms_api_context.inc b/membrane_solver_amd/csrc/ms_api_context.inc
--- a/membrane_solver_amd/csrc/ms_api_context.inc
+++ b/membrane_solver_amd/csrc/ms_api_context.inc
@@ -79,6 +79,10 @@
       packed[i] = (uint32_t)f.l0 | ((uint32_t)f.l1 << 10) | ((uint32_t)f.l2 << 20) | ((uint32_t)(f.flags & 3u) << 30);
     }
     CREATE_CHK(upload(c, &c->d_tile_facets32, packed));
+    CREATE_CHK(upload(c, &c->d_tile_quad_off, t.tile_quad_off));
+    CREATE_CHK(upload(c, &c->d_tile_quads, t.tile_quads));
+    std::vector<double> ones(2 * t.tile_quads.size(), 1.0);
+    CREATE_CHK(upload(c, &c->d_tq_gamma, ones));
   }
   CREATE_CHK(upload(c, &c->d_tile_halo_off, t.tile_halo_off));
   CREATE_CHK(upload(c, &c->d_halo_ids, t.halo_ids));
@@ -238,7 +242,8 @@
   }
   if (c->stream) (void)hipStreamSynchronize(c->stream);
   if (!c->own_state) c->state = nullptr;
-  void* ptrs[] = {c->d_perm, c->d_tile_facet_off, c->d_tile_facets, c->d_tile_facets32, c->d_tf_gamma, c->d_volgrad_cache,
+  void* ptrs[] = {c->d_perm, c->d_tile_facet_off, c->d_tile_facets, c->d_tile_facets32, c->d_tile_quad_off, c->d_tile_quads, c->d_tq_gamma, c->d_tf_gamma,
+                  c->d_volgrad_cache,
                   c->d_tile_halo_off, c->d_halo_ids, c->d_tile_ent_off, c->d_tile_voff, c->d_vent,
                   c->d_vflags, c->d_kappa, c->d_c0, c->tf[0].tilts, c->tf[0].grad, c->tf[0].trial, c->d_bt_vert, c->d_tn, c->tf[0].dir, c->tf[0].minv,
                   c->tf[1].tilts, c->tf[1].grad, c->tf[1].trial, c->tf[1].dir, c->tf[1].minv,
@@ -350,6 +355,11 @@
   for (int f = 1; f < t.nf && c->gamma_uniform; ++f) c->gamma_uniform = gamma[f] == c->gamma_const;
   if (!g.empty())
     HIPCHK(c, hipMemcpy(c->d_tf_gamma, g.data(), g.size() * sizeof(double), hipMemcpyHostToDevice));
+  if (c->d_tq_gamma && !t.tile_quad_inst.empty()) {
+    std::vector<double> q(t.tile_quad_inst.size());
+    for (size_t p = 0; p < q.size(); ++p) q[p] = t.tile_quad_inst[p] >= 0 ? g[(size_t)t.tile_quad_inst[p]] : 0.0;
+    HIPCHK(c, hipMemcpy(c->d_tq_gamma, q.data(), q.size() * sizeof(double), hipMemcpyHostToDevice));
+  }
   c->carry.carry_valid = c->carry.grad_valid = c->carry.bt_valid = c->carry.maxg2_valid = false;
   c->sh_carry_valid = c->sh_grad_valid = false;
   return MS_OK;
diff --git a/membrane_solver_amd/csrc/ms_api_ctx.inc b/membrane_solver_amd/csrc/ms_api_ctx.inc
--- a/membrane_solver_amd/csrc/ms_api_ctx.inc
+++ b/membrane_solver_amd/csrc/ms_api_ctx.inc
@@ -47,6 +47,9 @@
   int32_t* d_tile_facet_off = nullptr;
   TileFacet* d_tile_facets = nullptr;
   uint32_t* d_tile_facets32 = nullptr;
+  int32_t* d_tile_quad_off = nullptr;
+  uint64_t* d_tile_quads = nullptr;
+  double* d_tq_gamma = nullptr;
   double* d_tf_gamma = nullptr;
   double* d_volgrad_cache = nullptr;
   double volgrad_cache_norm2 = 0.0;
diff --git a/membrane_solver_amd/csrc/ms_api_misc.inc b/membrane_solver_amd/csrc/ms_api_misc.inc
--- a/membrane_solver_amd/csrc/ms_api_misc.inc
+++ b/membrane_solver_amd/csrc/ms_api_misc.inc
@@ -230,6 +230,53 @@
   stats[6] = owned_corners;
   stats[7] = (int64_t)gradient_lds_bytes(t.T, t.own + t.max_halo, t.max_ent, true, true);
   if (perm_out) memcpy(perm_out, t.perm.data(), sizeof(int32_t) * (size_t)nv);
+  return MS_OK;
+}
+
+int ms_plan_tiling_quads(int nv, int nf, const double* positions, const int32_t* tri, int tile_vertices,
+                         int64_t stats[4]) {
+  if (!stats) return fail(nullptr, MS_ERR_INVALID, "ms_plan_tiling_quads: stats is NULL");
+  Tiling t;
+  std::string err;
+  int rc = build_tiling(nv, nf, positions, tri, nullptr, tile_vertices, 1, t, err);
+  if (rc != MS_OK) return fail(nullptr, rc, err);
+  stats[0] = (int64_t)t.tile_facets.size();
+  stats[1] = t.paired_instances;
+  stats[2] = (int64_t)t.tile_quads.size();
+  stats[3] = t.max_tile_quads;
+  return MS_OK;
+}
+
+int ms_plan_tiling_quad_tile(int nv, int nf, const double* positions, const int32_t* tri, int tile_vertices, int tile,
+                             int max_records, uint64_t* records, int32_t* facets, int32_t* slot_vertex,
+                             int32_t counts[4]) {
+  if (!counts) return fail(nullptr, MS_ERR_INVALID, "ms_plan_tiling_quad_tile: counts is NULL");
+  Tiling t;
+  std::string err;
+  int rc = build_tiling(nv, nf, positions, tri, nullptr, tile_vertices, 1, t, err);
+  if (rc != MS_OK) return fail(nullptr, rc, err);
+  if (tile < 0 || tile >= t.n_tiles) return fail(nullptr, MS_ERR_INVALID, "ms_plan_tiling_quad_tile: no such tile");
+  const int v_lo = tile * t.own, n_owned = std::min(t.own, t.nv - v_lo);
+  const int h0 = t.tile_halo_off[tile], nh = t.tile_halo_off[tile + 1] - h0;
+  const bool have = !t.tile_quad_off.empty();
+  const int q0 = have ? t.tile_quad_off[tile] : 0, nq = have ? t.tile_quad_off[tile + 1] - q0 : 0;
+  counts[0] = nq;
+  counts[1] = t.tile_facet_off[tile + 1] - t.tile_facet_off[tile];
+  counts[2] = n_owned;
+  counts[3] = n_owned + nh;
+  if (nq > max_records) return fail(nullptr, MS_ERR_INVALID, "ms_plan_tiling_quad_tile: max_records is too small");
+  for (int i = 0; i < nq; ++i) {
+    if (records) records[i] = t.tile_quads[(size_t)q0 + i];
+    if (facets)
+      for (int k = 0; k < 2; ++k) {
+        const int32_t inst = t.tile_quad_inst[2 * ((size_t)q0 + i) + k];
+        facets[2 * i + k] = inst >= 0 ? t.tile_facet_ext[(size_t)inst] : -1;
+      }
+  }
+  if (slot_vertex && have) {
+    for (int i = 0; i < n_owned; ++i) slot_vertex[i] = t.perm[v_lo + i];
+    for (int i = 0; i < nh; ++i) slot_vertex[n_owned + i] = t.perm[t.halo_ids[h0 + i]];
+  }
   return MS_OK;
 }
 
diff --git a/membrane_solver_amd/csrc/ms_api_phases.inc b/membrane_solver_amd/csrc/ms_api_phases.inc
--- a/membrane_solver_amd/csrc/ms_api_phases.inc
+++ b/membrane_solver_amd/csrc/ms_api_phases.inc
@@ -60,6 +60,9 @@
   m.tile_facet_off = c->d_tile_facet_off;
   m.tile_facets = c->d_tile_facets;
   m.tile_facets32 = c->d_tile_facets32;
+  m.tile_quad_off = c->d_tile_quad_off;
+  m.tile_quads = c->d_tile_quads;
+  m.tq_gamma = c->d_tq_gamma;
   m.no_fast = c->no_fast ? 1 : 0;
   m.tf_gamma = c->d_tf_gamma;
   m.gamma_uniform = c->gamma_uniform ? 1 : 0;
diff --git a/membrane_solver_amd/csrc/ms_exec.inc b/membrane_solver_amd/csrc/ms_exec.inc
--- a/membrane_solver_amd/csrc/ms_exec.inc
+++ b/membrane_solver_amd/csrc/ms_exec.inc
@@ -299,6 +299,7 @@
 bool same_mesh(const DeviceMesh& a, const DeviceMesh& b) {
   return a.nv == b.nv && a.T == b.T && a.n_tiles == b.n_tiles && a.own == b.own && a.has_boundary == b.has_boundary &&
          a.tile_facet_off == b.tile_facet_off && a.tile_facets == b.tile_facets && a.tile_facets32 == b.tile_facets32 &&
+         a.tile_quad_off == b.tile_quad_off && a.tile_quads == b.tile_quads && a.tq_gamma == b.tq_gamma &&
          a.no_fast == b.no_fast && a.tf_gamma == b.tf_gamma && a.gamma_uniform == b.gamma_uniform &&
          a.kc_uniform == b.kc_uniform && a.gamma_const == b.gamma_const && a.kappa_const == b.kappa_const &&
          a.c0_const == b.c0_const && a.tile_halo_off == b.tile_halo_off && a.halo_ids == b.halo_ids &&
diff --git a/membrane_solver_amd/csrc/ms_internal.h b/membrane_solver_amd/csrc/ms_internal.h
--- a/membrane_solver_amd/csrc/ms_internal.h
+++ b/membrane_solver_amd/csrc/ms_internal.h
@@ -28,6 +28,13 @@
 
 constexpr uint16_t TF_OWNER = 1;
 constexpr uint16_t TF_BODY = 2;
+
+constexpr uint32_t TQ_HAS_B = 1u << 12;
+inline uint64_t quad_pack(const uint16_t s[4], uint16_t flags_a, uint16_t flags_b, bool has_b) {
+  const uint32_t lo = (uint32_t)s[0] | ((uint32_t)s[1] << 10) | ((uint32_t)s[2] << 20) | ((uint32_t)(flags_a & 3u) << 30);
+  const uint32_t hi = has_b ? ((uint32_t)s[3] | ((uint32_t)(flags_b & 3u) << 10) | TQ_HAS_B) : 0u;
+  return (uint64_t)lo | ((uint64_t)hi << 32);
+}
 
 constexpr int MS_MAX_TRIALS = 8;
 constexpr int MS_P_RAN = MS_NSCAL;
@@ -72,6 +79,11 @@
   int max_halo = 0;
   int max_tile_facets = 0;
   int64_t dropped_facets = 0;
+  std::vector<int32_t> tile_quad_off;
+  std::vector<uint64_t> tile_quads;
+  std::vector<int32_t> tile_quad_inst;
+  int max_tile_quads = 0;
+  int64_t paired_instances = 0;
 };
 
 int build_tiling(int nv, int nf, const double* positions, const int32_t* tri,
@@ -85,6 +97,9 @@
   const int32_t* tile_facet_off;
   const TileFacet* tile_facets;
   const uint32_t* tile_facets32;
+  const int32_t* tile_quad_off;
+  const uint64_t* tile_quads;
+  const double* tq_gamma;
   int no_fast;
   const double* tf_gamma;
   int gamma_uniform, kc_uniform;
diff --git a/membrane_solver_amd/csrc/ms_kernels.hip b/membrane_solver_amd/csrc/ms_kernels.hip
--- a/membrane_solver_amd/csrc/ms_kernels.hip
+++ b/membrane_solver_amd/csrc/ms_kernels.hip
@@ -378,6 +378,103 @@
 #define MS_STAMP(k) do {} while (0)
 #define MS_STAMP_ID() do {} while (0)
 #endif
+#ifndef MS_SCHED_FENCES
+#define MS_SCHED_FENCES 1
+#endif
+#if MS_SCHED_FENCES
+#define MS_SCHED_FENCE()                 \
+  do {                                   \
+    asm volatile("" ::: "memory");       \
+    __builtin_amdgcn_sched_barrier(0);   \
+  } while (0)
+#else
+#define MS_SCHED_FENCE() do {} while (0)
+#endif
+#ifndef MS_QUADS
+#define MS_QUADS 1
+#endif
+__device__ __forceinline__ uint2 quad_load(const DeviceMesh& m, size_t i) {
+  return reinterpret_cast<const uint2*>(m.tile_quads)[i];
+}
+
+struct EnergyFacetSums {
+  double e_surf = 0.0, vol = 0.0, min_e2 = 1.0e300, guard = 0.0, area = 0.0;
+};
+struct EnergyFacetTerms {
+  V3 K0, K1, K2;
+  double va0 = 0, va1 = 0, va2 = 0, ve0 = 0, ve1 = 0, ve2 = 0;
+};
+template <bool BEND, bool GUARD, bool AREA>
+__device__ __forceinline__ void energy_facet(const V3& v0, const V3& v1, const V3& v2, const V3& e2, int l0, int l1, int l2,
+                                             uint32_t flags, double gam, bool want_surf, bool want_vol, bool has_boundary,
+                                             const double* ox, const uint8_t* lfl, EnergyFacetSums& s,
+                                             EnergyFacetTerms& o) {
+  const bool owner = flags & TF_OWNER;
+  const V3 e0 = v2 - v1, e1 = v0 - v2;
+  const double l0q = dot(e0, e0), l1q = dot(e1, e1), l2q = dot(e2, e2);
+  const V3 n = cross(e2, -e1);
+#if MS_RSQRT_NORM
+  double A2, inv_A2;
+  norm_and_inverse(dot(n, n), A2, inv_A2);
+#else
+  const double A2 = norm(n);
+#endif
+  if (owner) {
+    if (want_surf && A2 >= 1.0e-12) s.e_surf += gam * (0.5 * A2);
+    if (want_vol && (flags & TF_BODY)) s.vol += dot(cross(v1, v2), v0);
+    if (AREA && (flags & TF_BODY) && A2 >= 1.0e-12) s.area += 0.5 * A2;
+    s.min_e2 = min_plain(s.min_e2, min_plain(l0q, min_plain(l1q, l2q)));
+    if (GUARD) {
+      const V3 o0 = lds_row3(ox, l0), o1 = lds_row3(ox, l1), o2 = lds_row3(ox, l2);
+      const V3 no = cross(o1 - o0, o2 - o0);
+      const double nno = norm(no);
+      if (nno > 1.0e-12) {
+        if (A2 < 1.0e-12) {
+          s.guard = 1.0;
+        } else {
+          double dd = dot(no, n) / (nno * A2);
+          dd = fmin(1.0, fmax(-1.0, dd));
+          if (!(acos(dd) <= 0.5)) s.guard = 1.0;
+        }
+      }
+    }
+  }
+  if (BEND) {
+    const double ad = A2 < 1.0e-12 ? 1.0e-12 : A2;
+#if MS_RSQRT_NORM
+    const double inv_ad = A2 < 1.0e-12 ? 1.0e12 : inv_A2;
+#else
+    const double inv_ad = 1.0 / ad;
+#endif
+    const double tri_area = 0.5 * ad;
+    const double c0 = dot(-e1, e2) * inv_ad, c1 = dot(-e2, e0) * inv_ad, c2 = dot(-e0, e1) * inv_ad;
+    corner_areas(c0, c1, c2, l0q, l1q, l2q, tri_area, o.va0, o.va1, o.va2);
+    o.ve0 = o.va0;
+    o.ve1 = o.va1;
+    o.ve2 = o.va2;
+    const double ta_eff = fmax(0.5 * A2, 1.0e-12);
+    if (ta_eff != tri_area) corner_areas(c0, c1, c2, l0q, l1q, l2q, ta_eff, o.ve0, o.ve1, o.ve2);
+    if (has_boundary) {
+      const int b0 = (lfl[l0] & VF_BOUNDARY) ? 1 : 0;
+      const int b1 = (lfl[l1] & VF_BOUNDARY) ? 1 : 0;
+      const int b2 = (lfl[l2] & VF_BOUNDARY) ? 1 : 0;
+      const int n_int = 3 - (b0 + b1 + b2);
+      if (n_int > 0 && n_int < 3) {
+        const double b_sum = o.ve0 * b0 + o.ve1 * b1 + o.ve2 * b2;
+        const double extra = b_sum / (double)n_int;
+        const double m0 = b0 ? 0.0 : 1.0, m1 = b1 ? 0.0 : 1.0, m2 = b2 ? 0.0 : 1.0;
+        o.ve0 = o.ve0 * m0 + m0 * extra;
+        o.ve1 = o.ve1 * m1 + m1 * extra;
+        o.ve2 = o.ve2 * m2 + m2 * extra;
+      }
+    }
+    const double hc0 = 0.5 * c0, hc1 = 0.5 * c1, hc2 = 0.5 * c2;
+    o.K0 = hc2 * e2 - hc1 * e1;
+    o.K1 = hc0 * e0 - hc2 * e2;
+    o.K2 = mk(-o.K0.x - o.K1.x, -o.K0.y - o.K1.y, -o.K0.z - o.K1.z);
+  }
+}
+
 template <bool BEND, bool GUARD, int TT, int CAPC, bool ATOMIC, int MULTI = 0, bool AREA = false>
 __device__ __forceinline__ void energy_body(EnergyArgs& a, int cap_rt, int max_ent, double* lds, int block_id) {
   int bid = block_id;
@@ -426,15 +523,22 @@
   const bool have_d = a.d != nullptr;
 
   constexpr bool PACKED = TT == 256;
+  constexpr bool QUAD = MS_QUADS && ATOMIC && BEND && !GUARD && !AREA && TT == 256;
   FacetRec<PACKED> tf_nx = facet_null<PACKED>();
   double gam_nx = 0.0;
-  if (t.f0 + tid < t.f1) {
+  uint2 tq_nx = make_uint2(0u, 0u);
+  int q0 = 0, q1 = 0;
+  if constexpr (QUAD) {
+    q0 = a.m.tile_quad_off[my_tile];
+    q1 = a.m.tile_quad_off[my_tile + 1];
+    if (q0 + tid < q1) tq_nx = quad_load(a.m, (size_t)(q0 + tid));
+  } else if (t.f0 + tid < t.f1) {
     tf_nx = facet_load<PACKED>(a.m, (size_t)(t.f0 + tid));
     gam_nx = a.m.gamma_uniform ? a.m.gamma_const : a.m.tf_gamma[t.f0 + tid];
   }
 
   double kappa_v = 0.0, c0_v = 0.0;
-  if (BEND && tid < t.n_owned) {
+  if (BEND && !QUAD && tid < t.n_owned) {
     kappa_v = a.m.kc_uniform ? a.m.kappa_const : a.m.kappa[t.v_lo + tid];
     c0_v = a.m.kc_uniform ? a.m.c0_const : a.m.c0[t.v_lo + tid];
   }
@@ -529,15 +633,66 @@
   __syncthreads();
   MS_STAMP(1);
 
-  double e_surf = 0.0, vol = 0.0, min_e2 = 1.0e300, guard = 0.0;
+  EnergyFacetSums fs;
   const bool want_surf = a.modules & MS_MOD_SURFACE;
   const bool want_vol = a.modules & (MS_MOD_VOLUME_PENALTY | MS_CON_VOLUME | MS_TRACK_VOLUME);
   constexpr bool want_area = AREA;
-  double area = 0.0;
   double aKx = 0, aKy = 0, aKz = 0, aAv = 0, aAe = 0;
   if (!(BEND && tid < t.n_owned)) cur = end = 0;
   const int ent_begin = cur;
 
+  if constexpr (QUAD) {
+    const int no = t.n_owned;
+    const bool hb = a.m.has_boundary != 0;
+    for (int c0 = q0; c0 < q1; c0 += T) {
+      const int p = c0 + tid;
+      uint2 tq = tq_nx;
+      if (c0 != q0 && p < q1) tq = quad_load(a.m, (size_t)p);
+      if (p < q1) {
+        const double gam_a = a.m.gamma_uniform ? a.m.gamma_const : a.m.tq_gamma[2 * (size_t)p];
+        const int la = (int)(tq.x & 1023u), lb = (int)((tq.x >> 10) & 1023u), lc = (int)((tq.x >> 20) & 1023u);
+        const int ld = (int)(tq.y & 1023u);
+        const V3 ra = lds_row3(px, la), rb = lds_row3(px, lb), rc = lds_row3(px, lc);
+        EnergyFacetTerms fa;
+        energy_facet<true, false, false>(ra, rb, rc, rb - ra, la, lb, lc, tq.x >> 30, gam_a, want_surf, want_vol, hb, ox, lfl, fs, fa);
+        if (lc < no) {
+          atomicAdd(&stg[lc], fa.K2.x); atomicAdd(&stg[T + lc], fa.K2.y); atomicAdd(&stg[2 * T + lc], fa.K2.z);
+          atomicAdd(&stg[3 * T + lc], fa.va2);
+          if (fa.ve2 != fa.va2) atomicAdd(&stg[4 * T + lc], fa.ve2 - fa.va2);
+        }
+        MS_SCHED_FENCE();
+        V3 Ka = fa.K0, Kb = fa.K1;
+        double ava = fa.va0, avb = fa.va1;
+        if (la < no && fa.ve0 != fa.va0) atomicAdd(&stg[4 * T + la], fa.ve0 - fa.va0);
+        if (lb < no && fa.ve1 != fa.va1) atomicAdd(&stg[4 * T + lb], fa.ve1 - fa.va1);
+        if (tq.y & TQ_HAS_B) {
+          const V3 rd = lds_row3(px, ld);
+          const double gam_b = a.m.gamma_uniform ? a.m.gamma_const : a.m.tq_gamma[2 * (size_t)p + 1];
+          EnergyFacetTerms fb;
+          energy_facet<true, false, false>(rb, ra, rd, ra - rb, lb, la, ld, (tq.y >> 10) & 3u, gam_b, want_surf, want_vol, hb, ox, lfl, fs, fb);
+          if (ld < no) {
+            atomicAdd(&stg[ld], fb.K2.x); atomicAdd(&stg[T + ld], fb.K2.y); atomicAdd(&stg[2 * T + ld], fb.K2.z);
+            atomicAdd(&stg[3 * T + ld], fb.va2);
+            if (fb.ve2 != fb.va2) atomicAdd(&stg[4 * T + ld], fb.ve2 - fb.va2);
+          }
+          Ka = Ka + fb.K1;
+          Kb = Kb + fb.K0;
+          ava += fb.va1;
+          avb += fb.va0;
+          if (la < no && fb.ve1 != fb.va1) atomicAdd(&stg[4 * T + la], fb.ve1 - fb.va1);
+          if (lb < no && fb.ve0 != fb.va0) atomicAdd(&stg[4 * T + lb], fb.ve0 - fb.va0);
+        }
+        if (la < no) {
+          atomicAdd(&stg[la], Ka.x); atomicAdd(&stg[T + la], Ka.y); atomicAdd(&stg[2 * T + la], Ka.z);
+          atomicAdd(&stg[3 * T + la], ava);
+        }
+        if (lb < no) {
+          atomicAdd(&stg[lb], Kb.x); atomicAdd(&stg[T + lb], Kb.y); atomicAdd(&stg[2 * T + lb], Kb.z);
+          atomicAdd(&stg[3 * T + lb], avb);
+        }
+      }
+    }
+  } else
   for (int c0 = t.f0; c0 < t.f1; c0 += T) {
     const int p = c0 + tid;
     const TileFacet tf = facet_unpack<PACKED>(tf_nx);
@@ -546,99 +701,41 @@
       tf_nx = facet_load<PACKED>(a.m, (size_t)(p + T));
       gam_nx = a.m.gamma_uniform ? a.m.gamma_const : a.m.tf_gamma[p + T];
     }
-    double va0 = 0, va1 = 0, va2 = 0, ve0 = 0, ve1 = 0, ve2 = 0;
+    EnergyFacetTerms ft;
     if (p < t.f1) {
       const bool owner = tf.flags & TF_OWNER;
       if (BEND || owner) {
         const V3 v0 = lds_row3(px, tf.l0), v1 = lds_row3(px, tf.l1), v2 = lds_row3(px, tf.l2);
-        const V3 e0 = v2 - v1, e1 = v0 - v2, e2 = v1 - v0;
-        const double l0 = dot(e0, e0), l1 = dot(e1, e1), l2 = dot(e2, e2);
-        const V3 n = cross(e2, -e1);
-#if MS_RSQRT_NORM
-        double A2, inv_A2;
-        norm_and_inverse(dot(n, n), A2, inv_A2);
-#else
-        const double A2 = norm(n);
-#endif
-        if (owner) {
-          if (want_surf && A2 >= 1.0e-12) e_surf += gam * (0.5 * A2);
-          if (want_vol && (tf.flags & TF_BODY)) vol += dot(cross(v1, v2), v0);
-          if (want_area && (tf.flags & TF_BODY) && A2 >= 1.0e-12) area += 0.5 * A2;
-          min_e2 = min_plain(min_e2, min_plain(l0, min_plain(l1, l2)));
-          if (GUARD) {
-            const V3 o0 = lds_row3(ox, tf.l0), o1 = lds_row3(ox, tf.l1), o2 = lds_row3(ox, tf.l2);
-            const V3 no = cross(o1 - o0, o2 - o0);
-            const double nno = norm(no);
-            if (nno > 1.0e-12) {
-              if (A2 < 1.0e-12) {
-                guard = 1.0;
-              } else {
-                double dd = dot(no, n) / (nno * A2);
-                dd = fmin(1.0, fmax(-1.0, dd));
-                if (!(acos(dd) <= 0.5)) guard = 1.0;
-              }
-            }
-          }
-        }
+        energy_facet<BEND, GUARD, AREA>(v0, v1, v2, v1 - v0, tf.l0, tf.l1, tf.l2, tf.flags, gam, want_surf, want_vol,
+                                        a.m.has_boundary != 0, ox, lfl, fs, ft);
         if (BEND) {
-          const double ad = A2 < 1.0e-12 ? 1.0e-12 : A2;
-#if MS_RSQRT_NORM
-          const double inv_ad = A2 < 1.0e-12 ? 1.0e12 : inv_A2;
-#else
-          const double inv_ad = 1.0 / ad;
-#endif
-          const double tri_area = 0.5 * ad;
-          const double c0 = dot(-e1, e2) * inv_ad, c1 = dot(-e2, e0) * inv_ad, c2 = dot(-e0, e1) * inv_ad;
-          corner_areas(c0, c1, c2, l0, l1, l2, tri_area, va0, va1, va2);
-          ve0 = va0;
-          ve1 = va1;
-          ve2 = va2;
-          const double ta_eff = fmax(0.5 * A2, 1.0e-12);
-          if (ta_eff != tri_area) corner_areas(c0, c1, c2, l0, l1, l2, ta_eff, ve0, ve1, ve2);
-          if (a.m.has_boundary) {
-            const int b0 = (lfl[tf.l0] & VF_BOUNDARY) ? 1 : 0;
-            const int b1 = (lfl[tf.l1] & VF_BOUNDARY) ? 1 : 0;
-            const int b2 = (lfl[tf.l2] & VF_BOUNDARY) ? 1 : 0;
-            const int n_int = 3 - (b0 + b1 + b2);
-            if (n_int > 0 && n_int < 3) {
-              const double b_sum = ve0 * b0 + ve1 * b1 + ve2 * b2;
-              const double extra = b_sum / (double)n_int;
-              const double m0 = b0 ? 0.0 : 1.0, m1 = b1 ? 0.0 : 1.0, m2 = b2 ? 0.0 : 1.0;
-              ve0 = ve0 * m0 + m0 * extra;
-              ve1 = ve1 * m1 + m1 * extra;
-              ve2 = ve2 * m2 + m2 * extra;
-            }
-          }
-          const double hc0 = 0.5 * c0, hc1 = 0.5 * c1, hc2 = 0.5 * c2;
-          const V3 K0 = hc2 * e2 - hc1 * e1;
-          const V3 K1 = hc0 * e0 - hc2 * e2;
-          const V3 K2 = mk(-K0.x - K1.x, -K0.y - K1.y, -K0.z - K1.z);
           if (ATOMIC) {
             const int no = t.n_owned;
             if (tf.l0 < no) {
-              atomicAdd(&stg[tf.l0], K0.x); atomicAdd(&stg[T + tf.l0], K0.y); atomicAdd(&stg[2 * T + tf.l0], K0.z);
-              atomicAdd(&stg[3 * T + tf.l0], va0);
-              if (ve0 != va0) atomicAdd(&stg[4 * T + tf.l0], ve0 - va0);
+              atomicAdd(&stg[tf.l0], ft.K0.x); atomicAdd(&stg[T + tf.l0], ft.K0.y); atomicAdd(&stg[2 * T + tf.l0], ft.K0.z);
+              atomicAdd(&stg[3 * T + tf.l0], ft.va0);
+              if (ft.ve0 != ft.va0) atomicAdd(&stg[4 * T + tf.l0], ft.ve0 - ft.va0);
             }
             if (tf.l1 < no) {
-              atomicAdd(&stg[tf.l1], K1.x); atomicAdd(&stg[T + tf.l1], K1.y); atomicAdd(&stg[2 * T + tf.l1], K1.z);
-              atomicAdd(&stg[3 * T + tf.l1], va1);
-              if (ve1 != va1) atomicAdd(&stg[4 * T + tf.l1], ve1 - va1);
+              atomicAdd(&stg[tf.l1], ft.K1.x); atomicAdd(&stg[T + tf.l1], ft.K1.y); atomicAdd(&stg[2 * T + tf.l1], ft.K1.z);
+              atomicAdd(&stg[3 * T + tf.l1], ft.va1);
+              if (ft.ve1 != ft.va1) atomicAdd(&stg[4 * T + tf.l1], ft.ve1 - ft.va1);
             }
             if (tf.l2 < no) {
-              atomicAdd(&stg[tf.l2], K2.x); atomicAdd(&stg[T + tf.l2], K2.y); atomicAdd(&stg[2 * T + tf.l2], K2.z);
-              atomicAdd(&stg[3 * T + tf.l2], va2);
-              if (ve2 != va2) atomicAdd(&stg[4 * T + tf.l2], ve2 - va2);
+              atomicAdd(&stg[tf.l2], ft.K2.x); atomicAdd(&stg[T + tf.l2], ft.K2.y); atomicAdd(&stg[2 * T + tf.l2], ft.K2.z);
+              atomicAdd(&stg[3 * T + tf.l2], ft.va2);
+              if (ft.ve2 != ft.va2) atomicAdd(&stg[4 * T + tf.l2], ft.ve2 - ft.va2);
             }
           } else {
             double* s = stg + tid;
-            s[0 * T] = K0.x; s[1 * T] = K0.y; s[2 * T] = K0.z;
-            s[3 * T] = K1.x; s[4 * T] = K1.y; s[5 * T] = K1.z;
-            s[6 * T] = K2.x; s[7 * T] = K2.y; s[8 * T] = K2.z;
+            s[0 * T] = ft.K0.x; s[1 * T] = ft.K0.y; s[2 * T] = ft.K0.z;
+            s[3 * T] = ft.K1.x; s[4 * T] = ft.K1.y; s[5 * T] = ft.K1.z;
+            s[6 * T] = ft.K2.x; s[7 * T] = ft.K2.y; s[8 * T] = ft.K2.z;
           }
         }
       }
     }
+    const double va0 = ft.va0, va1 = ft.va1, va2 = ft.va2, ve0 = ft.ve0, ve1 = ft.ve1, ve2 = ft.ve2;
     if (BEND && !ATOMIC) {
       const int lo = c0 - t.f0, hi = min(c0 + T, t.f1) - t.f0;
       __syncthreads();
@@ -685,6 +782,10 @@
   double e_bend = 0.0;
   if (BEND && tid < t.n_owned) {
     const int v = t.v_lo + tid;
+    if constexpr (QUAD) {
+      kappa_v = a.m.kc_uniform ? a.m.kappa_const : a.m.kappa[v];
+      c0_v = a.m.kc_uniform ? a.m.c0_const : a.m.c0[v];
+    }
     const V3 K = mk(aKx, aKy, aKz);
     const double kappa = kappa_v, c0 = c0_v;
     const bool interior = !(own_fl & VF_BOUNDARY);
@@ -781,17 +882,17 @@
   double* pout = a.partials + t.tile;
   const size_t pstride = (size_t)a.m.n_tiles;
   if (want_area) {
-    const double vals[6] = {e_surf, vol, e_bend, min_e2, guard, area};
+    const double vals[6] = {fs.e_surf, fs.vol, e_bend, fs.min_e2, fs.guard, fs.area};
     const int ops[6] = {0, 0, 0, 1, 2, 0};
     const int slots[6] = {MS_S_ESURF, MS_S_VOL, MS_S_EBEND, MS_S_MINEDGE2, MS_S_GUARD, MS_S_AREA};
     block_reduce_store<6>(vals, ops, slots, red, pout, pstride);
   } else if (GUARD || want_vol) {
-    const double vals[5] = {e_surf, vol, e_bend, min_e2, guard};
+    const double vals[5] = {fs.e_surf, fs.vol, e_bend, fs.min_e2, fs.guard};
     const int ops[5] = {0, 0, 0, 1, 2};
     const int slots[5] = {MS_S_ESURF, MS_S_VOL, MS_S_EBEND, MS_S_MINEDGE2, MS_S_GUARD};
     block_reduce_store<5>(vals, ops, slots, red, pout, pstride);
   } else {
-    const double vals[3] = {e_surf, e_bend, min_e2};
+    const double vals[3] = {fs.e_surf, e_bend, fs.min_e2};
     const int ops[3] = {0, 0, 1};
     const int slots[3] = {MS_S_ESURF, MS_S_EBEND, MS_S_MINEDGE2};
     if constexpr (MS_REDUCE_STAGED && ATOMIC && BEND && !GUARD && !AREA && TT == 256)
@@ -968,18 +1069,6 @@
   return e;
 }
 
-#ifndef MS_SCHED_FENCES
-#define MS_SCHED_FENCES 1
-#endif
-#if MS_SCHED_FENCES
-#define MS_SCHED_FENCE()                 \
-  do {                                   \
-    asm volatile("" ::: "memory");       \
-    __builtin_amdgcn_sched_barrier(0);   \
-  } while (0)
-#else
-#define MS_SCHED_FENCE() do {} while (0)
-#endif
 #ifndef MS_ABL_NOATOM
 #define MS_ABL_NOATOM 0
 #endif
diff --git a/membrane_solver_amd/csrc/ms_tiles.cpp b/membrane_solver_amd/csrc/ms_tiles.cpp
--- a/membrane_solver_amd/csrc/ms_tiles.cpp
+++ b/membrane_solver_amd/csrc/ms_tiles.cpp
@@ -37,6 +37,8 @@
 }
 
 }
+
+void build_quads(Tiling& out);
 
 int build_tiling(int nv, int nf, const double* positions, const int32_t* tri,
                  const uint8_t* body_facets, int T, int shard_count, Tiling& out,
@@ -336,7 +338,167 @@
     out.max_halo = std::max(out.max_halo, (int)halo_tmp.size());
     out.max_tile_facets = std::max(out.max_tile_facets, (int)(e - b));
   }
+  if (out.own + out.max_halo <= 1024) build_quads(out);
   return MS_OK;
 }
 
+void build_quads(Tiling& out) {
+  const int nt = out.n_tiles;
+  out.tile_quad_off.assign(nt + 1, 0);
+  out.tile_quads.clear();
+  out.tile_quad_inst.clear();
+  out.max_tile_quads = 0;
+  out.paired_instances = 0;
+  std::vector<int32_t> emap((size_t)1024 * 1024, -1);
+  struct Rec {
+    uint16_t s[4];
+    int32_t ia, ib;
+  };
+  std::vector<Rec> recs, recs_tmp;
+  std::vector<int32_t> nb, deg, bucket[4], order, seq;
+  std::vector<uint8_t> done, taken;
+  for (int t = 0; t < nt; ++t) {
+    const int b = out.tile_facet_off[t], n = out.tile_facet_off[t + 1] - b;
+    const TileFacet* tf = out.tile_facets.data() + b;
+    auto slot = [&](int i, int k) -> uint32_t { return k % 3 == 0 ? tf[i].l0 : (k % 3 == 1 ? tf[i].l1 : tf[i].l2); };
+    for (int i = 0; i < n; ++i)
+      for (int k = 0; k < 3; ++k) {
+        const uint32_t u = slot(i, k), v = slot(i, k + 1);
+        if (u != v && emap[u * 1024 + v] < 0) emap[u * 1024 + v] = i;
+      }
+    nb.assign(3 * (size_t)n, -1);
+    deg.assign(n, 0);
+    for (int i = 0; i < n; ++i)
+      for (int k = 0; k < 3; ++k) {
+        const uint32_t u = slot(i, k), v = slot(i, k + 1);
+        if (u == v || emap[u * 1024 + v] != i) continue;
+        const int j = emap[v * 1024 + u];
+        if (j < 0 || j == i) continue;
+        bool dup = false;
+        for (int q = 0; q < k; ++q) dup |= nb[3 * i + q] == j;
+        if (dup) continue;
+        nb[3 * i + k] = j;
+        ++deg[i];
+      }
+    for (int i = 0; i < n; ++i)
+      for (int k = 0; k < 3; ++k) {
+        const uint32_t u = slot(i, k), v = slot(i, k + 1);
+        if (u != v) emap[u * 1024 + v] = -1;
+      }
+    done.assign(n, 0);
+    for (auto& bk : bucket) bk.clear();
+    for (int i = n - 1; i >= 0; --i) bucket[deg[i]].push_back(i);
+    recs.clear();
+    int left = n;
+    while (left > 0) {
+      int i = -1;
+      for (int d = 0; d < 4 && i < 0; ++d)
+        while (!bucket[d].empty()) {
+          const int c = bucket[d].back();
+          bucket[d].pop_back();
+          if (!done[c] && deg[c] == d) {
+            i = c;
+            break;
+          }
+        }
+      if (i < 0) break;
+      int kbest = -1;
+      for (int k = 0; k < 3; ++k) {
+        const int j = nb[3 * i + k];
+        if (j >= 0 && !done[j] && (kbest < 0 || deg[j] < deg[nb[3 * i + kbest]])) kbest = k;
+      }
+      Rec r;
+      r.ia = i;
+      r.ib = -1;
+      done[i] = 1;
+      --left;
+      if (kbest < 0) {
+        r.s[0] = (uint16_t)slot(i, 0);
+        r.s[1] = (uint16_t)slot(i, 1);
+        r.s[2] = (uint16_t)slot(i, 2);
+        r.s[3] = 0;
+      } else {
+        const int j = nb[3 * i + kbest];
+        r.ib = j;
+        done[j] = 1;
+        --left;
+        r.s[0] = (uint16_t)slot(i, kbest);
+        r.s[1] = (uint16_t)slot(i, kbest + 1);
+        r.s[2] = (uint16_t)slot(i, kbest + 2);
+        int m = 0;
+        while (m < 3 && !(slot(j, m) == r.s[1] && slot(j, m + 1) == r.s[0])) ++m;
+        r.s[3] = (uint16_t)slot(j, m + 2);
+        out.paired_instances += 2;
+      }
+      for (int who = 0; who < 2; ++who) {
+        const int f = who == 0 ? r.ia : r.ib;
+        if (f < 0) continue;
+        for (int k = 0; k < 3; ++k) {
+          const int j = nb[3 * f + k];
+          if (j >= 0 && !done[j]) {
+            --deg[j];
+            bucket[deg[j]].push_back(j);
+          }
+        }
+      }
+      recs.push_back(r);
+    }
+    const size_t nr = recs.size();
+    if (nr >= 64) {
+      size_t S = std::max<size_t>(7, (nr + 63) / 64);
+      while (std::gcd(S, nr) != 1) ++S;
+      seq.clear();
+      for (size_t i = 0; i < nr; ++i) seq.push_back((int32_t)((i * S) % nr));
+      taken.assign(nr, 0);
+      order.clear();
+      size_t first_free = 0;
+      while (order.size() < nr) {
+        uint32_t m32[4] = {0, 0, 0, 0};
+        const size_t group_end = std::min(nr, order.size() + 32);
+        for (int half = 0; half < 2 && order.size() < group_end; ++half) {
+          uint32_t m16[4] = {0, 0, 0, 0};
+          const size_t half_end = std::min(group_end, order.size() + 16);
+          while (order.size() < half_end) {
+            size_t best = nr;
+            int best_cost = 99, seen = 0;
+            for (size_t q = first_free; q < nr && seen < 192; ++q) {
+              if (taken[q]) continue;
+              ++seen;
+              const Rec& f = recs[seq[q]];
+              const int ns = f.ib >= 0 ? 4 : 3;
+              int cost = 0;
+              for (int k = 0; k < ns; ++k)
+                cost += (int)((m32[k] >> (f.s[k] & 31)) & 1u) + (int)((m16[k] >> (f.s[k] & 15)) & 1u);
+              if (cost < best_cost) {
+                best_cost = cost;
+                best = q;
+                if (cost == 0) break;
+              }
+            }
+            if (best == nr) break;
+            const Rec& f = recs[seq[best]];
+            const int ns = f.ib >= 0 ? 4 : 3;
+            for (int k = 0; k < ns; ++k) {
+              m32[k] |= 1u << (f.s[k] & 31);
+              m16[k] |= 1u << (f.s[k] & 15);
+            }
+            taken[best] = 1;
+            order.push_back(seq[best]);
+            while (first_free < nr && taken[first_free]) ++first_free;
+          }
+        }
+      }
+      recs_tmp = recs;
+      for (size_t i = 0; i < nr; ++i) recs[i] = recs_tmp[order[i]];
+    }
+    for (const Rec& r : recs) {
+      out.tile_quads.push_back(quad_pack(r.s, tf[r.ia].flags, r.ib >= 0 ? tf[r.ib].flags : (uint16_t)0, r.ib >= 0));
+      out.tile_quad_inst.push_back(b + r.ia);
+      out.tile_quad_inst.push_back(r.ib >= 0 ? b + r.ib : -1);
+    }
+    out.tile_quad_off[t + 1] = (int32_t)out.tile_quads.size();
+    out.max_tile_quads = std::max(out.max_tile_quads, (int)nr);
+  }
 }
+
+}
```

After: 19040. 0.988x the previous value.
